# lixirui142/VidToMe

Hardware: AMD Instinct MI355X
Metric: denoising steps/sec, 16-frame 512x512 SD-1.5 chunk, ratio=0.5 (higher is better)
Workload: dtype f16 tokens; matching f16-MFMA filter + f32 exact refine (f32-identical indices); attention f16 MFMA with f32 accumulate

## Files before the change

### include/vidtome_hip.h

```cpp
#ifndef VIDTOME_HIP_H
#define VIDTOME_HIP_H

#include <stddef.h>
#include <stdint.h>

#ifdef __cplusplus
extern "C" {
#endif

#define VTM_ABI_VERSION 2

enum vtm_dtype { VTM_F32 = 0, VTM_F16 = 1, VTM_BF16 = 2 };

enum vtm_status {
    VTM_OK = 0,
    VTM_EINVAL = -1,
    VTM_ELAUNCH = -2,
    VTM_EWORKSPACE = -3
};

typedef void *vtm_stream_t;

int vtm_version(void);
const char *vtm_last_error(void);
int vtm_build_ablations(void);

#define VTM_MATCH_ROW_PAD 256
#define VTM_MATCH_K_PAD 32
int64_t vtm_pad_rows(int64_t n);
int64_t vtm_pad_k(int64_t C);

int vtm_normalize_gather(const void *x0, int64_t P0, const void *x1, int64_t P1, int dtype, int64_t B,
                         int64_t C, const int32_t *rows, int64_t n, float *norms, float *out,
                         int64_t n_pad, int64_t C_pad, vtm_stream_t stream);

int vtm_match(const float *a, const float *b, int64_t B, int64_t Ns, int64_t Nd, int64_t Ns_pad,
              int64_t Nd_pad, int64_t C_pad, int align, uint64_t *best, vtm_stream_t stream);

size_t vtm_match_filtered_ws_bytes(int64_t B, int64_t C, int64_t Ns, int64_t Nd, int align);
int vtm_match_filtered(const void *x0, int64_t P0, const void *x1, int64_t P1, int dtype, int64_t B,
                       int64_t C, const int32_t *a_rows, int64_t Ns, const int32_t *b_rows, int64_t Nd,
                       int align, void *ws, size_t ws_bytes, uint64_t *best, int32_t *flags_out,
                       vtm_stream_t stream);
int vtm_match_filtered_seeded(const void *x0, int64_t P0, const void *x1, int64_t P1, int dtype, int64_t B,
                              int64_t C, const int32_t *a_rows, int64_t Ns, const int32_t *b_rows, int64_t Nd,
                              int align, void *ws, size_t ws_bytes, uint64_t *best, int32_t *flags_out,
                              int64_t seed_L, int64_t seed_N, const int32_t *seed_pos1, const int32_t *seed_table,
                              vtm_stream_t stream);
#define VTM_MATCH_ONE_LAUNCH 0
#define VTM_MATCH_SCOUT_RANGE 1
#define VTM_MATCH_SCOUT_STEPS(k) (((k) & 0xff) << 8)
int vtm_match_filtered_plan(const void *x0, int64_t P0, const void *x1, int64_t P1, int dtype, int64_t B,
                            int64_t C, const int32_t *a_rows, int64_t Ns, const int32_t *b_rows, int64_t Nd,
                            int align, void *ws, size_t ws_bytes, uint64_t *best, int32_t *flags_out,
                            int64_t seed_L, int64_t seed_N, const int32_t *seed_pos1, const int32_t *seed_table,
                            int mode, vtm_stream_t stream);

#define VTM_POSITION_ORDER_MAX_N 16360
size_t vtm_position_order_counter_ints(int64_t B, int64_t N);
size_t vtm_position_order_ws_bytes(int64_t B, int64_t Ns, int64_t Nd, int64_t N);
int vtm_position_order(const int32_t *a_rows, int64_t Ns, const int32_t *b_rows, int64_t Nd, int64_t B, int64_t L,
                       int64_t N, const int32_t *pos1, int64_t P0, int64_t P1, int32_t *counters, void *ws,
                       size_t ws_bytes, int32_t *a_sorted, int32_t *a_order, int32_t *b_sorted, int32_t *b_order,
                       int32_t *table, int shared_order, vtm_stream_t stream);
int vtm_match_filtered_ordered(const void *x0, int64_t P0, const void *x1, int64_t P1, int dtype, int64_t B,
                               int64_t C, const int32_t *a_sorted, int64_t Ns, const int32_t *b_sorted, int64_t Nd,
                               int align, void *ws, size_t ws_bytes, uint64_t *best, int32_t *flags_out, int64_t seed_L,
                               int64_t seed_N, const int32_t *seed_pos1, const int32_t *seed_table, int mode,
                               const int32_t *a_order, const int32_t *b_order, vtm_stream_t stream);

int vtm_decode_best(const uint64_t *best, int64_t n, float *node_max, int32_t *node_idx,
                    vtm_stream_t stream);

size_t vtm_sort_ws_bytes(int64_t rows, int64_t n);
int vtm_sort_desc(const uint64_t *best, int64_t rows, int64_t n, int32_t *perm, void *ws,
                  size_t ws_bytes, vtm_stream_t stream);

int vtm_partition_counts(int64_t N_in, int64_t unm_pre, int64_t tnum, int64_t ts, int64_t randf,
                         int64_t *Ns, int64_t *Nd);
int vtm_partition_local(const int32_t *cur, int64_t B, int64_t N_in, int64_t unm_pre, int64_t tnum,
                        int64_t ts, int64_t randf, int32_t *a_pos, int32_t *b_pos, int32_t *a_rows,
                        int32_t *b_rows, int64_t Ns, int64_t Nd, vtm_stream_t stream);

int vtm_partition_global(const int32_t *cur_local, int64_t B, int64_t Ml, int64_t anchor_base,
                         int64_t Mg, int local_is_src, int32_t *a_pos, int32_t *b_pos,
                         int32_t *a_rows, int32_t *b_rows, int32_t *seed_table, int64_t tokens,
                         const int32_t *anchor_pos, vtm_stream_t stream);

int vtm_anchor_pos(const int32_t *amap, int64_t B, int64_t M, int64_t L, int64_t tokens, const int32_t *old_pos,
                   int64_t Mg, int32_t *out, vtm_stream_t stream);

int vtm_anchor_maps(const int32_t *inv_g, int64_t N_in, int64_t off, const int32_t *new_cur, int64_t M, int64_t B,
                    int64_t Ml, int64_t L, int64_t tokens, const int32_t *old_pos, int64_t Mg, int32_t *loc, int32_t *amap,
                    int32_t *pos, vtm_stream_t stream);

int vtm_plan_apply(const uint64_t *best, const int32_t *perm, const int32_t *a_pos,
                   const int32_t *b_pos, const int32_t *a_rows, const int32_t *b_rows, int64_t B,
                   int64_t N_in, int64_t Ns, int64_t Nd, int64_t r, int align, int32_t *new_cur,
                   int32_t *inv, int32_t *unm_idx, int32_t *src_idx, int32_t *dst_idx,
                   vtm_stream_t stream);

int vtm_compose(const int32_t *inv_acc, const int32_t *inv_level, int64_t B, int64_t n,
                int64_t level_len, int64_t offset, int32_t *out, vtm_stream_t stream);

int vtm_gather_rows(const void *x0, int64_t P0, const void *x1, int64_t P1, int dtype, int64_t B,
                    int64_t C, const int32_t *map, int64_t M, void *out, int64_t out_rows,
                    vtm_stream_t stream);

enum { VTM_REDUCE_SUM = 0, VTM_REDUCE_PROD = 1, VTM_REDUCE_MEAN = 2, VTM_REDUCE_AMAX = 3, VTM_REDUCE_AMIN = 4 };
int vtm_merge_reduce(const void *x, int dtype, int64_t B, int64_t N, int64_t C, const int32_t *src_rows,
                     const int32_t *dst_rows, const int32_t *seg_dst, const int32_t *seg_order, int64_t r, int64_t Nd,
                     int mode, void *out, int64_t out_ld, int64_t out_row0, vtm_stream_t stream);

int vtm_unmerge_add(const void *y, int64_t M, const int32_t *inv, const void *resid, int dtype,
                    int64_t B, int64_t L, int64_t C, void *out, vtm_stream_t stream);

int vtm_attention(const void *q, int64_t ldq, const void *k, int64_t ldk, const void *vt,
                  int64_t ldvt, void *out, int64_t ldo, int dtype, int64_t B, int64_t h, int64_t M,
                  int64_t Mp, int64_t d, float scale, int share_groups, void *ws, size_t ws_bytes,
                  vtm_stream_t stream);

size_t vtm_attention_ws_bytes(int64_t B, int64_t h, int64_t Mq, int64_t Mk, int64_t d);

int vtm_attention_kv(const void *q, int64_t ldq, const void *k, int64_t ldk, const void *vt, int64_t ldvt,
                     void *out, int64_t ldo, int dtype, int64_t B, int64_t h, int64_t Mq, int64_t Mqp,
                     int64_t Mk, int64_t Mkp, int64_t d, float scale, int share_groups, void *ws, size_t ws_bytes,
                     vtm_stream_t stream);

int vtm_attention_kv_sets(const void *q, int64_t ldq, const void *k, int64_t ldk, const void *vt, int64_t ldvt,
                          void *out, int64_t ldo, int dtype, int64_t B, int64_t h, int64_t Mq, int64_t Mqp,
                          int64_t Mkp, int64_t d, float scale, int n_sets, const int64_t *set_start,
                          const int64_t *set_len, const float *set_weight, vtm_stream_t stream);

int vtm_attention_kv_bounded(const void *q, int64_t ldq, const void *k, int64_t ldk, const void *vt, int64_t ldvt,
                             void *out, int64_t ldo, int dtype, int64_t B, int64_t h, int64_t Mq, int64_t Mqp,
                             int64_t Mk, int64_t Mkp, int64_t d, float scale, const int32_t *q_count, void *ws,
                             size_t ws_bytes, vtm_stream_t stream);
int vtm_attention_kv_shared_bounded(const void *q, int64_t ldq, const void *k, int64_t ldk, const void *vt, int64_t ldvt,
                                    void *out, int64_t ldo, int dtype, int64_t B, int64_t h, int64_t Mq, int64_t Mqp,
                                    int64_t Mk, int64_t Mkp, int64_t d, float scale, int share_groups,
                                    const int32_t *q_count, void *ws, size_t ws_bytes, vtm_stream_t stream);
size_t vtm_attention_kv_bounded_ws_bytes(int64_t B, int64_t h, int64_t Mq, int64_t Mk, int64_t d);

int vtm_transpose_cols(const void *x, int64_t ldx, int dtype, int64_t BF, int64_t N, int64_t C, void *out, int64_t ldo,
                       vtm_stream_t stream);

size_t vtm_fold_keys_ws_bytes(int64_t B, int64_t M, int64_t n_ids);
int vtm_fold_keys(const int32_t *cur, int64_t B, int64_t M, int64_t L, const int32_t *cid, int64_t Ma, int64_t n_ids,
                  int dtype, void *ws, size_t ws_bytes, int32_t *key_sel, uint32_t *k_bias, int64_t ldkb,
                  int32_t *k_count, vtm_stream_t stream);
int vtm_attention_kv_folded(const void *q, int64_t ldq, const void *k, int64_t ldk, const void *vt, int64_t ldvt,
                            void *out, int64_t ldo, int dtype, int64_t B, int64_t h, int64_t Mq, int64_t Mqp,
                            int64_t Mk, int64_t Mkp, int64_t d, float scale, const int32_t *q_count,
                            const int32_t *k_count, const uint32_t *k_bias, int64_t ldkb, void *ws, size_t ws_bytes,
                            vtm_stream_t stream);

size_t vtm_compact_queries_ws_bytes(int64_t B, int64_t Nd);
int vtm_compact_queries(const int32_t *loc, int64_t B, int64_t Ml, int64_t U, int64_t Nd, void *ws, size_t ws_bytes,
                        int32_t *qc, int32_t *tmap, int32_t *count, vtm_stream_t stream);

int64_t vtm_panel_rows(int64_t n);
int vtm_to_panels(const void *x, int dtype, int64_t rows, int64_t C, const int32_t *order, void *out, int64_t rows_pad,
                  vtm_stream_t stream);
int vtm_layernorm_panels(const void *x, const void *gamma, const void *beta, int dtype, int64_t rows, int64_t C, float eps,
                         void *out, int64_t panel_rows, vtm_stream_t stream);
int vtm_gather_panels(const void *x0, int64_t P0, const void *x1, int64_t P1, int dtype, int64_t B, int64_t C,
                      const int32_t *map, int64_t map_ld, const int32_t *map2, int64_t n, void *out, int64_t rows_per_sample,
                      vtm_stream_t stream);
int vtm_ff_geglu(const void *x_panels, int64_t n, int64_t n_pad, const void *w1_panels, int64_t D, int64_t w_rows_pad,
                 int64_t K, const float *bias, int dtype, void *out_panels, vtm_stream_t stream);
int vtm_linear_panels(const void *x_panels, int64_t n, int64_t n_pad, const void *w_panels, int64_t N, int64_t w_rows_pad,
                      int64_t K, const float *bias, const void *resid, int dtype, void *out, int64_t ldo,
                      vtm_stream_t stream);

int vtm_cfg_ddim(const void *x, const void *eps_uncond, const void *eps_cond, int dtype, int64_t n,
                 float guidance, float a, float b, float c, float d, void *eps_out, void *x_out,
                 vtm_stream_t stream);

int vtm_layernorm(const void *x, const void *gamma, const void *beta, int dtype, int64_t rows, int64_t C,
                  float eps, void *out, vtm_stream_t stream);

int vtm_geglu(const void *x, int dtype, int64_t rows, int64_t D, void *out, vtm_stream_t stream);

int vtm_linear_rows(const void *x0, int64_t P0, const void *x1, int64_t P1, int dtype, int64_t B, int64_t K,
                    const int32_t *rows, int64_t rows_ld, const int32_t *rows2, int64_t n, const void *W,
                    const void *bias, int64_t N, void *out, int64_t ldo, int64_t out_batch_stride,
                    int transposed, vtm_stream_t stream);

enum { VTM_LINEAR_NONE = 0, VTM_LINEAR_RESID = 1, VTM_LINEAR_GEGLU = 2 };
int vtm_linear_f32(const float *x0, int64_t P0, const float *x1, int64_t P1, int64_t B, int64_t K,
                   const int32_t *rows, int64_t rows_ld, const int32_t *rows2, int64_t n, const float *W,
                   const float *bias, int64_t N, int epilogue, const float *resid, void *out, int out_dtype,
                   int64_t ldo, int64_t out_batch_stride, int transposed, vtm_stream_t stream);

int vtm_lora_fold(const void *w, int dtype, const float *up, const float *down, int64_t c_out, int64_t c_in,
                  int64_t r, void *out, vtm_stream_t stream);

int vtm_dora_norms(const void *w, int dtype, const float *up, const float *down, int64_t c_out, int64_t c_in,
                   int64_t r, int64_t k_dora, float *norms, vtm_stream_t stream);
int vtm_dora_fold(const void *w, int dtype, const float *up, const float *down, const float *magnitude,
                  const float *norms, int64_t c_out, int64_t c_in, int64_t r, int64_t k_dora, void *out,
                  vtm_stream_t stream);

#ifdef __cplusplus
}
#endif
#endif
```

### vidtome_amd/_lib.py

```python
from __future__ import annotations

import ctypes
import functools
import os
import threading
from typing import Optional, Tuple

import torch

_HERE = os.path.dirname(os.path.abspath(__file__))
ABI_VERSION = 2
LIB_PATH = os.environ.get("VIDTOME_HIP_LIB") or os.path.join(_HERE, "lib", "libvidtome_hip.so")

VTM_F32, VTM_F16, VTM_BF16 = 0, 1, 2
ROW_PAD, K_PAD = 256, 32

_DT = {torch.float32: VTM_F32, torch.float16: VTM_F16, torch.bfloat16: VTM_BF16}

_vp, _i64, _int, _f32 = ctypes.c_void_p, ctypes.c_int64, ctypes.c_int, ctypes.c_float
_lib: Optional[ctypes.CDLL] = None

_SIGNATURES = {
    "vtm_version": ([], _int),
    "vtm_last_error": ([], ctypes.c_char_p),
    "vtm_build_ablations": ([], _int),
    "vtm_pad_rows": ([_i64], _i64),
    "vtm_pad_k": ([_i64], _i64),
    "vtm_normalize_gather": ([_vp, _i64, _vp, _i64, _int, _i64, _i64, _vp, _i64, _vp, _vp, _i64, _i64, _vp], _int),
    "vtm_match": ([_vp, _vp, _i64, _i64, _i64, _i64, _i64, _i64, _int, _vp, _vp], _int),
    "vtm_match_filtered_ws_bytes": ([_i64, _i64, _i64, _i64, _int], ctypes.c_size_t),
    "vtm_match_filtered": ([_vp, _i64, _vp, _i64, _int, _i64, _i64, _vp, _i64, _vp, _i64, _int, _vp, ctypes.c_size_t,
                            _vp, _vp, _vp], _int),
    "vtm_match_filtered_plan": ([_vp, _i64, _vp, _i64, _int, _i64, _i64, _vp, _i64, _vp, _i64, _int, _vp, ctypes.c_size_t,
                                 _vp, _vp, _i64, _i64, _vp, _vp, _int, _vp], _int),
    "vtm_match_filtered_ordered": ([_vp, _i64, _vp, _i64, _int, _i64, _i64, _vp, _i64, _vp, _i64, _int, _vp, ctypes.c_size_t,
                                    _vp, _vp, _i64, _i64, _vp, _vp, _int, _vp, _vp, _vp], _int),
    "vtm_position_order_counter_ints": ([_i64, _i64], ctypes.c_size_t),
    "vtm_position_order_ws_bytes": ([_i64, _i64, _i64, _i64], ctypes.c_size_t),
    "vtm_position_order": ([_vp, _i64, _vp, _i64, _i64, _i64, _i64, _vp, _i64, _i64, _vp, _vp, ctypes.c_size_t, _vp, _vp, _vp,
                            _vp, _vp, _int, _vp], _int),
    "vtm_match_filtered_seeded": ([_vp, _i64, _vp, _i64, _int, _i64, _i64, _vp, _i64, _vp, _i64, _int, _vp, ctypes.c_size_t,
                                   _vp, _vp, _i64, _i64, _vp, _vp, _vp], _int),
    "vtm_anchor_pos": ([_vp, _i64, _i64, _i64, _i64, _vp, _i64, _vp, _vp], _int),
    "vtm_decode_best": ([_vp, _i64, _vp, _vp, _vp], _int),
    "vtm_sort_ws_bytes": ([_i64, _i64], ctypes.c_size_t),
    "vtm_sort_desc": ([_vp, _i64, _i64, _vp, _vp, ctypes.c_size_t, _vp], _int),
    "vtm_partition_counts": ([_i64, _i64, _i64, _i64, _i64, ctypes.POINTER(_i64), ctypes.POINTER(_i64)], _int),
    "vtm_partition_local": ([_vp, _i64, _i64, _i64, _i64, _i64, _i64, _vp, _vp, _vp, _vp, _i64, _i64, _vp], _int),
    "vtm_partition_global": ([_vp, _i64, _i64, _i64, _i64, _int, _vp, _vp, _vp, _vp, _vp, _i64, _vp, _vp], _int),
    "vtm_plan_apply": ([_vp, _vp, _vp, _vp, _vp, _vp, _i64, _i64, _i64, _i64, _i64, _int, _vp, _vp, _vp, _vp,
                        _vp, _vp], _int),
    "vtm_compose": ([_vp, _vp, _i64, _i64, _i64, _i64, _vp, _vp], _int),
    "vtm_gather_rows": ([_vp, _i64, _vp, _i64, _int, _i64, _i64, _vp, _i64, _vp, _i64, _vp], _int),
    "vtm_unmerge_add": ([_vp, _i64, _vp, _vp, _int, _i64, _i64, _i64, _vp, _vp], _int),
    "vtm_merge_reduce": ([_vp, _int, _i64, _i64, _i64, _vp, _vp, _vp, _vp, _i64, _i64, _int, _vp, _i64, _i64, _vp], _int),
    "vtm_attention": ([_vp, _i64, _vp, _i64, _vp, _i64, _vp, _i64, _int, _i64, _i64, _i64, _i64, _i64, _f32,
                       _int, _vp, ctypes.c_size_t, _vp], _int),
    "vtm_attention_ws_bytes": ([_i64, _i64, _i64, _i64, _i64], ctypes.c_size_t),
    "vtm_attention_kv": ([_vp, _i64, _vp, _i64, _vp, _i64, _vp, _i64, _int, _i64, _i64, _i64, _i64, _i64, _i64, _i64,
                          _f32, _int, _vp, ctypes.c_size_t, _vp], _int),
    "vtm_attention_kv_sets": ([_vp, _i64, _vp, _i64, _vp, _i64, _vp, _i64, _int, _i64, _i64, _i64, _i64, _i64, _i64, _f32,
                               _int, ctypes.POINTER(_i64), ctypes.POINTER(_i64), ctypes.POINTER(_f32), _vp], _int),
    "vtm_attention_kv_bounded": ([_vp, _i64, _vp, _i64, _vp, _i64, _vp, _i64, _int, _i64, _i64, _i64, _i64, _i64, _i64, _i64,
                                  _f32, _vp, _vp, ctypes.c_size_t, _vp], _int),
    "vtm_attention_kv_shared_bounded": ([_vp, _i64, _vp, _i64, _vp, _i64, _vp, _i64, _int, _i64, _i64, _i64, _i64, _i64, _i64, _i64,
                                         _f32, _int, _vp, _vp, ctypes.c_size_t, _vp], _int),
    "vtm_attention_kv_bounded_ws_bytes": ([_i64, _i64, _i64, _i64, _i64], ctypes.c_size_t),
    "vtm_anchor_maps": ([_vp, _i64, _i64, _vp, _i64, _i64, _i64, _i64, _i64, _vp, _i64, _vp, _vp, _vp, _vp], _int),
    "vtm_transpose_cols": ([_vp, _i64, _int, _i64, _i64, _i64, _vp, _i64, _vp], _int),
    "vtm_fold_keys_ws_bytes": ([_i64, _i64, _i64], ctypes.c_size_t),
    "vtm_fold_keys": ([_vp, _i64, _i64, _i64, _vp, _i64, _i64, _int, _vp, ctypes.c_size_t, _vp, _vp, _i64, _vp, _vp], _int),
    "vtm_attention_kv_folded": ([_vp, _i64, _vp, _i64, _vp, _i64, _vp, _i64, _int, _i64, _i64, _i64, _i64, _i64, _i64, _i64,
                                 _f32, _vp, _vp, _vp, _i64, _vp, ctypes.c_size_t, _vp], _int),
    "vtm_compact_queries_ws_bytes": ([_i64, _i64], ctypes.c_size_t),
    "vtm_compact_queries": ([_vp, _i64, _i64, _i64, _i64, _vp, ctypes.c_size_t, _vp, _vp, _vp, _vp], _int),
    "vtm_panel_rows": ([_i64], _i64),
    "vtm_to_panels": ([_vp, _int, _i64, _i64, _vp, _vp, _i64, _vp], _int),
    "vtm_layernorm_panels": ([_vp, _vp, _vp, _int, _i64, _i64, _f32, _vp, _i64, _vp], _int),
    "vtm_gather_panels": ([_vp, _i64, _vp, _i64, _int, _i64, _i64, _vp, _i64, _vp, _i64, _vp, _i64, _vp], _int),
    "vtm_ff_geglu": ([_vp, _i64, _i64, _vp, _i64, _i64, _i64, _vp, _int, _vp, _vp], _int),
    "vtm_linear_panels": ([_vp, _i64, _i64, _vp, _i64, _i64, _i64, _vp, _vp, _int, _vp, _i64, _vp], _int),
    "vtm_cfg_ddim": ([_vp, _vp, _vp, _int, _i64, _f32, _f32, _f32, _f32, _f32, _vp, _vp, _vp], _int),
    "vtm_layernorm": ([_vp, _vp, _vp, _int, _i64, _i64, _f32, _vp, _vp], _int),
    "vtm_geglu": ([_vp, _int, _i64, _i64, _vp, _vp], _int),
    "vtm_linear_rows": ([_vp, _i64, _vp, _i64, _int, _i64, _i64, _vp, _i64, _vp, _i64, _vp, _vp, _i64, _vp, _i64, _i64,
                         _int, _vp], _int),
    "vtm_lora_fold": ([_vp, _int, _vp, _vp, _i64, _i64, _i64, _vp, _vp], _int),
    "vtm_dora_norms": ([_vp, _int, _vp, _vp, _i64, _i64, _i64, _i64, _vp, _vp], _int),
    "vtm_dora_fold": ([_vp, _int, _vp, _vp, _vp, _vp, _i64, _i64, _i64, _i64, _vp, _vp], _int),
    "vtm_linear_f32": ([_vp, _i64, _vp, _i64, _i64, _i64, _vp, _i64, _vp, _i64, _vp, _vp, _i64, _int, _vp, _vp, _int, _i64,
                        _i64, _int, _vp], _int),
}


def exported_symbols():
    return sorted(_SIGNATURES)


def lib() -> ctypes.CDLL:
    global _lib
    if _lib is None:
        if not os.path.exists(LIB_PATH):
            raise RuntimeError(
                f"{LIB_PATH} is missing: build it with `python -m vidtome_amd.build` (hipcc, gfx950). "
                "vidtome_amd has no CPU / eager fallback.")
        L = ctypes.CDLL(LIB_PATH)
        for name, (argtypes, restype) in _SIGNATURES.items():
            fn = getattr(L, name)
            fn.argtypes = argtypes
            fn.restype = restype
        if L.vtm_version() != ABI_VERSION:
            raise RuntimeError("libvidtome_hip.so ABI version mismatch")
        if L.vtm_build_ablations() != 0 and os.environ.get("VIDTOME_ALLOW_ABLATED") != "1":
            raise RuntimeError(f"{LIB_PATH} was built with ablation switches (mask {L.vtm_build_ablations():#x}); "
                               "set VIDTOME_ALLOW_ABLATED=1 to load it for a timing experiment")
        _lib = L
    return _lib


def _check(rc: int, what: str) -> None:
    if rc != 0:
        msg = lib().vtm_last_error()
        raise RuntimeError(f"{what} failed ({rc}): {msg.decode() if msg else ''}")


def _stream() -> int:
    return torch.cuda.current_stream().cuda_stream


def _on_device(fn):
    @functools.wraps(fn)
    def guarded(*args, **kwargs):
        dev = next((a.device if isinstance(a, torch.Tensor) else a for a in args
                    if isinstance(a, (torch.Tensor, torch.device))), None)
        if dev is None or dev.type != "cuda" or dev.index is None or dev.index == torch.cuda.current_device():
            return fn(*args, **kwargs)
        with torch.cuda.device(dev.index):
            return fn(*args, **kwargs)
    return guarded


def _ptr(t: Optional[torch.Tensor]) -> Optional[int]:
    return None if t is None else t.data_ptr()


_WS: dict = {}
_WS_LOCK = threading.Lock()


def _workspace(tag: str, nbytes: int, device: torch.device) -> torch.Tensor:
    key = (device.index, torch.cuda.current_stream(device).cuda_stream, tag, threading.get_ident())
    buf = _WS.get(key)
    if buf is None or buf.numel() < nbytes:
        new = torch.empty((max(int(nbytes), 16),), dtype=torch.uint8, device=device)
        with _WS_LOCK:
            if buf is None:
                alive = {t.ident for t in threading.enumerate()}
                for k in [k for k in list(_WS) if k[3] not in alive]:
                    _WS.pop(k, None)
            _WS[key] = new
        buf = new
    return buf


def release_workspaces() -> None:
    with _WS_LOCK:
        _WS.clear()
        _ZEROED.clear()


def _req(t: torch.Tensor, name: str) -> torch.Tensor:
    if not t.is_cuda:
        raise RuntimeError(f"{name} must live on the GPU (vidtome_amd has no CPU path)")
    if not t.is_contiguous():
        raise RuntimeError(f"{name} must be contiguous")
    return t


def dtype_code(t: torch.Tensor) -> int:
    try:
        return _DT[t.dtype]
    except KeyError:
        raise RuntimeError(f"unsupported dtype {t.dtype}") from None


def pad_rows(n: int) -> int:
    return (n + ROW_PAD - 1) // ROW_PAD * ROW_PAD


def pad_k(c: int) -> int:
    return (c + K_PAD - 1) // K_PAD * K_PAD


@_on_device
def normalize_gather(x0: torch.Tensor, x1: Optional[torch.Tensor], rows: torch.Tensor
                     ) -> Tuple[torch.Tensor, torch.Tensor]:
    _req(x0, "x0"), _req(rows, "rows")
    B, P0, C = x0.shape
    P1 = 0 if x1 is None else _req(x1, "x1").shape[1]
    n = rows.shape[1]
    n_pad, C_pad = pad_rows(n), pad_k(C)
    out = torch.empty((B, C_pad // 8, 2, n_pad, 4), dtype=torch.float32, device=x0.device)
    norms = torch.empty((B, max(n, 1)), dtype=torch.float32, device=x0.device)
    _check(lib().vtm_normalize_gather(_ptr(x0), P0, _ptr(x1), P1, dtype_code(x0), B, C, _ptr(rows), n,
                                      _ptr(norms), _ptr(out), n_pad, C_pad, _stream()), "vtm_normalize_gather")
    return out, norms


@_on_device
def match(a: torch.Tensor, b: torch.Tensor, Ns: int, Nd: int, align: bool) -> torch.Tensor:
    B, G, _, Ns_pad, _ = a.shape
    C_pad, Nd_pad = G * 8, b.shape[3]
    best = torch.empty((1 if align else B, Ns), dtype=torch.int64, device=a.device)
    _check(lib().vtm_match(_ptr(a), _ptr(b), B, Ns, Nd, Ns_pad, Nd_pad, C_pad, int(align), _ptr(best), _stream()),
           "vtm_match")
    return best


MATCH_ONE_LAUNCH, MATCH_SCOUT_RANGE = 0, 1


@_on_device
def match_filtered(x0: torch.Tensor, x1: Optional[torch.Tensor], a_rows: torch.Tensor, b_rows: torch.Tensor,
                   align: bool, want_flag: bool = False, seed=None, mode: int = MATCH_ONE_LAUNCH,
                   stats_host: Optional[torch.Tensor] = None, order=None, scout_steps: int = 0):
    _req(x0, "x0"), _req(a_rows, "a_rows"), _req(b_rows, "b_rows")
    B, P0, C = x0.shape
    P1 = 0 if x1 is None else _req(x1, "x1").shape[1]
    Ns, Nd = a_rows.shape[1], b_rows.shape[1]
    nbytes = lib().vtm_match_filtered_ws_bytes(B, C, Ns, Nd, int(align))
    ws = _workspace("match", nbytes, x0.device)
    best = torch.empty((1 if align else B, Ns), dtype=torch.int64, device=x0.device)
    flag = torch.zeros((8,), dtype=torch.int32, device=x0.device) if want_flag else None
    flags_out = _ptr(flag)
# ... 195 lines not shown
    if r > 0:
        keys = ((-1 - dst_idx.long()) << 32).contiguous()
        order = sort_desc(keys)
        seg_dst = torch.gather(dst_idx, 1, order.long()).contiguous()
    else:
        order = seg_dst = dst_idx
    _check(lib().vtm_merge_reduce(_ptr(x), dtype_code(x), B, N, C, _ptr(src_rows), _ptr(dst_rows), _ptr(seg_dst), _ptr(order),
                                  r, Nd, REDUCE_MODES[mode], _ptr(out), out.shape[1], out_row0, _stream()), "vtm_merge_reduce")
    return out


@_on_device
def unmerge_add(y: torch.Tensor, inv: torch.Tensor, resid: Optional[torch.Tensor]) -> torch.Tensor:
    _req(y, "y"), _req(inv, "inv")
    B, Mp, C = y.shape
    L = inv.shape[1]
    out = torch.empty((B, L, C), dtype=y.dtype, device=y.device)
    if resid is not None:
        _req(resid, "resid")
        if resid.numel() != out.numel() or resid.dtype != y.dtype:
            raise RuntimeError("residual shape/dtype mismatch")
    _check(lib().vtm_unmerge_add(_ptr(y), Mp, _ptr(inv), _ptr(resid), dtype_code(y), B, L, C, _ptr(out), _stream()),
           "vtm_unmerge_add")
    return out


@_on_device
def transpose_cols(x: torch.Tensor, c0: int, C: int) -> torch.Tensor:
    _req(x, "x")
    BF, N, ld = x.shape
    if x.stride(2) != 1 or x.stride(1) != ld or x.stride(0) != N * ld or c0 % 8 or C % 8:
        raise RuntimeError("transpose_cols: dense (BF, N, ld) input, column window aligned to 8")
    Np = (N + 7) // 8 * 8
    out = torch.empty((BF, C, Np), dtype=x.dtype, device=x.device)
    _check(lib().vtm_transpose_cols(x.data_ptr() + c0 * x.element_size(), ld, dtype_code(x), BF, N, C, _ptr(out), Np, _stream()),
           "vtm_transpose_cols")
    return out


SEED_MATCHER = os.environ.get("VIDTOME_SEED", "1") != "0"

SPLIT_ALL_BOUNDED = os.environ.get("VIDTOME_ATT_SPLIT_ALL", "1") != "0"

FOLD_KEYS = os.environ.get("VIDTOME_FOLD_KEYS", "1") != "0"


def _attention_ws(B: int, heads: int, Mq: int, Mk: int, d: int, device):
    nb = int(lib().vtm_attention_ws_bytes(B, heads, Mq, Mk, d))
    if nb == 0:
        return None, 0
    return _workspace("attention", nb, device), nb


@_on_device
def attention(q: torch.Tensor, k: torch.Tensor, vt: torch.Tensor, heads: int, M: int, scale: float,
              share_groups: int = 1) -> torch.Tensor:
    B, Mp, C = q.shape
    d = C // heads
    if q.stride(2) != 1 or k.stride(2) != 1 or vt.stride(2) != 1:
        raise RuntimeError("attention operands must be contiguous along their last axis")
    if q.stride(0) != Mp * q.stride(1) or k.stride(0) != Mp * k.stride(1) or vt.stride(0) != C * vt.stride(1):
        raise RuntimeError("attention operands must have dense batch strides")
    out = torch.zeros((B, Mp, C), dtype=q.dtype, device=q.device) if Mp != M else \
        torch.empty((B, Mp, C), dtype=q.dtype, device=q.device)
    ws, nb = _attention_ws(B, heads, M, M, d, q.device)
    _check(lib().vtm_attention(q.data_ptr(), q.stride(1), k.data_ptr(), k.stride(1), vt.data_ptr(), vt.stride(1),
                               out.data_ptr(), C, dtype_code(q), B, heads, M, Mp, d, float(scale),
                               int(share_groups), _ptr(ws), nb, _stream()), "vtm_attention")
    return out


@_on_device
def cfg_ddim(x: Optional[torch.Tensor], eps_uncond: torch.Tensor, eps_cond: Optional[torch.Tensor], guidance: float,
             a: float, b: float, c: float, d: float, want_eps: bool = False):
    _req(eps_uncond, "eps_uncond")
    n = eps_uncond.numel()
    b, c, d = (float(torch.tensor(v, dtype=torch.float32).to(eps_uncond.dtype)) for v in (b, c, d))
    a = float(torch.tensor(a, dtype=torch.float32))
    x_out = torch.empty_like(eps_uncond) if x is not None else None
    eps_out = torch.empty_like(eps_uncond) if (want_eps or x is None) else None
    _check(lib().vtm_cfg_ddim(_ptr(x), _ptr(eps_uncond), _ptr(eps_cond), dtype_code(eps_uncond), n, float(guidance),
                              float(a), float(b), float(c), float(d), _ptr(eps_out), _ptr(x_out), _stream()),
           "vtm_cfg_ddim")
    return (x_out, eps_out) if want_eps else (x_out if x is not None else eps_out)


@_on_device
def layernorm(x: torch.Tensor, weight: Optional[torch.Tensor], bias: Optional[torch.Tensor], eps: float) -> torch.Tensor:
    _req(x, "x")
    C = x.shape[-1]
    xc = x.contiguous()
    for name, p in (("weight", weight), ("bias", bias)):
        if p is not None and (p.dtype != x.dtype or p.numel() != C or p.device != x.device):
            raise RuntimeError(f"vidtome_amd: layernorm {name} must be a ({C},) {x.dtype} tensor on {x.device}")
    out = torch.empty_like(xc)
    _check(lib().vtm_layernorm(_ptr(xc), _ptr(weight.contiguous() if weight is not None else None),
                               _ptr(bias.contiguous() if bias is not None else None), dtype_code(xc),
                               xc.numel() // C, C, float(eps), _ptr(out), _stream()), "vtm_layernorm")
    return out


@_on_device
def attention_kv(q: torch.Tensor, k: torch.Tensor, vt: torch.Tensor, heads: int, Mq: int, Mk: int, scale: float,
                 use_workspace: bool = True, q_count: Optional[torch.Tensor] = None,
                 k_fold: Optional[Tuple[torch.Tensor, torch.Tensor]] = None, share_groups: int = 1) -> torch.Tensor:
    if share_groups != 1 and k_fold is not None:
        raise RuntimeError("attention_kv: shared probabilities do not go with folded keys")
    if k_fold is not None and q.dtype == torch.float32:
        raise RuntimeError("attention_kv: fp32 keys are never folded (k_fold takes fp16 / bf16 operands)")
    B, Mqp, C = q.shape
    Mkp = k.shape[1]
    d = C // heads
    if q.stride(2) != 1 or k.stride(2) != 1 or vt.stride(2) != 1:
        raise RuntimeError("attention operands must be contiguous along their last axis")
    if q.stride(0) != Mqp * q.stride(1) or k.stride(0) != Mkp * k.stride(1) or vt.stride(0) != C * vt.stride(1):
        raise RuntimeError("attention operands must have dense batch strides")
    out = torch.zeros((B, Mqp, C), dtype=q.dtype, device=q.device) if Mqp != Mq else \
        torch.empty((B, Mqp, C), dtype=q.dtype, device=q.device)
    ws, nb = _attention_ws(B, heads, Mq, Mk, d, q.device) if use_workspace else (None, 0)
    if q_count is not None and (q_count.dtype != torch.int32 or q_count.numel() != B or not q_count.is_cuda):
        raise RuntimeError("attention_kv: q_count must be a (B,) int32 device tensor")
    if q_count is not None and use_workspace and SPLIT_ALL_BOUNDED:
        nb2 = int(lib().vtm_attention_kv_bounded_ws_bytes(B, heads, Mq, Mk, d))
        if nb2 > nb:
            ws, nb = _workspace("attention", nb2, q.device), nb2
    if share_groups != 1 and q_count is not None:
        _check(lib().vtm_attention_kv_shared_bounded(q.data_ptr(), q.stride(1), k.data_ptr(), k.stride(1), vt.data_ptr(),
                                                     vt.stride(1), out.data_ptr(), C, dtype_code(q), B, heads, Mq, Mqp, Mk, Mkp,
                                                     d, float(scale), int(share_groups), _ptr(q_count), _ptr(ws), nb, _stream()),
               "vtm_attention_kv_shared_bounded")
        return out
    if k_fold is not None:
        k_count, k_bias = k_fold
        if k_count.dtype != torch.int32 or k_count.numel() != B or k_bias.dtype != torch.int32 or k_bias.dim() != 2 \
                or k_bias.shape[0] != B or k_bias.shape[1] < Mk or not k_bias.is_contiguous():
            raise RuntimeError("attention_kv: k_fold must be ((B,) int32 counts, (B, >= Mk) int32 bias words)")
        _check(lib().vtm_attention_kv_folded(q.data_ptr(), q.stride(1), k.data_ptr(), k.stride(1), vt.data_ptr(), vt.stride(1),
                                             out.data_ptr(), C, dtype_code(q), B, heads, Mq, Mqp, Mk, Mkp, d, float(scale),
                                             _ptr(q_count), _ptr(k_count), _ptr(k_bias), k_bias.shape[1], _ptr(ws), nb,
                                             _stream()), "vtm_attention_kv_folded")
        return out
    if q_count is not None:
        _check(lib().vtm_attention_kv_bounded(q.data_ptr(), q.stride(1), k.data_ptr(), k.stride(1), vt.data_ptr(),
                                              vt.stride(1), out.data_ptr(), C, dtype_code(q), B, heads, Mq, Mqp, Mk, Mkp,
                                              d, float(scale), _ptr(q_count), _ptr(ws), nb, _stream()),
               "vtm_attention_kv_bounded")
        return out
    _check(lib().vtm_attention_kv(q.data_ptr(), q.stride(1), k.data_ptr(), k.stride(1), vt.data_ptr(), vt.stride(1),
                                  out.data_ptr(), C, dtype_code(q), B, heads, Mq, Mqp, Mk, Mkp, d, float(scale),
                                  int(share_groups), _ptr(ws), nb, _stream()), "vtm_attention_kv")
    return out


MAX_KEY_SETS = 8


@_on_device
def attention_kv_range(q: torch.Tensor, k: torch.Tensor, vt: torch.Tensor, heads: int, Mq: int, start: int, Mk: int,
                       scale: float) -> torch.Tensor:
    start, Mk = int(start), int(Mk)
    B, Mqp, C = q.shape
    Mkp = k.shape[1]
    if start % 8 or start < 0 or Mk < 1 or start + Mk > Mkp or start + Mk > vt.shape[2]:
        raise RuntimeError("attention_kv_range: the range must start on a multiple of 8 and lie inside k and vt")
    if start == 0:
        return attention_kv(q, k, vt, heads, Mq, Mk, scale)
    d = C // heads
    if q.stride(2) != 1 or k.stride(2) != 1 or vt.stride(2) != 1:
        raise RuntimeError("attention operands must be contiguous along their last axis")
    if q.stride(0) != Mqp * q.stride(1) or k.stride(0) != Mkp * k.stride(1) or vt.stride(0) != C * vt.stride(1):
        raise RuntimeError("attention operands must have dense batch strides")
    out = torch.zeros((B, Mqp, C), dtype=q.dtype, device=q.device) if Mqp != Mq else \
        torch.empty((B, Mqp, C), dtype=q.dtype, device=q.device)
    ws, nb = _attention_ws(B, heads, Mq, Mk, d, q.device)
    es = k.element_size()
    _check(lib().vtm_attention_kv(q.data_ptr(), q.stride(1), k.data_ptr() + start * k.stride(1) * es, k.stride(1),
                                  vt.data_ptr() + start * es, vt.stride(1), out.data_ptr(), C, dtype_code(q), B, heads, Mq, Mqp,
                                  Mk, Mkp, d, float(scale), 1, _ptr(ws), nb, _stream()), "vtm_attention_kv")
    return out


@_on_device
def attention_kv_sets(q: torch.Tensor, k: torch.Tensor, vt: torch.Tensor, heads: int, Mq: int, sets, scale: float
                      ) -> torch.Tensor:
    sets = [(int(s), int(n), float(w)) for s, n, w in sets]
    if not 1 <= len(sets) <= MAX_KEY_SETS:
        raise RuntimeError(f"attention_kv_sets: 1 .. {MAX_KEY_SETS} key sets, got {len(sets)}")
    if q.dtype not in (torch.float16, torch.bfloat16) or k.dtype != q.dtype or vt.dtype != q.dtype:
        raise RuntimeError("attention_kv_sets: q, k and vt must share one of fp16 / bf16 (fp32 models keep the module path)")
    B, Mqp, C = q.shape
    Mkp = k.shape[1]
    d = C // heads
    if q.stride(2) != 1 or k.stride(2) != 1 or vt.stride(2) != 1:
        raise RuntimeError("attention operands must be contiguous along their last axis")
    if q.stride(0) != Mqp * q.stride(1) or k.stride(0) != Mkp * k.stride(1) or vt.stride(0) != C * vt.stride(1):
        raise RuntimeError("attention operands must have dense batch strides")
    if k.shape[0] != B or vt.shape[0] != B or k.shape[2] != C or vt.shape[1] != C:
        raise RuntimeError("attention_kv_sets: k must be (B, Mkp, C) and vt (B, C, ldvt)")
    if len(sets) == 1 and sets[0][2] == 1.0:
        return attention_kv_range(q, k, vt, heads, Mq, sets[0][0], sets[0][1], scale)
    out = torch.zeros((B, Mqp, C), dtype=q.dtype, device=q.device) if Mqp != Mq else \
        torch.empty((B, Mqp, C), dtype=q.dtype, device=q.device)
    n = len(sets)
    starts = (_i64 * n)(*[s for s, _, _ in sets])
    lens = (_i64 * n)(*[m for _, m, _ in sets])
    weights = (_f32 * n)(*[w for _, _, w in sets])
    _check(lib().vtm_attention_kv_sets(q.data_ptr(), q.stride(1), k.data_ptr(), k.stride(1), vt.data_ptr(), vt.stride(1),
                                       out.data_ptr(), C, dtype_code(q), B, heads, Mq, Mqp, Mkp, d, float(scale), n, starts,
                                       lens, weights, _stream()), "vtm_attention_kv_sets")
    return out


@_on_device
def compact_queries(loc: torch.Tensor, U: int, Nd: int) -> Tuple[torch.Tensor, torch.Tensor, torch.Tensor]:
    _req(loc, "loc")
    B, Ml = loc.shape
    i32 = dict(dtype=torch.int32, device=loc.device)
    qc, tmap, count = torch.empty((B, Ml), **i32), torch.empty((B, Ml), **i32), torch.empty((B,), **i32)
    nb = int(lib().vtm_compact_queries_ws_bytes(B, Nd))
    ws = _workspace("compact", nb, loc.device)
    _check(lib().vtm_compact_queries(_ptr(loc), B, Ml, U, Nd, _ptr(ws), nb, _ptr(qc), _ptr(tmap), _ptr(count), _stream()),
           "vtm_compact_queries")
    return qc, tmap, count


@_on_device
def fold_keys(cur: torch.Tensor, L: int, cid: torch.Tensor, n_ids: int, dtype: torch.dtype
              ) -> Tuple[torch.Tensor, torch.Tensor, torch.Tensor]:
    _req(cur, "cur")
    _req(cid, "cid")
    B, M = cur.shape
    Mp = (M + 7) // 8 * 8
    i32 = dict(dtype=torch.int32, device=cur.device)
    key_sel, k_bias, k_count = torch.empty((B, M), **i32), torch.empty((B, Mp), **i32), torch.empty((B,), **i32)
    code = {torch.float16: 1, torch.bfloat16: 2}[dtype]
    nb = int(lib().vtm_fold_keys_ws_bytes(B, M, n_ids))
    ws = _workspace("fold", nb, cur.device)
    _check(lib().vtm_fold_keys(_ptr(cur), B, M, L, _ptr(cid), cid.shape[1], n_ids, code, _ptr(ws), nb, _ptr(key_sel),
                               _ptr(k_bias), Mp, _ptr(k_count), _stream()), "vtm_fold_keys")
    return key_sel, k_bias, k_count


@_on_device
def geglu(x: torch.Tensor) -> torch.Tensor:
    _req(x, "x")
    D = x.shape[-1] // 2
    xc = x.contiguous()
    out = torch.empty(xc.shape[:-1] + (D,), dtype=x.dtype, device=x.device)
    _check(lib().vtm_geglu(_ptr(xc), dtype_code(xc), xc.numel() // (2 * D), D, _ptr(out), _stream()), "vtm_geglu")
    return out


@_on_device
def linear_rows(x0: torch.Tensor, x1: Optional[torch.Tensor], rows: Optional[torch.Tensor],
                rows2: Optional[torch.Tensor], n: int, weight: torch.Tensor, bias: Optional[torch.Tensor],
                transposed: bool = False, pad_to: int = 8, out: Optional[torch.Tensor] = None) -> torch.Tensor:
    _req(x0, "x0"), _req(weight, "weight")
    B, P0, K = x0.shape
    P1 = 0 if x1 is None else _req(x1, "x1").shape[1]
    N = weight.shape[0]
    if weight.shape[1] != K or weight.dtype != x0.dtype:
        raise RuntimeError("linear_rows: weight must be (N, K) in the token dtype")
    if rows is not None:
        _req(rows, "rows")
    if rows2 is not None:
        _req(rows2, "rows2")
    n_pad = (n + pad_to - 1) // pad_to * pad_to
    if out is None:
        out = torch.empty((B, N, n_pad) if transposed else (B, n_pad, N), dtype=x0.dtype, device=x0.device)
        if n_pad != n:
            (out[:, :, n:] if transposed else out[:, n:]).zero_()
    if out.stride(2) != 1:
        raise RuntimeError("linear_rows: out must be contiguous along its last axis")
    _check(lib().vtm_linear_rows(_ptr(x0), P0, _ptr(x1), P1, dtype_code(x0), B, K, _ptr(rows),
                                 0 if rows is None else rows.shape[1], _ptr(rows2), n, _ptr(weight),
                                 _ptr(bias.contiguous() if bias is not None else None), N, out.data_ptr(), out.stride(1),
                                 out.stride(0), int(transposed), _stream()), "vtm_linear_rows")
    return out


LINEAR_NONE, LINEAR_RESID, LINEAR_GEGLU = 0, 1, 2
_EPILOGUES = {"none": LINEAR_NONE, "resid": LINEAR_RESID, "geglu": LINEAR_GEGLU}


@_on_device
def linear_f32(x0: torch.Tensor, x1: Optional[torch.Tensor], rows: Optional[torch.Tensor],
               rows2: Optional[torch.Tensor], n: int, weight: torch.Tensor, bias: Optional[torch.Tensor],
               epilogue: str = "none", resid: Optional[torch.Tensor] = None, out_dtype: torch.dtype = torch.float32,
               transposed: bool = False, pad_to: int = 8, out: Optional[torch.Tensor] = None) -> torch.Tensor:
    _req(x0, "x0"), _req(weight, "weight")
    B, P0, K = x0.shape
    P1 = 0 if x1 is None else _req(x1, "x1").shape[1]
    N = weight.shape[0]
    if x0.dtype != torch.float32 or weight.dtype != torch.float32 or weight.shape[1] != K \
            or (x1 is not None and x1.dtype != torch.float32):
        raise RuntimeError("linear_f32: tokens and weight must be fp32, weight (N, K)")
    if out_dtype not in (torch.float32, torch.float16):
        raise RuntimeError("linear_f32: out_dtype must be fp32 or fp16")
    epi = _EPILOGUES[epilogue]
    Nout = N // 2 if epi == LINEAR_GEGLU else N
    if bias is not None:
        bias = bias.detach().float().contiguous()
    for t, name in ((rows, "rows"), (rows2, "rows2")):
        if t is not None:
            _req(t, name)
    n_pad = (n + pad_to - 1) // pad_to * pad_to
    if out is None:
        out = torch.empty((B, Nout, n_pad) if transposed else (B, n_pad, Nout), dtype=out_dtype, device=x0.device)
        if n_pad != n:
            (out[:, :, n:] if transposed else out[:, n:]).zero_()
    if out.stride(2) != 1 or out.dtype != out_dtype:
        raise RuntimeError("linear_f32: out must be of out_dtype and contiguous along its last axis")
    if epi == LINEAR_RESID and (resid is None or resid.dtype != torch.float32 or resid.shape[0] != B
                                or resid.stride()[B == 1:] != out.stride()[B == 1:]):
        raise RuntimeError("linear_f32: resid must be fp32 with the strides of the result")
    _check(lib().vtm_linear_f32(_ptr(x0), P0, _ptr(x1), P1, B, K, _ptr(rows), 0 if rows is None else rows.shape[1],
                                _ptr(rows2), n, _ptr(weight), _ptr(bias), N, epi, _ptr(resid), out.data_ptr(),
                                dtype_code(out), out.stride(1), out.stride(0), int(transposed), _stream()),
           "vtm_linear_f32")
    return out


def panel_rows(n: int) -> int:
    return (n + ROW_PAD - 1) // ROW_PAD * ROW_PAD


@_on_device
def to_panels(x: torch.Tensor, order: Optional[torch.Tensor] = None, rows: Optional[int] = None) -> torch.Tensor:
    _req(x, "x")
    C = x.shape[-1]
    x2 = x.reshape(-1, C)
    n = x2.shape[0] if order is None else order.numel()
    n = n if rows is None else rows
    out = torch.empty((C // 8, panel_rows(n), 8), dtype=x.dtype, device=x.device)
    _check(lib().vtm_to_panels(_ptr(x2), dtype_code(x2), n, C, _ptr(order), _ptr(out), out.shape[1], _stream()),
           "vtm_to_panels")
    return out


@_on_device
def layernorm_panels(x: torch.Tensor, weight: Optional[torch.Tensor], bias: Optional[torch.Tensor], eps: float) -> torch.Tensor:
    _req(x, "x")
    C = x.shape[-1]
    xc = x.contiguous()
    rows = xc.numel() // C
    out = torch.empty((C // 8, panel_rows(rows), 8), dtype=x.dtype, device=x.device)
    _check(lib().vtm_layernorm_panels(_ptr(xc), _ptr(weight), _ptr(bias), dtype_code(xc), rows, C, float(eps), _ptr(out),
                                      out.shape[1], _stream()), "vtm_layernorm_panels")
    return out


@_on_device
def ff_geglu(x_panels: torch.Tensor, n: int, w1_panels: torch.Tensor, D: int, bias: Optional[torch.Tensor]) -> torch.Tensor:
    K = x_panels.shape[0] * 8
    out = torch.empty((D // 8, x_panels.shape[1], 8), dtype=x_panels.dtype, device=x_panels.device)
    _check(lib().vtm_ff_geglu(_ptr(x_panels), n, x_panels.shape[1], _ptr(w1_panels), D, w1_panels.shape[1], K, _ptr(bias),
                              dtype_code(x_panels), _ptr(out), _stream()), "vtm_ff_geglu")
    return out


@_on_device
def linear_panels(x_panels: torch.Tensor, n: int, w_panels: torch.Tensor, N: int, bias: Optional[torch.Tensor],
                  resid: Optional[torch.Tensor] = None, out: Optional[torch.Tensor] = None) -> torch.Tensor:
    K = x_panels.shape[0] * 8
    if x_panels.stride(2) != 1 or x_panels.stride(1) != 8 or w_panels.stride(2) != 1 or w_panels.stride(1) != 8 \
            or w_panels.shape[0] * 8 != K:
        raise RuntimeError("linear_panels: operands must be (K / 8, rows, 8) panel tensors (or row ranges of one)")
    if out is None:
        out = torch.empty((n, N), dtype=x_panels.dtype, device=x_panels.device)
    if out.stride(1) != 1 or out.shape[0] < n or out.shape[1] < N:
        raise RuntimeError("linear_panels: out must be an (n, N) view, contiguous along its rows")
    if resid is not None:
        _req(resid, "resid")
        if resid.numel() != n * N or resid.dtype != out.dtype or out.stride(0) != N:
            raise RuntimeError("linear_panels: residual shape / dtype mismatch")
    _check(lib().vtm_linear_panels(_ptr(x_panels), n, x_panels.stride(0) // 8, _ptr(w_panels), N, w_panels.stride(0) // 8, K,
                                   _ptr(bias), _ptr(resid), dtype_code(x_panels), out.data_ptr(), out.stride(0), _stream()),
           "vtm_linear_panels")
    return out


@_on_device
def gather_panels(x0: torch.Tensor, x1: Optional[torch.Tensor], rows: Optional[torch.Tensor], rows2: Optional[torch.Tensor],
                  n: int) -> torch.Tensor:
    _req(x0, "x0")
    B, P0, C = x0.shape
    P1 = 0 if x1 is None else _req(x1, "x1").shape[1]
    n_pad = panel_rows(n)
    out = torch.empty((C // 8, B * n_pad, 8), dtype=x0.dtype, device=x0.device)
    _check(lib().vtm_gather_panels(_ptr(x0), P0, _ptr(x1), P1, dtype_code(x0), B, C, _ptr(rows),
                                   0 if rows is None else rows.shape[1], _ptr(rows2), n, _ptr(out), n_pad, _stream()),
           "vtm_gather_panels")
    return out


@_on_device
def lora_fold(w: torch.Tensor, up: torch.Tensor, down: torch.Tensor, out: Optional[torch.Tensor] = None) -> torch.Tensor:
    _req(w, "w"), _req(up, "up"), _req(down, "down")
    c_out, c_in = w.shape
    r = up.shape[1]
    if up.dtype != torch.float32 or down.dtype != torch.float32 or tuple(up.shape) != (c_out, r) \
            or tuple(down.shape) != (r, c_in) or up.device != w.device or down.device != w.device:
        raise RuntimeError("lora_fold: up must be (c_out, r) and down (r, c_in) fp32 tensors on w's device")
    if out is None:
        out = torch.empty_like(w)
    _check(lib().vtm_lora_fold(_ptr(w), dtype_code(w), _ptr(up), _ptr(down), c_out, c_in, r, _ptr(_req(out, "out")),
                               _stream()), "vtm_lora_fold")
    return out


def _fold_operands(what: str, w: torch.Tensor, up: torch.Tensor, down: torch.Tensor, k_dora: int) -> Tuple[int, int, int]:
    _req(w, "w"), _req(up, "up"), _req(down, "down")
    c_out, c_in = w.shape
    r = up.shape[1]
    if up.dtype != torch.float32 or down.dtype != torch.float32 or tuple(up.shape) != (c_out, r) \
            or tuple(down.shape) != (r, c_in) or up.device != w.device or down.device != w.device:
        raise RuntimeError(f"{what}: up must be (c_out, r) and down (r, c_in) fp32 tensors on w's device")
    if not 0 < k_dora <= r:
        raise RuntimeError(f"{what}: k_dora {k_dora} not in [1, r = {r}]")
    return c_out, c_in, r


@_on_device
def dora_norms(w: torch.Tensor, up: torch.Tensor, down: torch.Tensor, k_dora: int,
               out: Optional[torch.Tensor] = None) -> torch.Tensor:
    c_out, c_in, r = _fold_operands("dora_norms", w, up, down, k_dora)
    if out is None:
        out = torch.empty(c_out, dtype=torch.float32, device=w.device)
    if out.dtype != torch.float32 or tuple(out.shape) != (c_out,) or out.device != w.device:
        raise RuntimeError("dora_norms: out must be an fp32 (c_out,) tensor on w's device")
    _check(lib().vtm_dora_norms(_ptr(w), dtype_code(w), _ptr(up), _ptr(down), c_out, c_in, r, k_dora, _ptr(_req(out, "out")),
                                _stream()), "vtm_dora_norms")
    return out


@_on_device
def dora_fold(w: torch.Tensor, up: torch.Tensor, down: torch.Tensor, magnitude: torch.Tensor, k_dora: int,
              norms: Optional[torch.Tensor] = None, out: Optional[torch.Tensor] = None) -> torch.Tensor:
    c_out, c_in, r = _fold_operands("dora_fold", w, up, down, k_dora)
    if norms is None:
        norms = dora_norms(w, up, down, k_dora)
    for name, t in (("magnitude", magnitude), ("norms", norms)):
        if t.dtype != torch.float32 or tuple(t.shape) != (c_out,) or t.device != w.device:
            raise RuntimeError(f"dora_fold: {name} must be an fp32 (c_out,) tensor on w's device")
    if out is None:
        out = torch.empty_like(w)
    _check(lib().vtm_dora_fold(_ptr(w), dtype_code(w), _ptr(up), _ptr(down), _ptr(_req(magnitude, "magnitude")),
                               _ptr(_req(norms, "norms")), c_out, c_in, r, k_dora, _ptr(_req(out, "out")), _stream()),
           "vtm_dora_fold")
    return out
```

### vidtome_amd/csrc/attention.hip

```cpp
#include "attention_plan.h"

#include <algorithm>
#include <type_traits>

namespace {

template <typename T, int D>
__global__ __launch_bounds__(waves_for(D) * 64) void attention_combine_kernel(
    const float *__restrict__ partial, T *__restrict__ out, int64_t ldo, int64_t H, int64_t M, int64_t Mp, int64_t nqb,
    int64_t id0, int nsplit, int xcd_groups, const int32_t *__restrict__ q_count, const DevPlan *__restrict__ dev_plan) {
    constexpr int WAVES = waves_for(D), NT = WAVES * 64, QB = WAVES * QW, DV = (D + 31) / 32;
    constexpr bool PV16 = pv16_for(D);
    constexpr int NA = acc_floats(D), NM = max_floats(D), REC = rec_floats(D);
    const int tid = threadIdx.x, lane = tid & 63, wave = tid >> 6;
    const int l31 = lane & 31, hi = lane >> 5;
    int64_t rec0 = (int64_t)blockIdx.x * nsplit;
    int64_t pos = id0 + blockIdx.x;
    if (dev_plan != nullptr) {
        if ((int)blockIdx.x >= dev_plan->split_items) return;
        nqb = dev_plan->nqb;
        xcd_groups = nqb >= 64 ? xcd_groups : 0;
        pos = dev_plan->tier[0].items + blockIdx.x;
        int ti = 1;
        while (ti + 1 < dev_plan->ntiers && pos >= dev_plan->tier[ti + 1].item0) ++ti;
        const DevTier tr = dev_plan->tier[ti];
        nsplit = tr.nsplit;
        rec0 = tr.rec0 + (pos - tr.item0) * tr.nsplit;
    }
    const int64_t lin = item_of(pos, nqb, xcd_groups);
    const int64_t b = lin / (nqb * H), h = (lin / nqb) % H;
    const int64_t q0 = (lin % nqb) * QB + wave * QW;
    if (q_count != nullptr && (lin % nqb) * QB >= (int64_t)q_count[b]) return;
    float acc[NA], m[NM], l = 0.0f;
#pragma unroll
    for (int r = 0; r < NA; ++r) acc[r] = 0.0f;
#pragma unroll
    for (int j = 0; j < NM; ++j) m[j] = -INFINITY;
    for (int sp = 0; sp < nsplit; ++sp) {
        const float *pp = partial + (rec0 + sp) * REC * NT + tid;
        float fa[NM], fb[NM];
#pragma unroll
        for (int j = 0; j < NM; ++j) {
            const float ms = pp[(NA + j) * NT];
            const float mn = fmaxf(m[j], ms);
            fa[j] = __builtin_amdgcn_exp2f(m[j] - mn);
            fb[j] = __builtin_amdgcn_exp2f(ms - mn);
            m[j] = mn;
        }
        l = l * fa[0] + pp[(NA + NM) * NT] * fb[0];
#pragma unroll
        for (int r = 0; r < NA; ++r) {
            const int j = PV16 ? (r >> 2) & 1 : 0;
            acc[r] = acc[r] * fa[j] + pp[r * NT] * fb[j];
        }
    }
    if constexpr (PV16) {
        f32x4 o[(D + 16) / 16][2];
#pragma unroll
        for (int r = 0; r < NA; ++r) o[r >> 3][(r >> 2) & 1][r & 3] = acc[r];
        write_output16<T, D>(o, out, ldo, b, h, q0, M, Mp, lane);
    } else {
        f32x16 o[DV];
#pragma unroll
        for (int r = 0; r < NA; ++r) o[r >> 4][r & 15] = acc[r];
        write_output<T, D>(o, l, out, ldo, b, h, q0, M, Mp, l31, hi);
    }
}

template <typename T, int D>
__global__ __launch_bounds__(waves_for(D) * 64) void attention_combine_parts_kernel(
    const float *__restrict__ partial, T *__restrict__ out, int64_t ldo, int64_t H, int64_t M, int64_t Mp, int64_t nqb,
    int64_t id0, int nsplit, int xcd_groups, const int32_t *__restrict__ q_count) {
    using elem = typename Frag<T>::elem;
    static_assert(!pv16_for(D), "32-row O^T layout");
    constexpr int WAVES = waves_for(D), NT = WAVES * 64, QB = WAVES * QW;
    constexpr int NA = acc_floats(D), REC = rec_floats(D);
    constexpr bool SPARE = (D % 32) != 0;
    constexpr int LREG_ALL = SPARE ? (D / 32) * 16 + ((D % 32) & 3) + 4 * ((D % 32) >> 3) : 0;
    constexpr int LHI = ((D % 32) >> 2) & 1;
    const int tid = threadIdx.x, lane = tid & 63, wave = tid >> 6;
    const int l31 = lane & 31, hi = lane >> 5;
    const int64_t lin = item_of(id0 + blockIdx.x, nqb, xcd_groups);
    const int64_t b = lin / (nqb * H), h = (lin / nqb) % H;
    const int64_t q0 = (lin % nqb) * QB + wave * QW;
    if (q_count != nullptr && (lin % nqb) * QB >= (int64_t)q_count[b]) return;
    const int r0 = (int)blockIdx.y * 8;
    const float *p0 = partial + (int64_t)blockIdx.x * nsplit * REC * NT + tid;
    float m = -INFINITY;
#pragma unroll 4
    for (int sp = 0; sp < nsplit; ++sp) m = fmaxf(m, p0[((int64_t)sp * REC + NA) * NT]);
    float acc[8], den = 0.0f;
#pragma unroll
    for (int i = 0; i < 8; ++i) acc[i] = 0.0f;
#pragma unroll 4
    for (int sp = 0; sp < nsplit; ++sp) {
        const float *pp = p0 + (int64_t)sp * REC * NT;
        const float ms = pp[NA * NT];
        const float w = ms == -INFINITY ? 0.0f : __builtin_amdgcn_exp2f(ms - m);
        den = __builtin_fmaf(pp[(SPARE ? LREG_ALL : NA + 1) * NT], w, den);
#pragma unroll
        for (int i = 0; i < 8; ++i) acc[i] = __builtin_fmaf(pp[(r0 + i) * NT], w, acc[i]);
    }
    const float l_tot = SPARE ? __shfl(den, l31 + 32 * LHI, 64) : den + __shfl_xor(den, 32, 64);
    const float inv_l = 1.0f / l_tot;
    const int64_t qi = q0 + l31;
    if (qi < M) {
        T *op = out + (b * Mp + qi) * ldo + h * D;
        const int dv = r0 >> 4, g0 = (r0 & 15) >> 2;
#pragma unroll
        for (int gi = 0; gi < 2; ++gi) {
            const int d0 = dv * 32 + 8 * (g0 + gi) + 4 * hi;
            if (d0 < D) {
                elem w4[4];
#pragma unroll
                for (int e = 0; e < 4; ++e) w4[e] = (elem)(acc[gi * 4 + e] * inv_l);
                *reinterpret_cast<uint2 *>(op + d0) = *reinterpret_cast<uint2 *>(w4);
            }
        }
    }
}

template <typename T, int D, bool FOLD>
__global__ __launch_bounds__(waves_for(D) * 64, (D <= 48 ? 4 : D <= 96 ? 4 : 1)) void attention_kernel(
    const T *__restrict__ q, int64_t ldq, const T *__restrict__ k, int64_t ldk,
    const T *__restrict__ vt, int64_t ldvt, T *__restrict__ out, int64_t ldo, int64_t H,
    int64_t M, int64_t Mp, int64_t Mk_arg, int64_t Mkp, float scale_log2e, int64_t src_batch, int64_t nqb, int64_t nwhole,
    int nsplit_tail, float *__restrict__ partial_base, int xcd_groups, const int32_t *__restrict__ q_count,
    int64_t split_major_items, const int32_t *__restrict__ k_count, const uint32_t *__restrict__ k_bias, int64_t ldkb,
    const DevPlan *__restrict__ dev_plan) {
    using F = Frag<T>;
    using vec = typename F::vec;
    using elem = typename F::elem;
    constexpr int WAVES = waves_for(D), NT = WAVES * 64, QB = WAVES * QW;
    constexpr int DK = (D + 15) / 16;
    constexpr int DV = (D + 31) / 32;
    constexpr bool PV16 = pv16_for(D);
    constexpr int DV16 = (D + 16) / 16, VROWS = vrows_for(D);
    constexpr bool SPARE = (D % 32) != 0;
    constexpr bool BIAS = (D % 16) != 0;
    constexpr int BIAS_HI = (D % 16) / 8, BIAS_E = D % 8;
    static_assert(!FOLD || (BIAS && D % 8 == 0 && D % 16 == 8), "key folding needs the spare k-slots of a d % 16 == 8 head");
    constexpr int K_STRIDE = DK * 16 + 8;
    constexpr int DCH = D / 8;
    constexpr int K_CHUNKS = KV * DCH;
    constexpr int V_CHUNKS = D * (KV / 8);
    constexpr int K_PER_T = (K_CHUNKS + NT - 1) / NT;
    constexpr int V_PER_T = (V_CHUNKS + NT - 1) / NT;
    constexpr int SK_TILE = KV * K_STRIDE, SV_TILE = VROWS * VT_STRIDE;

    extern __shared__ __attribute__((aligned(16))) char smem[];
    elem *sK = reinterpret_cast<elem *>(smem);
    elem *sV = sK + 2 * SK_TILE;

    const int tid = threadIdx.x, lane = tid & 63, wave = tid >> 6;
    const int l31 = lane & 31, hi = lane >> 5;
    const int l15 = lane & 15, g16 = lane >> 4;
    int64_t tier_item0 = nwhole, tier_wg0 = nwhole, tier_rec0 = 0;
    if (dev_plan != nullptr) {
        nqb = dev_plan->nqb;
        xcd_groups = nqb >= 64 ? xcd_groups : 0;
        int ti = 0;
        while (ti + 1 < dev_plan->ntiers && (int)blockIdx.x >= dev_plan->tier[ti + 1].wg0) ++ti;
        const DevTier tr = dev_plan->tier[ti];
        if ((int64_t)blockIdx.x >= (int64_t)tr.wg0 + (int64_t)tr.items * tr.nsplit) return;
        nwhole = dev_plan->tier[0].items;
        nsplit_tail = tr.nsplit;
        split_major_items = tr.items;
        tier_item0 = tr.item0;
        tier_wg0 = tr.wg0;
        tier_rec0 = tr.rec0;
    }
    const bool tail_wg = (int64_t)blockIdx.x >= nwhole;
    const int64_t tail_id = (int64_t)blockIdx.x - tier_wg0;
    const int nsplit = tail_wg ? nsplit_tail : 1;
    const int64_t tail_item = split_major_items ? tail_id % split_major_items : tail_id / nsplit;
    const int split = !tail_wg ? 0 : split_major_items ? (int)(tail_id / split_major_items) : (int)(tail_id % nsplit);
    const int64_t lin = item_of(tail_wg ? tier_item0 + tail_item : (int64_t)blockIdx.x, nqb, xcd_groups);
    float *partial = tail_wg ? partial_base + (tier_rec0 + tail_item * nsplit + split) * rec_floats(D) * (waves_for(D) * 64) : nullptr;
    const int64_t b = lin / (nqb * H), h = (lin / nqb) % H;
    const int64_t bq = b % src_batch;
    const int64_t q0 = (lin % nqb) * QB + wave * QW;
    const int64_t C = H * D;
    int64_t Mk = Mk_arg;
    if constexpr (FOLD) {
        const int64_t kc = k_count[b];
        Mk = kc < Mk_arg ? (kc > 0 ? kc : 1) : Mk_arg;
    }
    if (q_count != nullptr && (lin % nqb) * QB >= (int64_t)q_count[b]) return;

    for (int i = tid; i < 2 * KV * (K_STRIDE - D); i += NT) {
        const int row = i / (K_STRIDE - D), c = D + i % (K_STRIDE - D);
        if (FOLD && (c == D + 2 || c == D + 3)) continue;
        sK[row * K_STRIDE + c] = (elem)((BIAS && c == D) ? 1.0f : 0.0f);
    }
    if constexpr (VROWS > D) {
        for (int i = tid; i < 2 * (VROWS - D) * VT_STRIDE; i += NT) {
            const int bufi = i / ((VROWS - D) * VT_STRIDE), rem = i % ((VROWS - D) * VT_STRIDE);
            const int row = D + rem / VT_STRIDE, c = rem % VT_STRIDE;
            sV[bufi * SV_TILE + row * VT_STRIDE + c] = (elem)((row == D) ? 1.0f : 0.0f);
        }
    }

    vec qf[DK];
    {
        const int64_t qi = q0 + l31;
        const T *qp = q + (bq * Mp + (qi < M ? qi : 0)) * ldq + h * D;
#pragma unroll
        for (int ks = 0; ks < DK; ++ks) {
            const int d0 = ks * 16 + hi * 8;
            uint4 v = make_uint4(0, 0, 0, 0);
            if (d0 < D && qi < M) v = *reinterpret_cast<const uint4 *>(qp + d0);
            qf[ks] = *reinterpret_cast<vec *>(&v);
            if constexpr (BIAS) {
#pragma unroll
                for (int e = 0; e < 8; ++e) qf[ks][e] = (elem)((float)qf[ks][e] * scale_log2e);
            }
        }
        if constexpr (FOLD) {
            if (hi == BIAS_HI) {
                qf[DK - 1][BIAS_E + 2] = (elem)1.0f;
                qf[DK - 1][BIAS_E + 3] = (elem)1.0f;
            }
        }
    }

    uint32_t kgo[K_PER_T], vgo[V_PER_T];
    int koff[K_PER_T], voff[V_PER_T], krow[K_PER_T], vkey[V_PER_T];
    bool kok[K_PER_T], vok[V_PER_T];
#pragma unroll
    for (int i = 0; i < K_PER_T; ++i) {
        const int c = tid + i * NT;
        kok[i] = c < K_CHUNKS;
        krow[i] = c / DCH;
        kgo[i] = kok[i] ? (uint32_t)(krow[i] * (int)ldk + (c % DCH) * 8) * 2u : 0u;
        koff[i] = krow[i] * K_STRIDE + (c % DCH) * 8;
    }
#pragma unroll
    for (int i = 0; i < V_PER_T; ++i) {
        const int c = tid + i * NT;
        vok[i] = c < V_CHUNKS;
        vkey[i] = (c % (KV / 8)) * 8;
        vgo[i] = vok[i] ? (uint32_t)((c / (KV / 8)) * (int)ldvt + vkey[i]) * 2u : 0u;
        voff[i] = (c / (KV / 8)) * VT_STRIDE + (vkey[i] & ~15) + ((vkey[i] >> 3) & 1) * 4;
    }
    const auto rsrc_k = __builtin_amdgcn_make_buffer_rsrc(const_cast<T *>(k + bq * Mkp * ldk + h * D), 0, 0x7fffffff, 0x00020000);
    const auto rsrc_v = __builtin_amdgcn_make_buffer_rsrc(const_cast<T *>(vt + (b * C + h * D) * ldvt), 0, 0x7fffffff, 0x00020000);
    const uint32_t kstep = (uint32_t)(KV * ldk) * 2u, vstep = (uint32_t)KV * 2u;
    uint32_t so_k = 0, so_v = 0;
    const auto rsrc_b = __builtin_amdgcn_make_buffer_rsrc(const_cast<uint32_t *>(FOLD ? k_bias + b * ldkb : nullptr), 0, 0x7fffffff, 0x00020000);
    uint32_t so_b = 0, rbias = 0;
    [[maybe_unused]] const uint32_t bgo = (uint32_t)(tid & (KV - 1)) * 4u;
    auto fetch = [](const auto &rsrc, uint32_t voff_, uint32_t soff_) {
        return __builtin_bit_cast(uint4, __builtin_amdgcn_raw_buffer_load_b128(rsrc, voff_, soff_, 0));
    };

    uint4 rk[K_PER_T], rv[V_PER_T];
    auto issue_full = [&]() {
#pragma unroll
        for (int i = 0; i < K_PER_T; ++i) rk[i] = fetch(rsrc_k, kgo[i], so_k);
#pragma unroll
        for (int i = 0; i < V_PER_T; ++i) rv[i] = fetch(rsrc_v, vgo[i], so_v);
        if constexpr (FOLD) {
            rbias = __builtin_amdgcn_raw_buffer_load_b32(rsrc_b, bgo, so_b, 0);
            so_b += (uint32_t)KV * 4u;
        }
        so_k += kstep;
        so_v += vstep;
    };
    auto issue_tail = [&](int64_t key0) {
#pragma unroll
        for (int i = 0; i < K_PER_T; ++i) {
            uint4 v = make_uint4(0, 0, 0, 0);
            if (kok[i] && key0 + krow[i] < Mk) v = fetch(rsrc_k, kgo[i], so_k);
            rk[i] = v;
        }
#pragma unroll
        for (int i = 0; i < V_PER_T; ++i) {
            uint4 v = make_uint4(0, 0, 0, 0);
            const int64_t key = key0 + vkey[i];
            if (vok[i] && key < Mk) {
                v = fetch(rsrc_v, vgo[i], so_v);
                mask_keys(v, (int)(Mk - key));
// ... 97 lines not shown
            }
        };

        auto raise_shift = [&]() {
            float mt = fmaxf(s[0][0], s[1][0]);
#pragma unroll
            for (int r = 1; r < 16; ++r) mt = fmaxf(fmaxf(mt, s[0][r]), s[1][r]);
            if constexpr (BIAS) {
                mt = fmaxf(mt, __shfl_xor(mt, 32, 64));
                if (!__all(m_bias + mt <= m_run + DEFER_THR)) {
                    const float m_new = (float)(elem)(fmaxf(m_run, m_bias + mt));
                    const float alpha = __builtin_amdgcn_exp2f(m_run - m_new);
                    const float delta = m_bias - m_new;
                    m_run = m_new;
                    m_bias = m_new;
                    l_run *= alpha;
                    rescale(alpha);
#pragma unroll
                    for (int kb = 0; kb < 2; ++kb)
#pragma unroll
                        for (int r = 0; r < 16; ++r) s[kb][r] += delta;
                    if (hi == BIAS_HI) qf[DK - 1][BIAS_E] = (elem)(-m_new);
                }
            } else {
                mt = fmaxf(mt, __shfl_xor(mt, 32, 64)) * scale_log2e;
                if (!__all(mt <= m_run + DEFER_THR)) {
                    const float m_new = fmaxf(m_run, mt);
                    const float alpha = __builtin_amdgcn_exp2f(m_run - m_new);
                    m_run = m_new;
                    l_run *= alpha;
                    rescale(alpha);
                }
            }
        };
        vec pf[4];
        auto softmax_step = [&](int st) {
            float p[8];
#pragma unroll
            for (int e = 0; e < 8; ++e) {
                const float sv = s[st >> 1][8 * (st & 1) + e];
                p[e] = __builtin_amdgcn_exp2f(BIAS ? sv : __builtin_fmaf(sv, scale_log2e, -m_run));
                if constexpr (!SPARE) l_run += p[e];
            }
            F::pack8(pf[st], p);
        };
        compute_s();
        if constexpr (PV16) {
            static_assert(BIAS, "16-row O^T blocks imply a spare k-slot");
            const elem *vp = sV + buf * SV_TILE + l15 * VT_STRIDE + (g16 & 1) * 16 + (g16 >> 1) * 8;
#pragma unroll
            for (int st = 0; st < 4; ++st) softmax_step(st);
            uint32_t pw[16];
#pragma unroll
            for (int st = 0; st < 4; ++st) {
                const u32x4 w = __builtin_bit_cast(u32x4, pf[st]);
#pragma unroll
                for (int j = 0; j < 4; ++j) pw[4 * st + j] = w[j];
            }
#pragma unroll
            for (int j = 0; j < 5; ++j) pw[j] = F::pmax3(pw[3 * j], pw[3 * j + 1], pw[3 * j + 2]);
            const uint32_t pr = F::pmax3(F::pmax3(pw[0], pw[1], pw[2]), F::pmax3(pw[3], pw[4], pw[15]), pw[15]);
            const uint32_t ptop = max(pr >> 16, pr & 0xffffu);
            if (__any(ptop > F::BITS_256 || m_run == -INFINITY)) {
                compute_s();
                raise_shift();
#pragma unroll
                for (int st = 0; st < 4; ++st) softmax_step(st);
            }
#pragma unroll
            for (int ks = 0; ks < 2; ++ks) {
                vec a[DV16];
#pragma unroll
                for (int dv = 0; dv < DV16; ++dv)
                    a[dv] = *reinterpret_cast<const vec *>(vp + ks * 32 + dv * 16 * VT_STRIDE);
                u32x4 x = __builtin_bit_cast(u32x4, pf[2 * ks]), y = __builtin_bit_cast(u32x4, pf[2 * ks + 1]);
#pragma unroll
                for (int w = 0; w < 4; ++w) {
                    const auto r = __builtin_amdgcn_permlane16_swap(x[w], y[w], false, false);
                    x[w] = r[0];
                    y[w] = r[1];
                }
                const vec p0 = __builtin_bit_cast(vec, x), p1 = __builtin_bit_cast(vec, y);
#pragma unroll
                for (int dv = 0; dv < DV16; ++dv) {
                    o16[dv][0] = F::mfma16(a[dv], p0, o16[dv][0]);
                    o16[dv][1] = F::mfma16(a[dv], p1, o16[dv][1]);
                }
            }
        } else {
            raise_shift();
#pragma unroll
            for (int st = 0; st < 4; ++st) softmax_step(st);
#pragma unroll
            for (int dv = 0; dv < DV; ++dv) {
                const elem *vp = sV + buf * SV_TILE + (dv * 32 + l31) * VT_STRIDE + 8 * hi;
#pragma unroll
                for (int st = 0; st < 4; ++st)
                    o[dv] = F::mfma(*reinterpret_cast<const vec *>(vp + st * 16), pf[st], o[dv]);
            }
        }
    };
    using std::false_type;
    using std::true_type;

    const int ntiles = (int)((Mk + KV - 1) / KV), nfull = (int)(Mk / KV);
    const int tps = (ntiles + nsplit - 1) / nsplit;
    const int tb = split * tps, te = tb + tps < ntiles ? tb + tps : ntiles;
    const int fe = te < nfull ? te : nfull;
    so_k = (uint32_t)tb * kstep;
    so_v = (uint32_t)tb * vstep;
    so_b = (uint32_t)tb * (uint32_t)KV * 4u;
    if (tb < fe) issue_full(); else issue_tail((int64_t)tb * KV);
    write_lds(0);
    __syncthreads();

    int t = tb;
    int buf = 0;
    for (; t + 1 < fe; ++t) {
        issue_full();
        tile(false_type{}, buf, (int64_t)t * KV);
        write_lds(buf ^ 1);
        __syncthreads();
        buf ^= 1;
    }
    if (t < fe) {
        const bool ragged_next = te > fe;
        if (ragged_next) issue_tail((int64_t)fe * KV);
        tile(false_type{}, buf, (int64_t)t * KV);
        if (ragged_next) write_lds(buf ^ 1);
        __syncthreads();
        ++t;
        buf ^= 1;
    }
    if (t < te) tile(true_type{}, buf, (int64_t)t * KV);

    if (partial) {
        constexpr int NA = acc_floats(D), NM = max_floats(D);
        float *pp = partial + tid;
        if constexpr (PV16) {
#pragma unroll
            for (int r = 0; r < NA; ++r) pp[r * NT] = o16[r >> 3][(r >> 2) & 1][r & 3];
#pragma unroll
            for (int qh = 0; qh < 2; ++qh) pp[(NA + qh) * NT] = __shfl(m_run, 16 * qh + l15, 64);
        } else {
#pragma unroll
            for (int r = 0; r < NA; ++r) pp[r * NT] = o[r >> 4][r & 15];
            pp[NA * NT] = m_run;
        }
        pp[(NA + NM) * NT] = l_run;
        return;
    }
    if constexpr (PV16)
        write_output16<T, D>(o16, out, ldo, b, h, q0, M, Mp, lane);
    else
        write_output<T, D>(o, l_run, out, ldo, b, h, q0, M, Mp, l31, hi);
}

constexpr size_t lds_for(int D) { return (size_t)2 * (KV * ((D + 15) / 16 * 16 + 8) + vrows_for(D) * VT_STRIDE) * 2; }

template <typename T, int D, bool FOLD>
void launch_main(const Call &c, const Launch &g) {
    hipLaunchKernelGGL((attention_kernel<T, D, FOLD>), dim3((unsigned)g.wgs), dim3(waves_for(D) * 64), lds_for(D), c.s,
                       (const T *)c.q, c.ldq, (const T *)c.k, c.ldk, (const T *)c.vt, c.ldvt, (T *)c.out, c.ldo, c.h, c.M, c.Mp,
                       c.Mk, c.Mkp, g.scale_log2e, g.src_batch, g.nqb, g.whole, g.nsplit, g.partial, g.xcd_groups, c.q_count,
                       g.split_major, c.k_count, c.k_bias, c.ldkb, plan_of(g));
}

template <typename T, int D>
void launch_combine(const Call &c, const Launch &g) {
    if constexpr (!pv16_for(D) && acc_floats(D) % 8 == 0) {
        if (g.plan == nullptr && g.split_items * 4 <= vtm::device_cus()) {
            hipLaunchKernelGGL((attention_combine_parts_kernel<T, D>), dim3((unsigned)g.split_items, (unsigned)(acc_floats(D) / 8)),
                               dim3(waves_for(D) * 64), 0, c.s, (const float *)g.partial, (T *)c.out, c.ldo, c.h, c.M, c.Mp,
                               g.nqb, g.whole, g.nsplit, g.xcd_groups, c.q_count);
            return;
        }
    }
    hipLaunchKernelGGL((attention_combine_kernel<T, D>), dim3((unsigned)g.split_items), dim3(waves_for(D) * 64), 0, c.s,
                       (const float *)g.partial, (T *)c.out, c.ldo, c.h, c.M, c.Mp, g.nqb, g.whole, g.nsplit, g.xcd_groups,
                       c.q_count, plan_of(g));
}

template <typename T, int D, bool FOLD = false>
Family make_family() {
    Family f;
    f.qb = waves_for(D) * QW;
    f.wg_per_cu = D <= 48 ? 2 : 1;
    f.rec_bytes = (size_t)rec_floats(D) * (waves_for(D) * 64) * sizeof(float);
    f.xcd_min_nqb = 64;
    f.ws_devplan_min_tiles = 16;
    if constexpr (lds_for(D) > 64 * 1024) f.lds_opt_in = opt_in_lds<attention_kernel<T, D, FOLD>, lds_for(D)>;
    f.main = launch_main<T, D, FOLD>;
    f.combine = launch_combine<T, D>;
    return f;
}

int shape16_for(int64_t d, int share_groups, int dtype) {
    if (d != 40 || (dtype != VTM_F16 && dtype != VTM_BF16)) return 0;
    return share_groups <= 3 ? share_groups : 0;
}

size_t ws_bytes_any(int64_t B, int64_t h, int64_t Mq, int64_t Mk, int64_t d, bool bounded) {
    if (B <= 0 || h <= 0 || Mq <= 0 || Mk <= 0) return 0;
    return with_head_dim(d, [&](auto dim) {
        constexpr int D = decltype(dim)::value;
        size_t n = ws_bytes(make_family<__half, D>(), B, h, Mq, Mk, bounded);
        if constexpr (D == 40) {
            n = std::max(n, ws_bytes(family16s(VTM_F16, false), B, h, Mq, Mk, bounded));
            for (int ng = 2; ng <= 3; ++ng)
                if (B % ng == 0) n = std::max(n, ws_bytes(family16g(VTM_F16, ng), B, h, Mq, Mk, bounded));
        }
        return n;
    });
}

int check_call(const Call &c, int64_t d, const char *who) {
    VTM_REQUIRE(c.q && c.k && c.vt && c.out && (!c.fold || (c.k_count && c.k_bias)), "%s: null pointer", who);
    VTM_REQUIRE(c.B > 0 && c.h > 0 && c.M > 0 && c.Mk > 0 && c.Mp >= c.M && c.Mkp >= c.Mk && (c.fold ? c.ldkb >= c.Mk : d > 0),
                "%s: bad sizes", who);
    VTM_REQUIRE(c.share_groups >= 1 && c.B % c.share_groups == 0, "%s: B %% share_groups != 0", who);
    if (c.fold)
        VTM_REQUIRE(d == 40 || d == 8, "%s: head dim %lld has no spare k-slots for the bias (d = 8, 40 do)", who, (long long)d);
    VTM_REQUIRE(c.ldq % 8 == 0 && c.ldk % 8 == 0 && c.ldvt % 8 == 0 && c.ldo % 4 == 0 && c.ldvt >= c.Mk,
                "%s: leading dimensions must keep 16-byte alignment (ldvt >= Mk, %% 8)", who);
    VTM_REQUIRE((c.Mkp * c.ldk + d) * 2 < (1ll << 31) && (d * c.ldvt + c.Mkp) * 2 < (1ll << 31) &&
                    (!c.fold || c.Mkp * 4 < (1ll << 31)),
                "%s: a (sample, head) slice of K or V^T must stay below 2 GiB", who);
    return VTM_OK;
}

}

VTM_EXPORT size_t vtm_attention_ws_bytes(int64_t B, int64_t h, int64_t Mq, int64_t Mk, int64_t d) {
    return ws_bytes_any(B, h, Mq, Mk, d, false);
}

VTM_EXPORT size_t vtm_attention_kv_bounded_ws_bytes(int64_t B, int64_t h, int64_t Mq, int64_t Mk, int64_t d) {
    return ws_bytes_any(B, h, Mq, Mk, d, true);
}

static int attention_any(const void *q, int64_t ldq, const void *k, int64_t ldk, const void *vt, int64_t ldvt,
                         void *out, int64_t ldo, int dtype, int64_t B, int64_t h, int64_t Mq, int64_t Mqp, int64_t Mk,
                         int64_t Mkp, int64_t d, float scale, int share_groups, void *ws, size_t ws_bytes,
                         const int32_t *q_count, vtm_stream_t stream) {
    const Call c{q, ldq, k, ldk, vt, ldvt, out, ldo, dtype, B, h, Mq, Mqp, Mk, Mkp, scale, share_groups, ws, ws_bytes,
                 q_count, vtm::as_stream(stream), false, nullptr, nullptr, 0};
    if (const int e = check_call(c, d, "vtm_attention")) return e;
    if (dtype == VTM_F32) return attention_f32(c, d);
    const int ng = shape16_for(d, share_groups, dtype);
    if (ng == 1) return attention16(c);
    if (ng > 1 && (ng * (B / share_groups) * h * d * ldvt) * 2 < (1ll << 31)) return attention16g(c, ng);
    if (dtype != VTM_F16 && dtype != VTM_BF16)
        return vtm::fail(VTM_EINVAL, "vtm_attention: dtype must be VTM_F16, VTM_BF16 or VTM_F32");
    return with_head_dim(d, [&](auto dim) {
        constexpr int D = decltype(dim)::value;
        return planned_launch(c, dtype == VTM_F16 ? make_family<__half, D>() : make_family<vtm_bf16, D>());
    });
}

VTM_EXPORT int vtm_attention_kv(const void *q, int64_t ldq, const void *k, int64_t ldk, const void *vt, int64_t ldvt,
                                void *out, int64_t ldo, int dtype, int64_t B, int64_t h, int64_t Mq, int64_t Mqp, int64_t Mk,
                                int64_t Mkp, int64_t d, float scale, int share_groups, void *ws, size_t ws_bytes,
                                vtm_stream_t stream) {
    return attention_any(q, ldq, k, ldk, vt, ldvt, out, ldo, dtype, B, h, Mq, Mqp, Mk, Mkp, d, scale, share_groups, ws,
                         ws_bytes, nullptr, stream);
}

VTM_EXPORT int vtm_attention_kv_bounded(const void *q, int64_t ldq, const void *k, int64_t ldk, const void *vt, int64_t ldvt,
                                        void *out, int64_t ldo, int dtype, int64_t B, int64_t h, int64_t Mq, int64_t Mqp,
                                        int64_t Mk, int64_t Mkp, int64_t d, float scale, const int32_t *q_count, void *ws,
                                        size_t ws_bytes, vtm_stream_t stream) {
    VTM_REQUIRE(q_count, "vtm_attention_kv_bounded: null q_count");
    return attention_any(q, ldq, k, ldk, vt, ldvt, out, ldo, dtype, B, h, Mq, Mqp, Mk, Mkp, d, scale, 1, ws, ws_bytes,
                         q_count, stream);
}

VTM_EXPORT int vtm_attention_kv_shared_bounded(const void *q, int64_t ldq, const void *k, int64_t ldk, const void *vt, int64_t ldvt,
                                               void *out, int64_t ldo, int dtype, int64_t B, int64_t h, int64_t Mq, int64_t Mqp,
                                               int64_t Mk, int64_t Mkp, int64_t d, float scale, int share_groups,
                                               const int32_t *q_count, void *ws, size_t ws_bytes, vtm_stream_t stream) {
    VTM_REQUIRE(q_count, "vtm_attention_kv_shared_bounded: null q_count");
    VTM_REQUIRE(share_groups >= 1 && B % share_groups == 0, "vtm_attention_kv_shared_bounded: B %% share_groups != 0");
    return attention_any(q, ldq, k, ldk, vt, ldvt, out, ldo, dtype, B, h, Mq, Mqp, Mk, Mkp, d, scale, share_groups, ws, ws_bytes,
                         q_count, stream);
}

VTM_EXPORT int vtm_attention_kv_folded(const void *q, int64_t ldq, const void *k, int64_t ldk, const void *vt, int64_t ldvt,
                                       void *out, int64_t ldo, int dtype, int64_t B, int64_t h, int64_t Mq, int64_t Mqp,
                                       int64_t Mk, int64_t Mkp, int64_t d, float scale, const int32_t *q_count,
                                       const int32_t *k_count, const uint32_t *k_bias, int64_t ldkb, void *ws, size_t ws_bytes,
                                       vtm_stream_t stream) {
    const Call c{q, ldq, k, ldk, vt, ldvt, out, ldo, dtype, B, h, Mq, Mqp, Mk, Mkp, scale, 1, ws, ws_bytes,
                 q_count, vtm::as_stream(stream), true, k_count, k_bias, ldkb};
    if (const int e = check_call(c, d, "vtm_attention_kv_folded")) return e;
    if (dtype == VTM_F32) return vtm::fail(VTM_EINVAL, "vtm_attention_kv_folded: fp32 keys are never folded (dtype must be VTM_F16 or VTM_BF16)");
    if (dtype != VTM_F16 && dtype != VTM_BF16) return vtm::fail(VTM_EINVAL, "vtm_attention_kv_folded: dtype must be VTM_F16 or VTM_BF16");
    if (d == 40) return attention16(c);
    return planned_launch(c, dtype == VTM_F16 ? make_family<__half, 8, true>() : make_family<vtm_bf16, 8, true>());
}

VTM_EXPORT int vtm_attention(const void *q, int64_t ldq, const void *k, int64_t ldk, const void *vt,
                             int64_t ldvt, void *out, int64_t ldo, int dtype, int64_t B, int64_t h, int64_t M,
                             int64_t Mp, int64_t d, float scale, int share_groups, void *ws, size_t ws_bytes,
                             vtm_stream_t stream) {
    return vtm_attention_kv(q, ldq, k, ldk, vt, ldvt, out, ldo, dtype, B, h, M, Mp, M, Mp, d, scale, share_groups, ws,
                            ws_bytes, stream);
}
```

### vidtome_amd/csrc/attention_common.h

```cpp
#pragma once
#include "common.h"

namespace vtm_att {

typedef float f32x16 __attribute__((ext_vector_type(16)));
typedef float f32x4 __attribute__((ext_vector_type(4)));
typedef unsigned u32x4 __attribute__((ext_vector_type(4)));
typedef unsigned short u16x2 __attribute__((ext_vector_type(2)));
typedef _Float16 h16x8 __attribute__((ext_vector_type(8)));
typedef _Float16 h16x2 __attribute__((ext_vector_type(2)));
typedef __bf16 b16x8 __attribute__((ext_vector_type(8)));

constexpr int waves_for(int D) { return D <= 48 ? 8 : D <= 96 ? 16 : 4; }
constexpr int QW = 32;
constexpr int KV = 64;
constexpr int VT_STRIDE = KV + 8;
constexpr float DEFER_THR = 8.0f;

constexpr bool pv16_for(int D) { return (D % 32) != 0 && (D + 16) / 16 * 16 < (D + 31) / 32 * 32; }
constexpr int vrows_for(int D) { return pv16_for(D) ? (D + 16) / 16 * 16 : (D + 31) / 32 * 32; }
constexpr int acc_floats(int D) { return pv16_for(D) ? (D + 16) / 16 * 8 : (D + 31) / 32 * 16; }
constexpr int max_floats(int D) { return pv16_for(D) ? 2 : 1; }
constexpr int rec_floats(int D) { return acc_floats(D) + max_floats(D) + 1; }

template <typename T> struct Frag;
template <> struct Frag<__half> {
    using vec = h16x8;
    using elem = _Float16;
    __device__ static f32x16 mfma(vec a, vec b, f32x16 c) {
        return __builtin_amdgcn_mfma_f32_32x32x16_f16(a, b, c, 0, 0, 0);
    }
    __device__ static f32x4 mfma16(vec a, vec b, f32x4 c) {
        return __builtin_amdgcn_mfma_f32_16x16x32_f16(a, b, c, 0, 0, 0);
    }
    static constexpr uint32_t BITS_256 = 0x5C00u;
    __device__ static uint32_t pmax3(uint32_t a, uint32_t b, uint32_t c) {
        uint32_t d;
        asm("v_pk_maximum3_f16 %0, %1, %2, %3" : "=v"(d) : "v"(a), "v"(b), "v"(c));
        return d;
    }
    __device__ static void pack8(vec &dst, const float (&p)[8]) {
#pragma unroll
        for (int i = 0; i < 8; ++i) dst[i] = (_Float16)p[i];
    }
};
template <> struct Frag<vtm_bf16> {
    using vec = b16x8;
    using elem = __bf16;
    __device__ static f32x16 mfma(vec a, vec b, f32x16 c) {
        return __builtin_amdgcn_mfma_f32_32x32x16_bf16(a, b, c, 0, 0, 0);
    }
    __device__ static f32x4 mfma16(vec a, vec b, f32x4 c) {
        return __builtin_amdgcn_mfma_f32_16x16x32_bf16(a, b, c, 0, 0, 0);
    }
    static constexpr uint32_t BITS_256 = 0x4380u;
    __device__ static uint32_t pmax3(uint32_t a, uint32_t b, uint32_t c) {
        const u16x2 m = __builtin_elementwise_max(__builtin_elementwise_max(__builtin_bit_cast(u16x2, a),
                                                                            __builtin_bit_cast(u16x2, b)),
                                                  __builtin_bit_cast(u16x2, c));
        return __builtin_bit_cast(uint32_t, m);
    }
    __device__ static void pack8(vec &dst, const float (&p)[8]) {
#pragma unroll
        for (int i = 0; i < 8; ++i) dst[i] = (__bf16)p[i];
    }
};

__device__ __forceinline__ int64_t item_of(int64_t pos, int64_t nqb, int xcd_groups) {
    if (xcd_groups == 0) return pos;
    const int64_t xcd = pos & 7, slot = pos >> 3;
    return (xcd + 8 * (slot / nqb)) * nqb + slot % nqb;
}

__device__ __forceinline__ void mask_keys(uint4 &v, int valid) {
    uint32_t *w = reinterpret_cast<uint32_t *>(&v);
#pragma unroll
    for (int j = 0; j < 4; ++j) {
        const uint32_t keep = (2 * j + 1 < valid) ? 0xffffffffu : (2 * j < valid) ? 0x0000ffffu : 0u;
        w[j] &= keep;
    }
}

template <typename T, int D>
__device__ __forceinline__ void write_output(const f32x16 (&o)[(D + 31) / 32], float l_run, T *__restrict__ out,
                                             int64_t ldo, int64_t b, int64_t h, int64_t q0, int64_t M, int64_t Mp,
                                             int l31, int hi) {
    using elem = typename Frag<T>::elem;
    constexpr int DV = (D + 31) / 32;
    constexpr bool SPARE = (D % 32) != 0;
    float l_tot;
    if constexpr (SPARE) {
        constexpr int LB = D / 32, LR = D % 32;
        constexpr int LHI = (LR >> 2) & 1, LREG = (LR & 3) + 4 * (LR >> 3);
        l_tot = __shfl(o[LB][LREG], l31 + 32 * LHI, 64);
    } else {
        l_tot = l_run + __shfl_xor(l_run, 32, 64);
    }
    const float inv_l = 1.0f / l_tot;
    const int64_t qi = q0 + l31;
    if (qi < M) {
        T *op = out + (b * Mp + qi) * ldo + h * D;
#pragma unroll
        for (int dv = 0; dv < DV; ++dv)
#pragma unroll
            for (int g = 0; g < 4; ++g) {
                const int d0 = dv * 32 + 8 * g + 4 * hi;
                if (d0 < D) {
                    elem w[4];
#pragma unroll
                    for (int e = 0; e < 4; ++e) w[e] = (elem)(o[dv][g * 4 + e] * inv_l);
                    *reinterpret_cast<uint2 *>(op + d0) = *reinterpret_cast<uint2 *>(w);
                }
            }
    }
}

template <typename T, int D>
__device__ __forceinline__ void write_output16(const f32x4 (&o)[(D + 16) / 16][2], T *__restrict__ out, int64_t ldo,
                                               int64_t b, int64_t h, int64_t q0, int64_t M, int64_t Mp, int lane) {
    using elem = typename Frag<T>::elem;
    constexpr int DV16 = (D + 16) / 16;
    constexpr int LB = D / 16, LG = (D % 16) / 4, LE = D % 4;
    const int l15 = lane & 15, g = lane >> 4;
#pragma unroll
    for (int qh = 0; qh < 2; ++qh) {
        const float inv_l = 1.0f / __shfl(o[LB][qh][LE], 16 * LG + l15, 64);
        const int64_t qi = q0 + 16 * qh + l15;
        if (qi < M) {
            T *op = out + (b * Mp + qi) * ldo + h * D;
#pragma unroll
            for (int dv = 0; dv < DV16; ++dv) {
                const int d0 = dv * 16 + 4 * g;
                if (d0 < D) {
                    elem w[4];
#pragma unroll
                    for (int e = 0; e < 4; ++e) w[e] = (elem)(o[dv][qh][e] * inv_l);
                    *reinterpret_cast<uint2 *>(op + d0) = *reinterpret_cast<uint2 *>(w);
                }
            }
        }
    }
}

}
```

### vidtome_amd/csrc/attention_plan.h

```cpp
#pragma once
#include "attention_common.h"

#include <algorithm>
#include <atomic>
#include <type_traits>

namespace vtm_att {

struct TailPlan {
    int64_t nqb, total, full;
    int nsplit;
    size_t ws_bytes;
    bool split_all;
};

inline TailPlan plan_tail(int64_t B_items, int64_t h, int64_t Mq, int64_t Mk, int64_t QB, int wg_per_cu, size_t rec_bytes,
                          bool bounded) {
    TailPlan p;
    p.nqb = vtm::cdiv(Mq, QB);
    p.total = p.nqb * h * B_items;
    const int64_t slots = (int64_t)vtm::device_cus() * wg_per_cu;
    p.full = p.total / slots * slots;
    const int64_t rem = p.total - p.full, ntiles = vtm::cdiv(Mk, KV);
    p.nsplit = 1;
    p.ws_bytes = 0;
    p.split_all = false;
    if (bounded && p.total >= 2 * slots && ntiles >= 64 && p.total % 8 == 0) {
        p.full = 0;
        p.nsplit = 2;
        p.split_all = true;
        p.ws_bytes = (size_t)p.total * 2 * rec_bytes;
        return p;
    }
    if (p.full > 0 && rem > 0 && rem * 4 <= slots && ntiles >= 32) {
        int64_t ns = slots / rem;
        if (ns > 16) ns = 16;
        if (ns > ntiles / 8) ns = ntiles / 8;
        if (ns >= 2) {
            p.nsplit = (int)ns;
            p.ws_bytes = (size_t)rem * ns * rec_bytes;
        }
    }
    if (p.nsplit == 1) p.full = p.total;
    return p;
}

struct Call {
    const void *q; int64_t ldq; const void *k; int64_t ldk; const void *vt; int64_t ldvt; void *out; int64_t ldo;
    int dtype; int64_t B, h, M, Mp, Mk, Mkp; float scale; int share_groups; void *ws; size_t ws_bytes;
    const int32_t *q_count; hipStream_t s; bool fold; const int32_t *k_count; const uint32_t *k_bias; int64_t ldkb;
    const struct KeySets *sets = nullptr;
};

constexpr int MAX_KEY_SETS = 8;
struct KeySets {
    int n;
    int start[MAX_KEY_SETS], len[MAX_KEY_SETS];
    float w[MAX_KEY_SETS];
};

struct Launch {
    int64_t wgs;
    int64_t split_items;
    int64_t nqb, whole;
    int nsplit;
    float *partial;
    int xcd_groups;
    int64_t split_major;
    const void *plan;
    float scale_log2e;
    int64_t src_batch;
};

struct Family {
    const char *name = "vtm_attention";
    int qb = 0;
    int wg_per_cu = 1;
    size_t rec_bytes = 0;
    int share = 1;
    int key_tile = KV;
    int xcd_min_nqb = 0;
    bool host_split_all = true;
    int64_t ws_devplan_min_tiles = 0;
    hipError_t (*lds_opt_in)() = nullptr;
    void (*main)(const Call &, const Launch &) = nullptr;
    void (*combine)(const Call &, const Launch &) = nullptr;
};

template <typename Fn>
auto with_head_dim(int64_t d, Fn &&fn) {
    switch (d) {
        case 40: return fn(std::integral_constant<int, 40>{});
        case 64: return fn(std::integral_constant<int, 64>{});
        case 80: return fn(std::integral_constant<int, 80>{});
        case 160: return fn(std::integral_constant<int, 160>{});
        case 8: return fn(std::integral_constant<int, 8>{});
        case 16: return fn(std::integral_constant<int, 16>{});
        case 32: return fn(std::integral_constant<int, 32>{});
        case 96: return fn(std::integral_constant<int, 96>{});
        case 128: return fn(std::integral_constant<int, 128>{});
    }
    using R = decltype(fn(std::integral_constant<int, 8>{}));
    if constexpr (std::is_same_v<R, size_t>)
        return size_t(0);
    else
        return vtm::fail(VTM_EINVAL, "vtm_attention: unsupported head dim %lld (have 8,16,32,40,64,80,96,128,160)",
                         (long long)d);
}

Family family16s(int dtype, bool fold);
int attention16(const Call &c);
Family family16g(int dtype, int ng);
int attention16g(const Call &c, int ng);
int attention_f32(const Call &c, int64_t d);

}

namespace {

using namespace vtm_att;

constexpr int PLAN_TIERS = 8;
constexpr int PLAN_MAX_SPLIT = 16;
struct DevTier {
    int wg0, item0, items, nsplit, rec0;
};
struct DevPlan {
    int nqb, ntiers, split_items, pad;
    DevTier tier[PLAN_TIERS];
};
constexpr int64_t plan_tail_wgs(int slots) { return (int64_t)(PLAN_TIERS - 1) * slots; }
constexpr int64_t plan_split_items(int slots) { return slots; }

__global__ void attention16_plan_kernel(const int32_t *__restrict__ q_count, int B, int H, int QB, int slots, int ntiles,
                                        DevPlan *__restrict__ plan) {
    if (threadIdx.x != 0 || blockIdx.x != 0) return;
    int nqb = 1;
    for (int b = 0; b < B; ++b) {
        const int n = (q_count[b] + QB - 1) / QB;
        nqb = n > nqb ? n : nqb;
    }
    const int L = nqb * H * B, S = slots;
    int max_ns = ntiles / 8;
    max_ns = max_ns > PLAN_MAX_SPLIT ? PLAN_MAX_SPLIT : max_ns < 1 ? 1 : max_ns;
    DevPlan p;
    p.nqb = nqb;
    p.pad = 0;
    int nt = 0, wg = 0, item = 0, rec = 0;
    int whole = L - L % S;
    if (max_ns < 2 || (L % S) * 5 >= S * 4 || (L < S && L * 2 > S)) whole = L;
    p.tier[nt++] = DevTier{0, 0, whole, 1, 0};
    wg = item = whole;
    while (item < L && nt < PLAN_TIERS) {
        const int rem = L - item;
        int n = 2;
        while (n < max_ns && S / n > rem) n *= 2;
        if (n > max_ns) n = max_ns;
        int take = S / n < rem ? S / n : rem;
        if (nt == PLAN_TIERS - 1) take = rem;
        p.tier[nt++] = DevTier{wg, item, take, n, rec};
        wg += take * n;
        rec += take * n;
        item += take;
    }
    p.ntiers = nt;
    p.split_items = L - whole;
    for (int i = nt; i < PLAN_TIERS; ++i) p.tier[i] = DevTier{wg, item, 0, 1, rec};
    *plan = p;
}

constexpr size_t DEVPLAN_HEADER = 256;
static_assert(sizeof(DevPlan) <= 256, "the plan lives in the workspace header");
inline size_t devplan_ws_bytes(int slots, size_t rec_bytes) { return DEVPLAN_HEADER + (size_t)plan_tail_wgs(slots) * rec_bytes; }

inline const DevPlan *plan_of(const Launch &g) { return static_cast<const DevPlan *>(g.plan); }

template <auto Kernel, size_t LDS>
hipError_t opt_in_lds() {
    static_assert(LDS > 64 * 1024, "up to 64 KB of dynamic LDS need no opt-in");
    static std::atomic<bool> done[vtm::MAX_DEVICES];
    const int dev = vtm::current_device();
    if (done[dev].load(std::memory_order_acquire)) return hipSuccess;
    const hipError_t e = hipFuncSetAttribute(reinterpret_cast<const void *>(Kernel),
                                             hipFuncAttributeMaxDynamicSharedMemorySize, (int)LDS);
    if (e == hipSuccess) done[dev].store(true, std::memory_order_release);
    return e;
}

inline int planned_launch(const Call &c, const Family &f) {
    if (f.lds_opt_in) {
        const hipError_t e = f.lds_opt_in();
        if (e != hipSuccess) return vtm::fail(VTM_ELAUNCH, "%s: LDS attribute: %s", f.name, hipGetErrorString(e));
    }
    const int64_t B = c.B / f.share;
    const int slots = vtm::device_cus() * f.wg_per_cu;
    const int xcd_pairs = (B * c.h) % 8 == 0 ? (int)(B * c.h / 8) : 0;
    Launch g;
    g.scale_log2e = c.scale * 1.4426950408889634f;
    g.src_batch = c.B / c.share_groups;
    const int64_t nqb_max = vtm::cdiv(c.M, f.qb);
    if (c.q_count != nullptr && c.ws != nullptr && c.ws_bytes >= devplan_ws_bytes(slots, f.rec_bytes) &&
        nqb_max * c.h * B >= 2 * slots) {
        DevPlan *plan = reinterpret_cast<DevPlan *>(c.ws);
        const int64_t total = nqb_max * c.h * B, tail_max = plan_tail_wgs(slots);
// ... 49 lines not shown
```

### vidtome_amd/csrc/ff.hip

```cpp
#include "common.h"

#include <algorithm>
#include <cstdlib>
#include <type_traits>

namespace {

constexpr int FBD = 128;
constexpr int FBS = 256;
constexpr int FBK = 64;
constexpr int THREADS = 256;
constexpr int MAX_TILES_PER_WG = 16;

typedef float f32x16 __attribute__((ext_vector_type(16)));
typedef _Float16 h16x8 __attribute__((ext_vector_type(8)));
typedef __bf16 b16x8 __attribute__((ext_vector_type(8)));
typedef uint32_t u32x4 __attribute__((ext_vector_type(4)));
typedef __attribute__((address_space(3))) void lds_void;

template <typename T> struct Mma;
template <> struct Mma<__half> {
    __device__ static f32x16 run(u32x4 a, u32x4 b, f32x16 c) {
        return __builtin_amdgcn_mfma_f32_32x32x16_f16(__builtin_bit_cast(h16x8, a), __builtin_bit_cast(h16x8, b), c, 0, 0, 0);
    }
    __device__ static uint16_t bits(float v) { return __half_as_ushort(__float2half_rn(v)); }
    __device__ static float round(float v) { return __half2float(__float2half_rn(v)); }
};
template <> struct Mma<vtm_bf16> {
    __device__ static f32x16 run(u32x4 a, u32x4 b, f32x16 c) {
        return __builtin_amdgcn_mfma_f32_32x32x16_bf16(__builtin_bit_cast(b16x8, a), __builtin_bit_cast(b16x8, b), c, 0, 0, 0);
    }
    __device__ static uint16_t bits(float v) { return __bfloat16_as_ushort(__float2bfloat16(v)); }
    __device__ static float round(float v) { return __bfloat162float(__float2bfloat16(v)); }
};

__device__ __forceinline__ float gelu_erf(float g) {
    const float x = __builtin_fabsf(g) * 0.70710678118654752440f;
    const float t = __builtin_amdgcn_rcpf(__builtin_fmaf(0.3275911f, x, 1.0f));
    float p = __builtin_fmaf(1.061405429f, t, -1.453152027f);
    p = __builtin_fmaf(p, t, 1.421413741f);
    p = __builtin_fmaf(p, t, -0.284496736f);
    p = __builtin_fmaf(p, t, 0.254829592f);
    const float e = p * t * __builtin_amdgcn_exp2f(-x * x * 1.4426950408889634f);
    return 0.5f * g * (g < 0.0f ? e : 2.0f - e);
}

enum { EPI_GEGLU = 0, EPI_ROWS = 1 };

struct Epi {
    const float *bias;
    void *out;
    int64_t out_rows_pad;
    int64_t ldo;
    const void *resid;
    int64_t n;
    int64_t N;
    int64_t nbias;
};

template <typename T, int EPI>
__global__ __launch_bounds__(THREADS, 2) void panel_gemm_kernel(
    const uint4 *__restrict__ ah, const uint4 *__restrict__ bh, int64_t Ns_pad, int64_t Nd_pad, int64_t C_pad,
    int ns_tiles, int nd_tiles, int nsplit, int tiles_per_split, int total_src_tiles, int patch_tiles, Epi E) {
    __shared__ __attribute__((aligned(16))) uint4 sA[2][8 * FBD];
    __shared__ float sBias[MAX_TILES_PER_WG * FBD];
    __shared__ __attribute__((aligned(16))) uint16_t sOut[EPI == EPI_ROWS ? 4 * 32 * (FBD + 8) : 8];

    const int tid = threadIdx.x, lane = tid & 63;
    const int wave = __builtin_amdgcn_readfirstlane(tid >> 6);
    const int l31 = lane & 31, kh = lane >> 5;

    const int xcd = blockIdx.x & 7, slot = blockIdx.x >> 3;
    const int per_group = patch_tiles * nsplit;
    const int grp = (slot / per_group) * 8 + xcd;
    const int q = slot % per_group;
    const int stg = grp * patch_tiles + q % patch_tiles;
    const int split = q / patch_tiles;
    if (stg >= total_src_tiles) return;
    const int st_ = stg % ns_tiles;
    const int jt0 = split * tiles_per_split;
    const int jt1 = min(jt0 + tiles_per_split, nd_tiles);
    if (jt0 >= jt1) return;

    const int KT = (int)(C_pad / FBK);
    const int steps = (jt1 - jt0) * KT;
    const uint4 *srch = ah, *dsth = bh;
    const int64_t srow0 = (int64_t)st_ * FBS + wave * 64;

    __shared__ Epi sE;
    if (tid == 0) sE = E;
    {
        const int cnt = (jt1 - jt0) * FBD;
        const float *bsrc = E.bias != nullptr ? E.bias + (int64_t)jt0 * FBD : nullptr;
#pragma unroll
        for (int k = 0; k < MAX_TILES_PER_WG * FBD / THREADS; ++k) {
            const int i = tid + k * THREADS;
            if (i < cnt) sBias[i] = (bsrc != nullptr && (int64_t)jt0 * FBD + i < E.nbias) ? bsrc[i] : 0.0f;
        }
    }

    constexpr int NB = 2, PG = 2;
    const uint32_t voff_b = (uint32_t)(kh * Ns_pad + srow0 + l31) * 16u;
    const int64_t bgroup = 2 * Ns_pad;
    u32x4 rb[4][2];
    auto await_b = [&](auto count_tag, u32x4 (&r)[2]) {
        constexpr int N = decltype(count_tag)::value;
        asm volatile("s_waitcnt vmcnt(%2)" : "+v"(r[0]), "+v"(r[1]) : "n"(N));
    };
    const uint32_t voff_a = (uint32_t)lane * 16u;
    f32x16 acc[4][2];

    const char *const src_b = reinterpret_cast<const char *>(srch);
    const int64_t kstep_b = bgroup * 16;
    const int64_t panel_b = Nd_pad * 16;
    const int64_t tile_dk = 8 * panel_b;
    const int64_t tile_dwrap = FBD * 16 - (int64_t)(KT - 1) * tile_dk;
    const uint32_t lds_a = (uint32_t)reinterpret_cast<uintptr_t>((lds_void *)&sA[0][wave * 2 * FBD]);
    auto load_b1 = [&](const char *pb_, int ks, int sb, u32x4 &dst) {
        const char *ph = pb_ + ks * kstep_b;
        if (sb == 0) asm volatile("global_load_dwordx4 %0, %1, %2" : "=v"(dst) : "v"(voff_b), "s"(ph));
        else asm volatile("global_load_dwordx4 %0, %1, %2 offset:512" : "=v"(dst) : "v"(voff_b), "s"(ph));
    };
    auto load_a_piece = [&](const char *pa_, int buf_, int t) {
        const char *g = pa_ + (t >> 1) * panel_b + (t & 1) * 1024;
        const uint32_t lds_off = lds_a + (uint32_t)buf_ * (uint32_t)sizeof(sA[0]) + (uint32_t)t * 1024u;
        asm volatile("s_mov_b32 m0, %0\n\ts_nop 0\n\tglobal_load_lds_dwordx4 %1, %2" : : "s"(lds_off), "v"(voff_a), "s"(g) : "memory");
    };
    const uint32_t *const dummy_rows = reinterpret_cast<const uint32_t *>(bh);
    uint32_t am[2] = {0u, 0u};
    const uint32_t voff_m = 0u;
    u32x4 fa[2][4];
    const char *pa1 = reinterpret_cast<const char *>(dsth + (int64_t)wave * 2 * Nd_pad + (int64_t)jt0 * FBD);
    const char *pb = src_b;
    {
        load_a_piece(pa1, 0, 0);
        load_a_piece(pa1, 0, 1);
        load_a_piece(pa1, 0, 2);
        load_a_piece(pa1, 0, 3);
        asm volatile("s_waitcnt vmcnt(0)" ::: "memory");
        __syncthreads();
        if (steps > 1) pa1 += KT == 1 ? tile_dwrap : tile_dk;
        load_b1(pb, 0, 0, rb[0][0]);
        load_b1(pb, 0, 1, rb[0][1]);
        load_b1(pb, 1, 0, rb[1][0]);
        load_b1(pb, 1, 1, rb[1][1]);
        load_a_piece(pa1, 1, 0);
        load_a_piece(pa1, 1, 1);
#pragma unroll
        for (int ib = 0; ib < 4; ++ib) fa[0][ib] = __builtin_bit_cast(u32x4, sA[0][kh * FBD + ib * 32 + l31]);
    }

    auto epilogue = [&](int jt) {
        const float *bt = sBias + (jt - jt0) * FBD;
        if constexpr (EPI == EPI_GEGLU) {
            uint16_t *outp = static_cast<uint16_t *>(sE.out);
            const int64_t out_rows_pad = sE.out_rows_pad;
#pragma unroll
            for (int sb = 0; sb < 2; ++sb) {
                const int64_t tok = srow0 + sb * 32 + l31;
#pragma unroll
                for (int ibp = 0; ibp < 2; ++ibp)
#pragma unroll
                    for (int qq = 0; qq < 4; ++qq) {
                        uint16_t w4[4];
#pragma unroll
                        for (int e = 0; e < 4; ++e) {
                            const int r = 4 * qq + e, row = 32 * ibp + e + 8 * qq + 4 * kh;
                            const float bv = bt[row], bg = bt[64 + row];
                            const float v = Mma<T>::round(acc[ibp][sb][r] + bv);
                            const float g = Mma<T>::round(acc[ibp + 2][sb][r] + bg);
                            w4[e] = Mma<T>::bits(v * Mma<T>::round(gelu_erf(g)));
                        }
                        const int64_t g2 = (int64_t)jt * 8 + ibp * 4 + qq;
                        *reinterpret_cast<uint2 *>(outp + (g2 * out_rows_pad + tok) * 8 + 4 * kh) = *reinterpret_cast<const uint2 *>(w4);
                    }
            }
        } else {
            constexpr int SO = FBD + 8;
            uint16_t *my = sOut + wave * 32 * SO;
            uint16_t *outp = static_cast<uint16_t *>(sE.out);
            const uint16_t *resp = static_cast<const uint16_t *>(sE.resid);
            const int64_t ldo = sE.ldo, n_tok = sE.n, n_ch = sE.N;
#pragma unroll
            for (int sb = 0; sb < 2; ++sb) {
#pragma unroll
                for (int ib = 0; ib < 4; ++ib)
#pragma unroll
                    for (int qq = 0; qq < 4; ++qq) {
                        float f4[4];
#pragma unroll
                        for (int e = 0; e < 4; ++e) {
                            const int row = 32 * ib + e + 8 * qq + 4 * kh;
                            f4[e] = acc[ib][sb][4 * qq + e] + bt[row];
                        }
                        uint16_t w4[4];
#pragma unroll
                        for (int e = 0; e < 4; ++e) w4[e] = Mma<T>::bits(f4[e]);
                        *reinterpret_cast<uint2 *>(my + l31 * SO + 32 * ib + 8 * qq + 4 * kh) = *reinterpret_cast<const uint2 *>(w4);
                    }
                __builtin_amdgcn_wave_barrier();
                constexpr int PR = FBD / 8;
#pragma unroll
                for (int it = 0; it < 32 * PR / 64; ++it) {
                    const int p = lane + 64 * it;
                    const int row = p / PR, c8 = (p % PR) * 8;
                    const int64_t tok = srow0 + sb * 32 + row, ch = (int64_t)jt * FBD + c8;
                    if (tok < n_tok && ch < n_ch) {
                        uint4 v = *reinterpret_cast<const uint4 *>(my + row * SO + c8);
                        if (resp != nullptr) {
                            const uint4 rv = *reinterpret_cast<const uint4 *>(resp + tok * ldo + ch);
                            const T *a8 = reinterpret_cast<const T *>(&v), *r8 = reinterpret_cast<const T *>(&rv);
                            uint4 o;
                            uint16_t *o8 = reinterpret_cast<uint16_t *>(&o);
#pragma unroll
                            for (int e = 0; e < 8; ++e) o8[e] = Mma<T>::bits(vtm::to_f32(a8[e]) + vtm::to_f32(r8[e]));
                            v = o;
                        }
                        *reinterpret_cast<uint4 *>(outp + tok * ldo + ch) = v;
                    }
                }
                __builtin_amdgcn_wave_barrier();
            }
        }
    };

    int kt = 0, jt = jt0;
    for (int st = 0; st < steps; ++st) {
        const int buf = st & 1;
        const bool wrap = kt + 1 == KT;
        const int kt1 = wrap ? 0 : kt + 1;
        const bool wrap1 = kt1 + 1 == KT;
        const char *const pbn = st + 1 < steps ? (wrap ? src_b : pb + 4 * kstep_b) : pb;
        const char *const pa2 = st + 2 < steps ? pa1 + (wrap1 ? tile_dwrap : tile_dk) : pa1;
        auto group = [&](auto s_tag, auto first_tag) {
            constexpr int s = decltype(s_tag)::value;
            constexpr bool FIRST = decltype(first_tag)::value;
            constexpr int COUNT = s == 1 ? NB + 2 * PG : s == 2 ? NB + PG + 2 : NB + 2;
            if constexpr (s != 0) await_b(std::integral_constant<int, COUNT>{}, rb[s]);
            if constexpr (s == 1) asm volatile("" : : "v"(am[0]), "v"(am[1]));
            u32x4 (&fh)[4] = fa[s & 1];
            u32x4 (&fn)[4] = fa[(s + 1) & 1];
#pragma unroll
            for (int j = 0; j < 8; ++j) {
                const int sb = j >> 2, ib = j & 3;
                f32x16 c = acc[ib][sb];
                if constexpr (FIRST) {
#pragma unroll
                    for (int r = 0; r < 16; ++r) c[r] = 0.0f;
                }
                acc[ib][sb] = Mma<T>::run(fh[ib], rb[s][sb], c);
                __builtin_amdgcn_sched_barrier(0);
                if (j < 4) {
                    if constexpr (s < 3) fn[j] = __builtin_bit_cast(u32x4, sA[buf][((s + 1) * 2 + kh) * FBD + j * 32 + l31]);
                    else fn[j] = __builtin_bit_cast(u32x4, sA[buf ^ 1][kh * FBD + j * 32 + l31]);
                } else if (j < 6) {
                    if constexpr (s < 2) load_b1(pb, s + 2, j - 4, rb[s + 2][j - 4]);
                    else load_b1(pbn, s - 2, j - 4, rb[s - 2][j - 4]);
                } else {
                    if constexpr (s == 0) load_a_piece(pa1, buf ^ 1, j - 4);
                    if constexpr (s == 3) load_a_piece(pa2, buf, j - 6);
                    if constexpr (s == 1)
                        asm volatile("global_load_dword %0, %1, %2" : "=v"(am[j - 6]) : "v"(voff_m), "s"(dummy_rows));
                }
                __builtin_amdgcn_sched_barrier(0);
            }
        };
        await_b(std::integral_constant<int, NB + PG>{}, rb[0]);
        if (kt == 0) group(std::integral_constant<int, 0>{}, std::true_type{});
        else group(std::integral_constant<int, 0>{}, std::false_type{});
        group(std::integral_constant<int, 1>{}, std::false_type{});
        group(std::integral_constant<int, 2>{}, std::false_type{});
        asm volatile("s_waitcnt vmcnt(%0) lgkmcnt(0)" ::"n"(2 * NB + 2) : "memory");
        __syncthreads();
        group(std::integral_constant<int, 3>{}, std::false_type{});
        if (wrap) {
            epilogue(jt);
            ++jt;
        }
        kt = kt1;
        pb = pbn;
        pa1 = pa2;
    }
    asm volatile("s_waitcnt vmcnt(0)" ::: "memory");
}

template <typename T>
__global__ __launch_bounds__(256) void to_panels_kernel(const T *__restrict__ x, int64_t rows, int64_t C, int64_t rows_pad,
                                                        const int32_t *__restrict__ order, uint4 *__restrict__ out) {
    const int64_t G = C / 8;
    const int64_t i = (int64_t)blockIdx.x * blockDim.x + threadIdx.x;
    if (i >= rows_pad * G) return;
    const int64_t g = i % G, r = i / G;
    uint4 v = make_uint4(0, 0, 0, 0);
    if (r < rows) {
        const int64_t src = order ? order[r] : r;
        if (src >= 0) v = *reinterpret_cast<const uint4 *>(x + src * C + g * 8);
    }
    out[g * rows_pad + r] = v;
}

template <typename T>
__global__ __launch_bounds__(256) void gather_panels_kernel(const T *__restrict__ x0, int64_t P0, const T *__restrict__ x1,
                                                            int64_t P1, int64_t B, int64_t C, const int32_t *__restrict__ map,
                                                            int64_t map_ld, const int32_t *__restrict__ map2, int64_t n,
                                                            int64_t rows_per_sample, int64_t stride, uint4 *__restrict__ out) {
    const int64_t G = C / 8;
    const int64_t i = (int64_t)blockIdx.x * blockDim.x + threadIdx.x;
    if (i >= B * rows_per_sample * G) return;
    const int64_t g = i % G, r = (i / G) % rows_per_sample, b = i / (G * rows_per_sample);
    uint4 v = make_uint4(0, 0, 0, 0);
    if (r < n) {
        int64_t p = map2 ? map2[b * n + r] : r;
        if (map) p = map[b * map_ld + p];
        const T *row = p < P0 ? x0 + (b * P0 + p) * C : x1 + (b * P1 + (p - P0)) * C;
        v = *reinterpret_cast<const uint4 *>(row + g * 8);
    }
    out[g * stride + b * rows_per_sample + r] = v;
}

inline int64_t pad256(int64_t n) { return vtm::cdiv(n, FBS) * FBS; }

template <typename T, int EPI>
int launch_panel_gemm(const void *tok, int64_t n, int64_t n_pad, const void *w, int64_t Nw, int64_t Nw_pad, int64_t K,
                      const Epi &E, hipStream_t s) {
    VTM_REQUIRE(2 * n_pad * 16 < (1ll << 32), "panel GEMM: %lld token panel rows exceed the 32-bit fragment offset",
                (long long)n_pad);
    const int ns_tiles = (int)vtm::cdiv(n, FBS), nd_tiles = (int)vtm::cdiv(Nw, FBD);
    const int total_src_tiles = ns_tiles;
    const int max_patch = (int64_t)16 * FBS * K * 2 <= (3 << 20) ? 16 : 8;
    const int tiles_per_xcd = (int)vtm::cdiv(total_src_tiles, 8);
    const int patches_per_xcd = (int)vtm::cdiv(tiles_per_xcd, max_patch);
    const int patch_tiles = (int)vtm::cdiv(tiles_per_xcd, patches_per_xcd);
    const int ngroups = (int)vtm::cdiv(total_src_tiles, patch_tiles);
    const int64_t slots = (int64_t)vtm::device_cus() * 2;
    int64_t nsplit = vtm::cdiv(3 * slots, (int64_t)ns_tiles);
    nsplit = std::max<int64_t>(nsplit, vtm::cdiv(nd_tiles, MAX_TILES_PER_WG));
    nsplit = std::min<int64_t>(std::max<int64_t>(nsplit, 1), nd_tiles);
    const int tiles_per_split = (int)vtm::cdiv(nd_tiles, nsplit);
    nsplit = vtm::cdiv(nd_tiles, tiles_per_split);
    const int64_t grid = (int64_t)8 * vtm::cdiv(ngroups, 8) * patch_tiles * nsplit;
    if (grid >= (1ll << 31)) return vtm::fail(VTM_EINVAL, "vtm_ff: grid too large");
    hipLaunchKernelGGL((panel_gemm_kernel<T, EPI>), dim3((unsigned)grid), dim3(THREADS), 0, s, (const uint4 *)tok,
                       (const uint4 *)w, n_pad, Nw_pad, K, ns_tiles, nd_tiles, (int)nsplit, tiles_per_split, total_src_tiles,
                       patch_tiles, E);
    return vtm::launch_status("vtm_ff");
}

}

VTM_EXPORT int64_t vtm_panel_rows(int64_t n) { return n <= 0 ? 0 : pad256(n); }

VTM_EXPORT int vtm_to_panels(const void *x, int dtype, int64_t rows, int64_t C, const int32_t *order, void *out,
                             int64_t rows_pad, vtm_stream_t stream) {
    VTM_REQUIRE(x && out && rows > 0 && C > 0 && C % 8 == 0, "vtm_to_panels: bad arguments");
    VTM_REQUIRE(rows_pad >= rows && rows_pad % FBS == 0, "vtm_to_panels: rows_pad must be vtm_panel_rows(rows) or more");
    VTM_REQUIRE(dtype == VTM_F16 || dtype == VTM_BF16, "vtm_to_panels: dtype must be VTM_F16 or VTM_BF16");
    const int64_t total = rows_pad * (C / 8);
    hipLaunchKernelGGL(to_panels_kernel<__half>, dim3((unsigned)vtm::cdiv(total, 256)), dim3(256), 0, vtm::as_stream(stream),
                       (const __half *)x, rows, C, rows_pad, order, (uint4 *)out);
    return vtm::launch_status("vtm_to_panels");
}

VTM_EXPORT int vtm_gather_panels(const void *x0, int64_t P0, const void *x1, int64_t P1, int dtype, int64_t B, int64_t C,
                                 const int32_t *map, int64_t map_ld, const int32_t *map2, int64_t n, void *out,
                                 int64_t rows_per_sample, vtm_stream_t stream) {
    VTM_REQUIRE(x0 && out && B > 0 && C > 0 && C % 8 == 0 && n > 0, "vtm_gather_panels: bad arguments");
    VTM_REQUIRE(P1 == 0 || x1, "vtm_gather_panels: x1 is null but P1 > 0");
    VTM_REQUIRE(map || map2 || n <= P0 + P1, "vtm_gather_panels: identity rows must lie inside the pool");
    VTM_REQUIRE(!map || map_ld > 0, "vtm_gather_panels: map_ld");
    VTM_REQUIRE(rows_per_sample >= n && rows_per_sample % FBS == 0, "vtm_gather_panels: rows_per_sample must be a multiple of 256 >= n");
    VTM_REQUIRE(dtype == VTM_F16 || dtype == VTM_BF16, "vtm_gather_panels: dtype must be VTM_F16 or VTM_BF16");
    const int64_t total = B * rows_per_sample * (C / 8);
    hipLaunchKernelGGL(gather_panels_kernel<__half>, dim3((unsigned)vtm::cdiv(total, 256)), dim3(256), 0, vtm::as_stream(stream),
                       (const __half *)x0, P0, (const __half *)x1, P1, B, C, map, map_ld, map2, n, rows_per_sample,
                       B * rows_per_sample, (uint4 *)out);
    return vtm::launch_status("vtm_gather_panels");
}

VTM_EXPORT int vtm_ff_geglu(const void *x_panels, int64_t n, int64_t n_pad, const void *w1_panels, int64_t D, int64_t w_rows_pad,
                            int64_t K, const float *bias, int dtype, void *out_panels, vtm_stream_t stream) {
    VTM_REQUIRE(x_panels && w1_panels && out_panels, "vtm_ff_geglu: null pointer");
    VTM_REQUIRE(n > 0 && n_pad >= n && n_pad % FBS == 0, "vtm_ff_geglu: token rows must be padded to 256");
    VTM_REQUIRE(D > 0 && D % 64 == 0 && w_rows_pad >= 2 * D && w_rows_pad % FBS == 0, "vtm_ff_geglu: D %% 64, packed weight rows padded to 256");
    VTM_REQUIRE(K > 0 && K % FBK == 0, "vtm_ff_geglu: K must be a multiple of 64");
    Epi E{bias, out_panels, n_pad, 0, nullptr, n, D, 2 * D};
    hipStream_t s = vtm::as_stream(stream);
    if (dtype == VTM_F16) return launch_panel_gemm<__half, EPI_GEGLU>(x_panels, n, n_pad, w1_panels, 2 * D, w_rows_pad, K, E, s);
    if (dtype == VTM_BF16) return launch_panel_gemm<vtm_bf16, EPI_GEGLU>(x_panels, n, n_pad, w1_panels, 2 * D, w_rows_pad, K, E, s);
    return vtm::fail(VTM_EINVAL, "vtm_ff_geglu: dtype must be VTM_F16 or VTM_BF16");
}

VTM_EXPORT int vtm_linear_panels(const void *x_panels, int64_t n, int64_t n_pad, const void *w_panels, int64_t N, int64_t w_rows_pad,
                                 int64_t K, const float *bias, const void *resid, int dtype, void *out, int64_t ldo,
                                 vtm_stream_t stream) {
    VTM_REQUIRE(x_panels && w_panels && out, "vtm_linear_panels: null pointer");
    VTM_REQUIRE(n > 0 && n_pad >= vtm::cdiv(n, FBS) * FBS, "vtm_linear_panels: token rows must be padded to 256");
    VTM_REQUIRE(N > 0 && N % 8 == 0 && w_rows_pad >= vtm::cdiv(N, FBD) * FBD, "vtm_linear_panels: N %% 8, weight rows padded to 128");
    VTM_REQUIRE(K > 0 && K % FBK == 0, "vtm_linear_panels: K must be a multiple of 64");
    VTM_REQUIRE(ldo >= N && ldo % 8 == 0 && (reinterpret_cast<uintptr_t>(out) & 15) == 0 &&
                    (reinterpret_cast<uintptr_t>(resid) & 15) == 0, "vtm_linear_panels: output rows must be 16-byte aligned");
    Epi E{bias, out, 0, ldo, resid, n, N, N};
    hipStream_t s = vtm::as_stream(stream);
    if (dtype == VTM_F16) return launch_panel_gemm<__half, EPI_ROWS>(x_panels, n, n_pad, w_panels, N, w_rows_pad, K, E, s);
    if (dtype == VTM_BF16) return launch_panel_gemm<vtm_bf16, EPI_ROWS>(x_panels, n, n_pad, w_panels, N, w_rows_pad, K, E, s);
    return vtm::fail(VTM_EINVAL, "vtm_linear_panels: dtype must be VTM_F16 or VTM_BF16");
}
```

### vidtome_amd/patch.py

```python
from __future__ import annotations

import math
import os
from typing import Any, Callable, Dict, Optional, Tuple, Type

import torch
import torch.nn.functional as F

from . import _lib, ip_adapter, lora, merge
from .utils import init_generator, isinstance_str, join_frame, split_frame

LIVE_QUERIES = os.environ.get("VIDTOME_LIVE_QUERIES", "1") != "0"
COMPACT_QUERIES = os.environ.get("VIDTOME_COMPACT_QUERIES", "1") != "0"


class MergePlan:

    __slots__ = ("fsize", "L", "M", "gather_map", "_inv", "_inv_parts", "_merged", "levels", "global_level", "local_chunk",
                 "x_joined", "anchors_in", "q_rows", "inv_q", "q_count", "pad_to", "fold_args", "_key_fold", "aligned")

    def __init__(self):
        self.levels = []
        self.global_level = None
        self.local_chunk = None
# ... 253 lines not shown
def _pnp_share_groups(attn: torch.nn.Module) -> int:
    sched = getattr(attn, "injection_schedule", None)
    if sched is not None:
        t = getattr(attn, "t", None)
        if t is not None and (t in sched or t == 1000):
            n = _pnp_num_inputs(attn)
            if n is None:
                raise RuntimeError("PnP injection is registered on attn1 but num_inputs is unknown")
            return n
    return 1


def _built_here(device):
    if not torch.cuda.is_available() or torch.device(device).type != "cuda":
        return None
    st = torch.cuda.current_stream(device)
    ev = torch.cuda.Event()
    ev.record(st)
    return ev, st.cuda_stream


def _built_before(mark, device) -> None:
    if mark is not None:
        cur = torch.cuda.current_stream(device)
        if cur.cuda_stream != mark[1]:
            cur.wait_event(mark[0])


def _linear(m: torch.nn.Module, dtype=None, device=None):
    p = lora.linear_params(m, dtype, device)
    if p is None:
        raise RuntimeError(f"vidtome_amd: {type(m).__name__} is not a projection the fused path can read")
    return p


def _fused_weights(attn: torch.nn.Module, dtype, device):
    cache = attn.__dict__.get("_vtm_wcache")
    wq, bq, kq = _linear(attn.to_q)
    wk, bk, kk = _linear(attn.to_k)
    key = (kq, kk, dtype, device)
    if cache is None or cache[0] != key:
        wqk = torch.cat([wq, wk], dim=0).to(device=device, dtype=dtype).contiguous()
        bqk = None
        if bq is not None or bk is not None:
            zq = bq if bq is not None else torch.zeros_like(wq[:, 0])
            zk = bk if bk is not None else torch.zeros_like(wk[:, 0])
            bqk = torch.cat([zq, zk]).to(device=device, dtype=dtype)
        cache = (key, wqk, bqk, _built_here(device))
        attn.__dict__["_vtm_wcache"] = cache
    _built_before(cache[3], device)
    return cache[1], cache[2]


_HEAD_DIMS = (8, 16, 32, 40, 64, 80, 96, 128, 160)
_PLAIN_PROCESSORS = ("AttnProcessor", "AttnProcessor2_0", "XFormersAttnProcessor")
_warned = set()


def _warn_once(key: str, msg: str) -> None:
    if key not in _warned:
        _warned.add(key)
        import warnings
        warnings.warn(msg, stacklevel=3)


def _readable_linear(m) -> bool:
    return lora.recognise(m) is not None


def _out_linear(attn: torch.nn.Module):
    to_out = attn.to_out
    return to_out[0] if isinstance(to_out, (torch.nn.ModuleList, torch.nn.Sequential, list, tuple)) else to_out


def fused_attention_ok(attn: torch.nn.Module, x: torch.Tensor, self_attn: bool = True,
                       processors=_PLAIN_PROCESSORS) -> bool:
    if not (x.is_cuda and x.dim() == 3 and x.dtype in (torch.float16, torch.bfloat16, torch.float32)):
        return False
    if not all(hasattr(attn, a) for a in ("to_q", "to_k", "to_v", "to_out", "heads")):
        return False
    if not all(_readable_linear(m) for m in (attn.to_q, attn.to_k, attn.to_v, _out_linear(attn))):
        return False
    C = x.shape[-1]
    if lora.base_linear(attn.to_q).out_features != C or C % attn.heads or (C // attn.heads) not in _HEAD_DIMS:
        return False
    if any(getattr(attn, a, None) is not None for a in ("group_norm", "spatial_norm", "norm_cross", "norm_q", "norm_k")):
        return False
    if getattr(attn, "rescale_output_factor", 1.0) != 1.0 or getattr(attn, "residual_connection", False):
        return False
    proc = getattr(attn, "processor", None)
    if proc is not None and type(proc).__name__ not in processors:
        return False
    if "forward" in attn.__dict__ and not (self_attn and _pnp_num_inputs(attn) is not None):
        return False
    to_out = attn.to_out
    if attn.training and isinstance(to_out, (torch.nn.ModuleList, torch.nn.Sequential)) and len(to_out) > 1 \
            and getattr(to_out[1], "p", 0.0) != 0.0:
        return False
    return True


PROJ_MODE = os.environ.get("VIDTOME_PROJ", "auto")
FUSED_PROJ = PROJ_MODE != "blas"


def _proj_dtypes_ok(attn: torch.nn.Module, dtype) -> bool:
    for lin in (attn.to_q, attn.to_k, attn.to_v, _out_linear(attn)):
        if not _linear_dtype_ok(lin, dtype):
            return False
    return True


def _linear_dtype_ok(lin: torch.nn.Module, dtype) -> bool:
    base = lora.base_linear(lin)
    return base.weight.dtype == dtype and (base.bias is None or base.bias.dtype == dtype)


def _has_bias(lin: torch.nn.Module) -> bool:
    return lora.linear_params(lin)[1] is not None


def fused_projections_ok(attn: torch.nn.Module, x: torch.Tensor) -> bool:
    if not FUSED_PROJ or x.dtype not in (torch.float16, torch.bfloat16) or x.shape[-1] % 32 \
            or not _proj_dtypes_ok(attn, x.dtype):
        return False
    return PROJ_MODE == "rows" or (PROJ_MODE == "auto" and x.shape[-1] <= 320)


def panel_projections_ok(attn: torch.nn.Module, x: torch.Tensor) -> bool:
    return (PROJ_MODE in ("auto", "panels") and x.dtype in (torch.float16, torch.bfloat16) and x.shape[-1] % 64 == 0
            and _proj_dtypes_ok(attn, x.dtype) and not _has_bias(attn.to_v))


def _panel_weight(lin: torch.nn.Module):
    w, b, key = _linear(lin)
    return _packed(lin, "rows", key, w.device, lambda: (_lib.to_panels(w.detach().contiguous()),
                                                       None if b is None else b.detach().float().contiguous()))


def self_attention_panels(attn: torch.nn.Module, x0: torch.Tensor, x1: Optional[torch.Tensor], rows: Optional[torch.Tensor],
                          q_rows: Optional[torch.Tensor] = None, q_count: Optional[torch.Tensor] = None) -> torch.Tensor:
    B, _, C = x0.shape
    M = x0.shape[1] if rows is None else rows.shape[1]
    heads = attn.heads
    scale = getattr(attn, "scale", None) or (C // heads) ** -0.5
    share = _pnp_share_groups(attn)
    Mpad = _lib.panel_rows(M)
    xp = _lib.gather_panels(x0, x1, rows, None, M)
    wq, bq = _panel_weight(attn.to_q)
    wk, bk = _panel_weight(attn.to_k)
    wv, _ = _panel_weight(attn.to_v)
    k_op = _lib.linear_panels(xp, B * Mpad, wk, C, bk).view(B, Mpad, C)
    vt = torch.empty((B, C, Mpad), dtype=x0.dtype, device=x0.device)
    M8 = (M + 7) // 8 * 8
    for b in range(B):
        _lib.linear_panels(wv, C, xp[:, b * Mpad:(b + 1) * Mpad], M8, None, out=vt[b])
    if q_rows is None:
        q_op = _lib.linear_panels(xp, B * Mpad, wq, C, bq).view(B, Mpad, C)
        o = _lib.attention(q_op, k_op, vt, heads, M, scale, share)
        Mq, Mqpad = M, Mpad
    else:
        Mq = q_rows.shape[1]
        Mqpad = _lib.panel_rows(Mq)
        qp = _lib.gather_panels(x0, x1, rows, q_rows, Mq)
        q_op = _lib.linear_panels(qp, B * Mqpad, wq, C, bq).view(B, Mqpad, C)
        o = _lib.attention_kv(q_op, k_op, vt, heads, Mq, M, scale, q_count=q_count, share_groups=share)
    wo, bo = _panel_weight(_out_linear(attn))
    op = _lib.to_panels(o.view(B * Mqpad, C))
    return _lib.linear_panels(op, B * Mqpad, wo, C, bo).view(B, Mqpad, C)


def unmerged_site(block: torch.nn.Module, x: torch.Tensor) -> bool:
    info = block._tome_info
    if info["size"] is None:
        return False
    downsample = int(math.ceil(math.sqrt((info["size"][0] * info["size"][1]) // x.shape[1])))
    return downsample > info["args"]["max_downsample"]


def unmerged_self_attention_ok(block: torch.nn.Module, x: torch.Tensor) -> bool:
    norm, attn = block.norm1, block.attn1
    return (x.is_cuda and x.dim() == 3 and x.shape[1] % 8 == 0 and type(norm) is torch.nn.LayerNorm and len(norm.normalized_shape) == 1
            and norm.normalized_shape[0] == x.shape[-1] and (norm.weight is None or norm.weight.dtype == x.dtype)
            and (norm.bias is None or norm.bias.dtype == x.dtype) and fused_attention_ok(attn, x)
            and panel_projections_ok(attn, x) and not fused_projections_ok(attn, x) and _pnp_share_groups(attn) == 1
            and unmerged_site(block, x))


def unmerged_self_attention_residual(block: torch.nn.Module, hidden_states: torch.Tensor) -> torch.Tensor:
    attn, norm = block.attn1, block.norm1
    BF, N, C = hidden_states.shape
    heads = attn.heads
    scale = getattr(attn, "scale", None) or (C // heads) ** -0.5
    hs = hidden_states.contiguous()
    n = BF * N

    qkv_params = [_linear(m) for m in (attn.to_q, attn.to_k, attn.to_v)]

    def pack_qkv():
        w = torch.cat([p[0] for p in qkv_params], dim=0).detach().contiguous()
        bs = [p[1] for p in qkv_params]
        b = None if all(x is None for x in bs) else torch.cat(
            [torch.zeros(C, device=w.device) if x is None else x.detach().float() for x in bs]).contiguous()
        return _lib.to_panels(w), b
    wqkv, bqkv = _packed(attn, "qkv", tuple(p[2] for p in qkv_params), qkv_params[0][0].device, pack_qkv)
    xp = _lib.layernorm_panels(hs, norm.weight, norm.bias, norm.eps)
    qkv = _lib.linear_panels(xp, n, wqkv, 3 * C, bqkv).view(BF, N, 3 * C)
    vt = _lib.transpose_cols(qkv, 2 * C, C)
    o = _lib.attention(qkv[:, :, :C], qkv[:, :, C:2 * C], vt, heads, N, scale, 1)
    wo, bo = _panel_weight(_out_linear(attn))
    op = _lib.to_panels(o.view(n, C))
    return _lib.linear_panels(op, n, wo, C, bo, resid=hs.view(n, C)).view(BF, N, C)


def self_attention_segment(block: torch.nn.Module, hidden_states: torch.Tensor, encoder_hidden_states=None,
                           attention_mask=None, cross_attention_kwargs=None) -> torch.Tensor:
    if (encoder_hidden_states is None or not block.only_cross_attention) and attention_mask is None \
            and not cross_attention_kwargs and unmerged_self_attention_ok(block, hidden_states):
        return unmerged_self_attention_residual(block, hidden_states)
    return patched_self_attention_segment(block, hidden_states, layer_norm(block.norm1, hidden_states),
                                          encoder_hidden_states, attention_mask, cross_attention_kwargs, None)


def _weight(m: torch.nn.Module, dtype) -> torch.Tensor:
    w = _linear(m)[0]
    return w if (w.dtype == dtype and w.is_contiguous()) else w.to(dtype).contiguous()


def _bias(m: torch.nn.Module, dtype) -> Optional[torch.Tensor]:
    b = _linear(m)[1]
    return None if b is None else b.to(dtype)


def self_attention_rows(attn: torch.nn.Module, x0: torch.Tensor, x1: Optional[torch.Tensor],
                        rows: Optional[torch.Tensor], q_rows: Optional[torch.Tensor] = None,
                        q_count: Optional[torch.Tensor] = None, plan: Optional["MergePlan"] = None) -> torch.Tensor:
    B, _, C = x0.shape
    M = x0.shape[1] if rows is None else rows.shape[1]
    Mp = (M + 7) // 8 * 8
    heads = attn.heads
    scale = getattr(attn, "scale", None) or (C // heads) ** -0.5
    share = _pnp_share_groups(attn)
    dt = x0.dtype
    wqk, bqk = _fused_weights(attn, dt, x0.device)
    bv = _bias(attn.to_v, dt)
    fold = None
    if plan is not None and rows is not None and share == 1 and (C // heads) in (8, 40):
        fold = plan.key_fold(dt)
    if fold is not None:
        key_sel, k_bias, k_count = fold
        vt = _lib.linear_rows(x0, x1, rows, key_sel, M, _weight(attn.to_v, dt), bv, transposed=True)
        k_op = _lib.linear_rows(x0, x1, rows, key_sel, M, wqk[C:], None if bqk is None else bqk[C:])
        Mq = M if q_rows is None else q_rows.shape[1]
        q_op = _lib.linear_rows(x0, x1, rows, q_rows, Mq, wqk[:C], None if bqk is None else bqk[:C])
        o = _lib.attention_kv(q_op, k_op, vt, heads, Mq, M, scale, q_count=q_count, k_fold=(k_count, k_bias))
        to_out = _out_linear(attn)
        return _lib.linear_rows(o, None, None, None, Mq, _weight(to_out, dt), _bias(to_out, dt))
    vt = _lib.linear_rows(x0, x1, rows, None, M, _weight(attn.to_v, dt), bv, transposed=True)
    if q_rows is None:
        qk = _lib.linear_rows(x0, x1, rows, None, M, wqk, bqk)
        o = _lib.attention(qk[:, :, :C], qk[:, :, C:], vt, heads, M, scale, share)
        Mq = M
    else:
        Mq = q_rows.shape[1]
        k_op = _lib.linear_rows(x0, x1, rows, None, M, wqk[C:], None if bqk is None else bqk[C:])
        q_op = _lib.linear_rows(x0, x1, rows, q_rows, Mq, wqk[:C], None if bqk is None else bqk[:C])
        o = _lib.attention_kv(q_op, k_op, vt, heads, Mq, M, scale, q_count=q_count, share_groups=share)
    to_out = _out_linear(attn)
    return _lib.linear_rows(o, None, None, None, Mq, _weight(to_out, dt), _bias(to_out, dt))


def _fp32_projections(block: torch.nn.Module) -> bool:
    return getattr(block, "fp32_projections", False) is True


def f32_projections_ok(attn: torch.nn.Module, x: torch.Tensor) -> bool:
    return x.is_cuda and x.dtype == torch.float32 and x.shape[-1] % 8 == 0 and _proj_dtypes_ok(attn, torch.float32)


def self_attention_f32(attn: torch.nn.Module, x0: torch.Tensor, x1: Optional[torch.Tensor], rows: Optional[torch.Tensor],
                       q_rows: Optional[torch.Tensor] = None, q_count: Optional[torch.Tensor] = None,
                       fp32_core: bool = False) -> torch.Tensor:
    B, _, C = x0.shape
    M = x0.shape[1] if rows is None else rows.shape[1]
    heads = attn.heads
    scale = getattr(attn, "scale", None) or (C // heads) ** -0.5
    share = _pnp_share_groups(attn)
    f32 = torch.float32
    core = f32 if fp32_core else torch.float16
    wqk, bqk = _fused_weights(attn, f32, x0.device)
    vt = _lib.linear_f32(x0, x1, rows, None, M, _weight(attn.to_v, f32), _bias(attn.to_v, f32), out_dtype=core,
                         transposed=True)
    if q_rows is None:
        qk = _lib.linear_f32(x0, x1, rows, None, M, wqk, bqk, out_dtype=core)
        o = _lib.attention(qk[:, :, :C], qk[:, :, C:], vt, heads, M, scale, share)
        Mq = M
    else:
        Mq = q_rows.shape[1]
        k_op = _lib.linear_f32(x0, x1, rows, None, M, wqk[C:], None if bqk is None else bqk[C:], out_dtype=core)
        q_op = _lib.linear_f32(x0, x1, rows, q_rows, Mq, wqk[:C], None if bqk is None else bqk[:C], out_dtype=core)
        o = _lib.attention_kv(q_op, k_op, vt, heads, Mq, M, scale, q_count=q_count, share_groups=share)
    to_out = _out_linear(attn)
    return _lib.linear_f32(o.float(), None, None, None, Mq, _weight(to_out, f32), _bias(to_out, f32))


def self_attention(attn: torch.nn.Module, x: torch.Tensor, M: Optional[int] = None,
                   q_rows: Optional[torch.Tensor] = None, q_count: Optional[torch.Tensor] = None,
                   fp32_core: bool = False) -> torch.Tensor:
    B, Mp, C = x.shape
    M = Mp if M is None else M
    heads = attn.heads
    scale = getattr(attn, "scale", None) or (C // heads) ** -0.5
    share = _pnp_share_groups(attn)
    if x.shape[1] % 8:
        pad = 8 - x.shape[1] % 8
        x = F.pad(x, (0, 0, 0, pad))
        Mp = x.shape[1]
    core = x.dtype
    if x.dtype != torch.float32 and PROJ_MODE != "blas":
        _warn_once("lib-proj", f"vidtome_amd: attn1 projections of a {x.dtype} model run as library GEMMs (C = {C}: the "
                               "hand-written projection kernels take C % 32 == 0 with all four projection weights in the "
                               "tokens' dtype and no bias on to_v at C > 320)")
    if x.dtype == torch.float32 and not fp32_core:
        core = torch.float16
        _warn_once("fp32-core", "vidtome_amd: fp32 model -- the self-attention core (QK^T, softmax, PV) runs on the "
                                "fp16 MFMA with fp32 accumulation; projections, matching and merging stay fp32")
    wqk, bqk = _fused_weights(attn, x.dtype, x.device)
    if q_rows is None:
        qk = F.linear(x, wqk, bqk).to(core)
        q_op, k_op = qk[:, :, :C], qk[:, :, C:]
    else:
        xq = _lib.gather_rows(x, None, q_rows, pad_to=8)
        q_op = F.linear(xq, wqk[:C], None if bqk is None else bqk[:C]).to(core)
        k_op = F.linear(x, wqk[C:], None if bqk is None else bqk[C:]).to(core)
    wv, bv, _ = _linear(attn.to_v, x.dtype)
    if B <= 4:
        vt = torch.empty((B, C, Mp), dtype=x.dtype, device=x.device)
        for bi in range(B):
            torch.mm(wv, x[bi].t(), out=vt[bi])
    else:
        vt = torch.matmul(wv, x.transpose(1, 2))
    if bv is not None:
        vt = vt + bv[None, :, None]
    vt = vt.to(core)
    if q_rows is None:
        o = _lib.attention(q_op, k_op, vt, heads, M, scale, share)
    else:
        o = _lib.attention_kv(q_op, k_op, vt, heads, q_rows.shape[1], M, scale, q_count=q_count, share_groups=share)
    o = o.to(x.dtype)
    wo, bo, _ = _linear(_out_linear(attn), o.dtype)
    return F.linear(o, wo, bo)


def _cross_kv(to_k: torch.nn.Module, to_v: torch.nn.Module, enc: torch.Tensor, C: int, panels: bool = True):
    B, Mkp, D = enc.shape
    dt = enc.dtype
    if panels and D % 64 == 0 and lora.base_linear(to_k).weight.dtype == dt and lora.base_linear(to_v).weight.dtype == dt:
        ep = _lib.to_panels(enc.reshape(B * Mkp, D))
        wk, bk = _panel_weight(to_k)
        wv, bv = _panel_weight(to_v)
        k = _lib.linear_panels(ep, B * Mkp, wk, C, bk).view(B, Mkp, C)
        vt = _lib.linear_panels(ep, B * Mkp, wv, C, bv).view(B, Mkp, C).transpose(1, 2).contiguous()
    else:
        if panels:
            _warn_once("lib-cross-kv", f"vidtome_amd: attn2's k / v projections run as library GEMMs (conditioning width "
                                       f"{D} is not a multiple of 64, or to_k / to_v are not of the tokens' dtype)")
        k = _apply_linear(to_k, enc)
        vt = _apply_linear(to_v, enc).transpose(1, 2).contiguous()
    return k, vt


def _pad_keys(enc: torch.Tensor, dt) -> torch.Tensor:
    enc = enc.to(dt)
    pad = -enc.shape[1] % 8
    return F.pad(enc, (0, 0, 0, pad)) if pad else enc


def _ip_key_sets(attn: torch.nn.Module, ip: "ip_adapter.Call", dt, C: int, panels: bool):
    sets, active, _ = ip_adapter.key_sets(ip.text.shape[1], [im.shape[1] for im in ip.images], ip.scales)
    k, vt = _cross_kv(attn.to_k, attn.to_v, _pad_keys(ip.text, dt), C, panels)
    if active:
        parts = [(k, vt)] + [_cross_kv(ip.k_proj[a], ip.v_proj[a], _pad_keys(ip.images[a], dt), C, panels) for a in active]
        k = torch.cat([p[0] for p in parts], dim=1)
        vt = torch.cat([p[1] for p in parts], dim=2)
    return k, vt, sets


def norm_cross_attention_residual(norm: torch.nn.Module, attn: torch.nn.Module, hidden_states: torch.Tensor,
                                  encoder_hidden_states: torch.Tensor, ip: Optional["ip_adapter.Call"] = None
                                  ) -> torch.Tensor:
    B, N, C = hidden_states.shape
    heads = attn.heads
    scale = getattr(attn, "scale", None) or (C // heads) ** -0.5
    dt = hidden_states.dtype
    hs = hidden_states.contiguous()
    n = B * N
    wq, bq = _panel_weight(attn.to_q)
    wo, bo = _panel_weight(_out_linear(attn))
    xp = _lib.layernorm_panels(hs, norm.weight, norm.bias, norm.eps)
    q = _lib.linear_panels(xp, n, wq, C, bq).view(B, N, C)
    if N % 8:
        raise RuntimeError("norm_cross_attention_residual: token count must be a multiple of 8")
    if ip is None:
        Mk = encoder_hidden_states.shape[1]
        k, vt = _cross_kv(attn.to_k, attn.to_v, _pad_keys(encoder_hidden_states, dt), C)
        o = _lib.attention_kv(q, k, vt, heads, N, Mk, scale)
    else:
        k, vt, sets = _ip_key_sets(attn, ip, dt, C, True)
        o = _lib.attention_kv_sets(q, k, vt, heads, N, sets, scale)
    op = _lib.to_panels(o.view(n, C))
    return _lib.linear_panels(op, n, wo, C, bo, resid=hs.view(n, C)).view(B, N, C)


def _apply_linear(m: torch.nn.Module, t: torch.Tensor) -> torch.Tensor:
    w, b, _ = _linear(m, t.dtype)
    return F.linear(t, w, b)


def fused_cross_ok(norm: torch.nn.Module, attn: torch.nn.Module, x: torch.Tensor, encoder_hidden_states,
                   attention_mask, kwargs, processors=_PLAIN_PROCESSORS) -> bool:
    return (FF_MODE == "panels" and isinstance(encoder_hidden_states, torch.Tensor) and attention_mask is None and not kwargs
            and encoder_hidden_states.dim() == 3 and x.dim() == 3 and x.is_cuda and x.dtype in (torch.float16, torch.bfloat16)
            and type(norm) is torch.nn.LayerNorm and len(norm.normalized_shape) == 1
            and norm.normalized_shape[0] == x.shape[-1] and x.shape[-1] % 64 == 0 and x.shape[1] % 8 == 0
            and (norm.weight is None or norm.weight.dtype == x.dtype) and (norm.bias is None or norm.bias.dtype == x.dtype)
            and _proj_dtypes_ok(attn, x.dtype) and fused_attention_ok(attn, x, self_attn=False, processors=processors))


def ip_cross_call(attn: torch.nn.Module, x: torch.Tensor, encoder_hidden_states, attention_mask, kwargs,
                  norm: Optional[torch.nn.Module] = None) -> Optional["ip_adapter.Call"]:
    if not ip_adapter.is_ip_processor(attn):
        return None
    ip = ip_adapter.recognise(attn, x, encoder_hidden_states, attention_mask, kwargs)
    if ip is None:
        return None
    if norm is not None:
        return ip if fused_cross_ok(norm, attn, x, ip.text, None, None, ip_adapter.PROCESSORS) else None
    return ip if fused_attention_ok(attn, x, self_attn=False, processors=ip_adapter.PROCESSORS) else None


def _f32_layernorm_ok(norm: torch.nn.Module, x: torch.Tensor) -> bool:
    return (type(norm) is torch.nn.LayerNorm and len(norm.normalized_shape) == 1 and norm.normalized_shape[0] == x.shape[-1]
            and x.shape[-1] % 8 == 0 and x.shape[-1] <= 2048
            and (norm.weight is None or norm.weight.dtype == torch.float32)
            and (norm.bias is None or norm.bias.dtype == torch.float32))


def f32_cross_ok(block: torch.nn.Module, norm: torch.nn.Module, attn: torch.nn.Module, x: torch.Tensor,
                 encoder_hidden_states, attention_mask, kwargs) -> bool:
    return (_fp32_projections(block) and isinstance(encoder_hidden_states, torch.Tensor) and attention_mask is None
            and not kwargs and encoder_hidden_states.dim() == 3 and x.dim() == 3 and x.is_cuda and x.dtype == torch.float32
            and encoder_hidden_states.shape[0] == x.shape[0] and encoder_hidden_states.shape[-1] % 8 == 0
            and _f32_layernorm_ok(norm, x) and _proj_dtypes_ok(attn, torch.float32)
            and fused_attention_ok(attn, x, self_attn=False))


def norm_cross_attention_f32(norm: torch.nn.Module, attn: torch.nn.Module, hidden_states: torch.Tensor,
                             encoder_hidden_states: torch.Tensor) -> torch.Tensor:
    B, N, C = hidden_states.shape
    heads = attn.heads
    scale = getattr(attn, "scale", None) or (C // heads) ** -0.5
    f32 = torch.float32
    hs = hidden_states.contiguous()
    enc = encoder_hidden_states.to(f32).contiguous()
    Mk = enc.shape[1]
    xn = _lib.layernorm(hs, norm.weight, norm.bias, norm.eps)
    q = _lib.linear_f32(xn, None, None, None, N, _weight(attn.to_q, f32), _bias(attn.to_q, f32))
    k = _lib.linear_f32(enc, None, None, None, Mk, _weight(attn.to_k, f32), _bias(attn.to_k, f32))
    vt = _lib.linear_f32(enc, None, None, None, Mk, _weight(attn.to_v, f32), _bias(attn.to_v, f32),
                         transposed=True)
    o = _lib.attention_kv(q, k, vt, heads, N, Mk, scale)
    to_out = _out_linear(attn)
    return _lib.linear_f32(o, None, None, None, N, _weight(to_out, f32), _bias(to_out, f32), epilogue="resid", resid=hs,
                           out=torch.empty_like(hs))


def cross_attention(attn: torch.nn.Module, x: torch.Tensor, encoder_hidden_states: Optional[torch.Tensor],
                    attention_mask=None, **kwargs) -> torch.Tensor:
    plain = (isinstance(encoder_hidden_states, torch.Tensor) and attention_mask is None and not kwargs
             and encoder_hidden_states.dim() == 3 and x.dtype in (torch.float16, torch.bfloat16)
             and fused_attention_ok(attn, x, self_attn=False))
    if not plain:
        ip = ip_cross_call(attn, x, encoder_hidden_states, attention_mask, kwargs)
        if ip is None:
            return attn(x, encoder_hidden_states=encoder_hidden_states, attention_mask=attention_mask, **kwargs)
        B, N, C = x.shape
        scale = getattr(attn, "scale", None) or (C // attn.heads) ** -0.5
        xq = F.pad(x, (0, 0, 0, -N % 8)) if N % 8 else x
        k, vt, sets = _ip_key_sets(attn, ip, x.dtype, C, False)
        o = _lib.attention_kv_sets(_apply_linear(attn.to_q, xq), k, vt, attn.heads, N, sets, scale)
        return _apply_linear(_out_linear(attn), o)[:, :N]
    B, N, C = x.shape
    enc = encoder_hidden_states.to(x.dtype)
    Mk = enc.shape[1]
    heads = attn.heads
    scale = getattr(attn, "scale", None) or (C // heads) ** -0.5
    Np, Mkp = (N + 7) // 8 * 8, (Mk + 7) // 8 * 8
    if Np != N:
        x = F.pad(x, (0, 0, 0, Np - N))
    if Mkp != Mk:
        enc = F.pad(enc, (0, 0, 0, Mkp - Mk))
    q = _apply_linear(attn.to_q, x)
    k = _apply_linear(attn.to_k, enc)
    vt = _apply_linear(attn.to_v, enc).transpose(1, 2).contiguous()
    o = _lib.attention_kv(q, k, vt, heads, N, Mk, scale)
    return _apply_linear(_out_linear(attn), o)[:, :N]


FF_MODE = os.environ.get("VIDTOME_FF", "panels")


def _packed(module: torch.nn.Module, name: str, tag, dev, build):
    cache = module.__dict__.setdefault("_vtm_packed", {})
    hit = cache.get(name)
    if hit is None or hit[0] != tag:
        hit = cache[name] = (tag, build(), _built_here(dev))
    _built_before(hit[2], dev)
    return hit[1]


def _geglu_ff(ff: torch.nn.Module):
    net = getattr(ff, "net", None)
    if (net is not None and len(net) == 3 and net[0].__class__.__name__ == "GEGLU" and hasattr(net[0], "proj")
            and _readable_linear(net[0].proj) and _readable_linear(net[2])
            and (not ff.training or getattr(net[1], "p", 0.0) == 0.0)):
        return net[0].proj, net[2]
    return None


def fused_ff_ok(norm: torch.nn.Module, ff: torch.nn.Module, x: torch.Tensor) -> bool:
    if FF_MODE != "panels" or not x.is_cuda or x.dtype not in (torch.float16, torch.bfloat16):
        return False
    lin = _geglu_ff(ff)
    if lin is None or type(norm) is not torch.nn.LayerNorm or len(norm.normalized_shape) != 1:
        return False
    proj, out = (lora.base_linear(m) for m in lin)
    C = x.shape[-1]
    D = proj.out_features // 2
    return (norm.normalized_shape[0] == C and C % 64 == 0 and C <= 2048 and proj.in_features == C and D % 64 == 0
            and out.in_features == D and out.out_features == C and proj.weight.dtype == x.dtype
            and out.weight.dtype == x.dtype and (norm.weight is None or norm.weight.dtype == x.dtype)
            and (norm.bias is None or norm.bias.dtype == x.dtype))


def norm_feed_forward_residual(norm: torch.nn.Module, ff: torch.nn.Module, hidden_states: torch.Tensor) -> torch.Tensor:
    proj, out = _geglu_ff(ff)
    C = hidden_states.shape[-1]
    pw, pb, pkey = _linear(proj)
    D = pw.shape[0] // 2

    def pack_w1():
        t = torch.arange(D // 64, device=pw.device)[:, None] * 64 + torch.arange(64, device=pw.device)[None, :]
        order = torch.cat([t, t + D], dim=1).reshape(-1).to(torch.int32)
        b = None if pb is None else pb.detach().float()[order.long()].contiguous()
        return _lib.to_panels(pw.detach().contiguous(), order), b

    w1, b1 = _packed(proj, "geglu", pkey, pw.device, pack_w1)
    w2, b2 = _panel_weight(out)
    hs = hidden_states.contiguous()
    n = hs.numel() // C
    xp = _lib.layernorm_panels(hs, norm.weight, norm.bias, norm.eps)
    hp = _lib.ff_geglu(xp, n, w1, D, b1)
    return _lib.linear_panels(hp, n, w2, C, b2, resid=hs.view(n, C)).view(hidden_states.shape)
# ... 297 lines not shown
```

Baseline: 22.71.

## Write attention output directly in panel layout and batch per-sample V projections

Adds a panel-layout epilogue to the attention main and combine kernels, so self and cross attention write the (C/8, rows, 8) panel tensor that the output projection consumes. This removes the separate to_panels pass and its round trip through memory. It also replaces the per-sample Python loop of V-transposed linear_panels calls with one batched GEMM launch over a second grid dimension. The cost is extra template instantiations and zero-fill work for padding rows in the panel writer, and the panel path only covers head dims 64 and 160.

Result: no change. 22.84, median of 2 (+0.6%).

```diff
diff --git a/include/vidtome_hip.h b/include/vidtome_hip.h
--- a/include/vidtome_hip.h
+++ b/include/vidtome_hip.h
@@ -142,6 +142,11 @@
                                     const int32_t *q_count, void *ws, size_t ws_bytes, vtm_stream_t stream);
 size_t vtm_attention_kv_bounded_ws_bytes(int64_t B, int64_t h, int64_t Mq, int64_t Mk, int64_t d);
 
+int vtm_attention_kv_panels(const void *q, int64_t ldq, const void *k, int64_t ldk, const void *vt, int64_t ldvt,
+                            void *out_panels, int64_t panel_rows, int dtype, int64_t B, int64_t h, int64_t Mq, int64_t Mqp,
+                            int64_t Mk, int64_t Mkp, int64_t d, float scale, int share_groups, const int32_t *q_count,
+                            void *ws, size_t ws_bytes, vtm_stream_t stream);
+
 int vtm_transpose_cols(const void *x, int64_t ldx, int dtype, int64_t BF, int64_t N, int64_t C, void *out, int64_t ldo,
                        vtm_stream_t stream);
 
@@ -172,6 +177,9 @@
 int vtm_linear_panels(const void *x_panels, int64_t n, int64_t n_pad, const void *w_panels, int64_t N, int64_t w_rows_pad,
                       int64_t K, const float *bias, const void *resid, int dtype, void *out, int64_t ldo,
                       vtm_stream_t stream);
+int vtm_linear_panels_batched(const void *x_panels, int64_t n, int64_t n_pad, const void *w_panels, int64_t N,
+                              int64_t w_rows_pad, int64_t K, const float *bias, int dtype, void *out, int64_t ldo,
+                              int64_t nbatch, int64_t w_batch_rows, int64_t out_batch, vtm_stream_t stream);
 
 int vtm_cfg_ddim(const void *x, const void *eps_uncond, const void *eps_cond, int dtype, int64_t n,
                  float guidance, float a, float b, float c, float d, void *eps_out, void *x_out,
diff --git a/vidtome_amd/_lib.py b/vidtome_amd/_lib.py
--- a/vidtome_amd/_lib.py
+++ b/vidtome_amd/_lib.py
@@ -65,6 +65,8 @@
                                   _f32, _vp, _vp, ctypes.c_size_t, _vp], _int),
     "vtm_attention_kv_shared_bounded": ([_vp, _i64, _vp, _i64, _vp, _i64, _vp, _i64, _int, _i64, _i64, _i64, _i64, _i64, _i64, _i64,
                                          _f32, _int, _vp, _vp, ctypes.c_size_t, _vp], _int),
+    "vtm_attention_kv_panels": ([_vp, _i64, _vp, _i64, _vp, _i64, _vp, _i64, _int, _i64, _i64, _i64, _i64, _i64, _i64, _i64,
+                                 _f32, _int, _vp, _vp, ctypes.c_size_t, _vp], _int),
     "vtm_attention_kv_bounded_ws_bytes": ([_i64, _i64, _i64, _i64, _i64], ctypes.c_size_t),
     "vtm_anchor_maps": ([_vp, _i64, _i64, _vp, _i64, _i64, _i64, _i64, _i64, _vp, _i64, _vp, _vp, _vp, _vp], _int),
     "vtm_transpose_cols": ([_vp, _i64, _int, _i64, _i64, _i64, _vp, _i64, _vp], _int),
@@ -80,6 +82,7 @@
     "vtm_gather_panels": ([_vp, _i64, _vp, _i64, _int, _i64, _i64, _vp, _i64, _vp, _i64, _vp, _i64, _vp], _int),
     "vtm_ff_geglu": ([_vp, _i64, _i64, _vp, _i64, _i64, _i64, _vp, _int, _vp, _vp], _int),
     "vtm_linear_panels": ([_vp, _i64, _i64, _vp, _i64, _i64, _i64, _vp, _vp, _int, _vp, _i64, _vp], _int),
+    "vtm_linear_panels_batched": ([_vp, _i64, _i64, _vp, _i64, _i64, _i64, _vp, _int, _vp, _i64, _i64, _i64, _i64, _vp], _int),
     "vtm_cfg_ddim": ([_vp, _vp, _vp, _int, _i64, _f32, _f32, _f32, _f32, _f32, _vp, _vp, _vp], _int),
     "vtm_layernorm": ([_vp, _vp, _vp, _int, _i64, _i64, _f32, _vp, _vp], _int),
     "vtm_geglu": ([_vp, _int, _i64, _i64, _vp, _vp], _int),
@@ -581,6 +584,43 @@
     return out
 
 
+PANEL_HEAD_DIMS = (64, 80, 160)
+PANEL_SITE_HEAD_DIMS = (64, 160)
+
+
+@_on_device
+def attention_kv_panels(q: torch.Tensor, k: torch.Tensor, vt: torch.Tensor, heads: int, Mq: int, Mk: int, scale: float,
+                        q_count: Optional[torch.Tensor] = None, share_groups: int = 1,
+                        out: Optional[torch.Tensor] = None) -> torch.Tensor:
+    B, Mqp, C = q.shape
+    Mkp = k.shape[1]
+    d = C // heads
+    if d not in PANEL_HEAD_DIMS or q.dtype not in (torch.float16, torch.bfloat16):
+        raise RuntimeError(f"attention_kv_panels: fp16 / bf16 heads of {PANEL_HEAD_DIMS} channels, got {q.dtype}, d = {d}")
+    if q.stride(2) != 1 or k.stride(2) != 1 or vt.stride(2) != 1:
+        raise RuntimeError("attention operands must be contiguous along their last axis")
+    if q.stride(0) != Mqp * q.stride(1) or k.stride(0) != Mkp * k.stride(1) or vt.stride(0) != C * vt.stride(1):
+        raise RuntimeError("attention operands must have dense batch strides")
+    if q_count is not None and (q_count.dtype != torch.int32 or q_count.numel() != B or not q_count.is_cuda):
+        raise RuntimeError("attention_kv_panels: q_count must be a (B,) int32 device tensor")
+    if out is None:
+        shape = (C // 8, panel_rows(B * Mqp), 8)
+        out = torch.zeros(shape, dtype=q.dtype, device=q.device) if q_count is not None else \
+            torch.empty(shape, dtype=q.dtype, device=q.device)
+    elif out.shape[0] != C // 8 or out.shape[1] < B * Mqp or out.shape[2] != 8 or not out.is_contiguous() or out.dtype != q.dtype:
+        raise RuntimeError("attention_kv_panels: out must be a contiguous (C / 8, >= B * Mqp, 8) panel tensor")
+    ws, nb = _attention_ws(B, heads, Mq, Mk, d, q.device)
+    if q_count is not None and SPLIT_ALL_BOUNDED:
+        nb2 = int(lib().vtm_attention_kv_bounded_ws_bytes(B, heads, Mq, Mk, d))
+        if nb2 > nb:
+            ws, nb = _workspace("attention", nb2, q.device), nb2
+    _check(lib().vtm_attention_kv_panels(q.data_ptr(), q.stride(1), k.data_ptr(), k.stride(1), vt.data_ptr(), vt.stride(1),
+                                         out.data_ptr(), out.shape[1], dtype_code(q), B, heads, Mq, Mqp, Mk, Mkp, d,
+                                         float(scale), int(share_groups), _ptr(q_count), _ptr(ws), nb, _stream()),
+           "vtm_attention_kv_panels")
+    return out
+
+
 MAX_KEY_SETS = 8
 
 
@@ -810,6 +850,23 @@
 
 
 @_on_device
+def linear_panels_batched(w_panels: torch.Tensor, n: int, x_panels: torch.Tensor, B: int, rows: int, batch_rows: int,
+                          out: torch.Tensor) -> torch.Tensor:
+    K = x_panels.shape[0] * 8
+    if x_panels.stride(2) != 1 or x_panels.stride(1) != 8 or w_panels.stride(2) != 1 or w_panels.stride(1) != 8 \
+            or w_panels.shape[0] * 8 != K:
+        raise RuntimeError("linear_panels_batched: operands must be (K / 8, rows, 8) panel tensors (or row ranges of one)")
+    if out.dim() != 3 or out.shape[0] != B or out.shape[1] != n or out.shape[2] < rows or out.stride(2) != 1 \
+            or out.stride(0) != n * out.stride(1) or out.dtype != x_panels.dtype:
+        raise RuntimeError("linear_panels_batched: out must be a dense (B, n, ldo >= rows) tensor of the operands' dtype")
+    _check(lib().vtm_linear_panels_batched(_ptr(w_panels), n, w_panels.stride(0) // 8, _ptr(x_panels), rows,
+                                           x_panels.stride(0) // 8, K, None, dtype_code(x_panels), out.data_ptr(),
+                                           out.stride(1), B, batch_rows, out.stride(0), _stream()),
+           "vtm_linear_panels_batched")
+    return out
+
+
+@_on_device
 def gather_panels(x0: torch.Tensor, x1: Optional[torch.Tensor], rows: Optional[torch.Tensor], rows2: Optional[torch.Tensor],
                   n: int) -> torch.Tensor:
     _req(x0, "x0")
diff --git a/vidtome_amd/csrc/attention.hip b/vidtome_amd/csrc/attention.hip
--- a/vidtome_amd/csrc/attention.hip
+++ b/vidtome_amd/csrc/attention.hip
@@ -5,10 +5,11 @@
 
 namespace {
 
-template <typename T, int D>
+template <typename T, int D, bool PANEL = false>
 __global__ __launch_bounds__(waves_for(D) * 64) void attention_combine_kernel(
     const float *__restrict__ partial, T *__restrict__ out, int64_t ldo, int64_t H, int64_t M, int64_t Mp, int64_t nqb,
-    int64_t id0, int nsplit, int xcd_groups, const int32_t *__restrict__ q_count, const DevPlan *__restrict__ dev_plan) {
+    int64_t id0, int nsplit, int xcd_groups, const int32_t *__restrict__ q_count, const DevPlan *__restrict__ dev_plan,
+    int64_t nsamples) {
     constexpr int WAVES = waves_for(D), NT = WAVES * 64, QB = WAVES * QW, DV = (D + 31) / 32;
     constexpr bool PV16 = pv16_for(D);
     constexpr int NA = acc_floats(D), NM = max_floats(D), REC = rec_floats(D);
@@ -63,14 +64,18 @@
         f32x16 o[DV];
 #pragma unroll
         for (int r = 0; r < NA; ++r) o[r >> 4][r & 15] = acc[r];
-        write_output<T, D>(o, l, out, ldo, b, h, q0, M, Mp, l31, hi);
-    }
-}
-
-template <typename T, int D>
+        if constexpr (PANEL)
+            write_output_panels<T, D>(o, l, out, ldo, b, h, q0, M, Mp, b + 1 == nsamples ? ldo - b * Mp : Mp,
+                                      lin % nqb == nqb - 1, QB, l31, hi);
+        else
+            write_output<T, D>(o, l, out, ldo, b, h, q0, M, Mp, l31, hi);
+    }
+}
+
+template <typename T, int D, bool PANEL = false>
 __global__ __launch_bounds__(waves_for(D) * 64) void attention_combine_parts_kernel(
     const float *__restrict__ partial, T *__restrict__ out, int64_t ldo, int64_t H, int64_t M, int64_t Mp, int64_t nqb,
-    int64_t id0, int nsplit, int xcd_groups, const int32_t *__restrict__ q_count) {
+    int64_t id0, int nsplit, int xcd_groups, const int32_t *__restrict__ q_count, int64_t nsamples) {
     using elem = typename Frag<T>::elem;
     static_assert(!pv16_for(D), "32-row O^T layout");
     constexpr int WAVES = waves_for(D), NT = WAVES * 64, QB = WAVES * QW;
@@ -104,6 +109,31 @@
     const float l_tot = SPARE ? __shfl(den, l31 + 32 * LHI, 64) : den + __shfl_xor(den, 32, 64);
     const float inv_l = 1.0f / l_tot;
     const int64_t qi = q0 + l31;
+    if constexpr (PANEL) {
+        static_assert(D % 16 == 0, "a part holds whole panels");
+        const int64_t prows = ldo, row_end = b + 1 == nsamples ? prows - b * Mp : Mp;
+        const int dv = r0 >> 4, g0 = (r0 & 15) >> 2;
+        if (dv * 32 + 8 * g0 >= D) return;
+        uint2 w2[2];
+#pragma unroll
+        for (int gi = 0; gi < 2; ++gi) {
+            elem w4[4];
+#pragma unroll
+            for (int e = 0; e < 4; ++e) w4[e] = (elem)(acc[gi * 4 + e] * inv_l);
+            w2[gi] = *reinterpret_cast<uint2 *>(w4);
+        }
+        const uint2 keep = hi ? w2[1] : w2[0], give = hi ? w2[0] : w2[1];
+        uint2 got;
+        got.x = __shfl_xor(give.x, 32, 64);
+        got.y = __shfl_xor(give.y, 32, 64);
+        uint4 v = hi ? make_uint4(got.x, got.y, keep.x, keep.y) : make_uint4(keep.x, keep.y, got.x, got.y);
+        if (qi >= M) v = make_uint4(0, 0, 0, 0);
+        uint4 *op = reinterpret_cast<uint4 *>(out) + (h * (D / 8) + dv * 4 + g0 + hi) * prows + b * Mp;
+        if (qi < row_end) op[qi] = v;
+        if (lin % nqb == nqb - 1)
+            for (int64_t r = qi + QB; r < row_end; r += QB) op[r] = make_uint4(0, 0, 0, 0);
+        return;
+    }
     if (qi < M) {
         T *op = out + (b * Mp + qi) * ldo + h * D;
         const int dv = r0 >> 4, g0 = (r0 & 15) >> 2;
@@ -120,14 +150,14 @@
     }
 }
 
-template <typename T, int D, bool FOLD>
+template <typename T, int D, bool FOLD, bool PANEL = false>
 __global__ __launch_bounds__(waves_for(D) * 64, (D <= 48 ? 4 : D <= 96 ? 4 : 1)) void attention_kernel(
     const T *__restrict__ q, int64_t ldq, const T *__restrict__ k, int64_t ldk,
     const T *__restrict__ vt, int64_t ldvt, T *__restrict__ out, int64_t ldo, int64_t H,
     int64_t M, int64_t Mp, int64_t Mk_arg, int64_t Mkp, float scale_log2e, int64_t src_batch, int64_t nqb, int64_t nwhole,
     int nsplit_tail, float *__restrict__ partial_base, int xcd_groups, const int32_t *__restrict__ q_count,
     int64_t split_major_items, const int32_t *__restrict__ k_count, const uint32_t *__restrict__ k_bias, int64_t ldkb,
-    const DevPlan *__restrict__ dev_plan) {
+    const DevPlan *__restrict__ dev_plan, int64_t nsamples) {
     using F = Frag<T>;
     using vec = typename F::vec;
     using elem = typename F::elem;
@@ -531,36 +561,39 @@
     }
     if constexpr (PV16)
         write_output16<T, D>(o16, out, ldo, b, h, q0, M, Mp, lane);
+    else if constexpr (PANEL)
+        write_output_panels<T, D>(o, l_run, out, ldo, b, h, q0, M, Mp, b + 1 == nsamples ? ldo - b * Mp : Mp,
+                                  lin % nqb == nqb - 1, QB, l31, hi);
     else
         write_output<T, D>(o, l_run, out, ldo, b, h, q0, M, Mp, l31, hi);
 }
 
 constexpr size_t lds_for(int D) { return (size_t)2 * (KV * ((D + 15) / 16 * 16 + 8) + vrows_for(D) * VT_STRIDE) * 2; }
 
-template <typename T, int D, bool FOLD>
+template <typename T, int D, bool FOLD, bool PANEL>
 void launch_main(const Call &c, const Launch &g) {
-    hipLaunchKernelGGL((attention_kernel<T, D, FOLD>), dim3((unsigned)g.wgs), dim3(waves_for(D) * 64), lds_for(D), c.s,
+    hipLaunchKernelGGL((attention_kernel<T, D, FOLD, PANEL>), dim3((unsigned)g.wgs), dim3(waves_for(D) * 64), lds_for(D), c.s,
                        (const T *)c.q, c.ldq, (const T *)c.k, c.ldk, (const T *)c.vt, c.ldvt, (T *)c.out, c.ldo, c.h, c.M, c.Mp,
                        c.Mk, c.Mkp, g.scale_log2e, g.src_batch, g.nqb, g.whole, g.nsplit, g.partial, g.xcd_groups, c.q_count,
-                       g.split_major, c.k_count, c.k_bias, c.ldkb, plan_of(g));
-}
-
-template <typename T, int D>
+                       g.split_major, c.k_count, c.k_bias, c.ldkb, plan_of(g), c.B);
+}
+
+template <typename T, int D, bool PANEL>
 void launch_combine(const Call &c, const Launch &g) {
     if constexpr (!pv16_for(D) && acc_floats(D) % 8 == 0) {
         if (g.plan == nullptr && g.split_items * 4 <= vtm::device_cus()) {
-            hipLaunchKernelGGL((attention_combine_parts_kernel<T, D>), dim3((unsigned)g.split_items, (unsigned)(acc_floats(D) / 8)),
+            hipLaunchKernelGGL((attention_combine_parts_kernel<T, D, PANEL>), dim3((unsigned)g.split_items, (unsigned)(acc_floats(D) / 8)),
                                dim3(waves_for(D) * 64), 0, c.s, (const float *)g.partial, (T *)c.out, c.ldo, c.h, c.M, c.Mp,
-                               g.nqb, g.whole, g.nsplit, g.xcd_groups, c.q_count);
+                               g.nqb, g.whole, g.nsplit, g.xcd_groups, c.q_count, c.B);
             return;
         }
     }
-    hipLaunchKernelGGL((attention_combine_kernel<T, D>), dim3((unsigned)g.split_items), dim3(waves_for(D) * 64), 0, c.s,
+    hipLaunchKernelGGL((attention_combine_kernel<T, D, PANEL>), dim3((unsigned)g.split_items), dim3(waves_for(D) * 64), 0, c.s,
                        (const float *)g.partial, (T *)c.out, c.ldo, c.h, c.M, c.Mp, g.nqb, g.whole, g.nsplit, g.xcd_groups,
-                       c.q_count, plan_of(g));
-}
-
-template <typename T, int D, bool FOLD = false>
+                       c.q_count, plan_of(g), c.B);
+}
+
+template <typename T, int D, bool FOLD = false, bool PANEL = false>
 Family make_family() {
     Family f;
     f.qb = waves_for(D) * QW;
@@ -568,9 +601,9 @@
     f.rec_bytes = (size_t)rec_floats(D) * (waves_for(D) * 64) * sizeof(float);
     f.xcd_min_nqb = 64;
     f.ws_devplan_min_tiles = 16;
-    if constexpr (lds_for(D) > 64 * 1024) f.lds_opt_in = opt_in_lds<attention_kernel<T, D, FOLD>, lds_for(D)>;
-    f.main = launch_main<T, D, FOLD>;
-    f.combine = launch_combine<T, D>;
+    if constexpr (lds_for(D) > 64 * 1024) f.lds_opt_in = opt_in_lds<attention_kernel<T, D, FOLD, PANEL>, lds_for(D)>;
+    f.main = launch_main<T, D, FOLD, PANEL>;
+    f.combine = launch_combine<T, D, PANEL>;
     return f;
 }
 
@@ -600,7 +633,7 @@
     VTM_REQUIRE(c.share_groups >= 1 && c.B % c.share_groups == 0, "%s: B %% share_groups != 0", who);
     if (c.fold)
         VTM_REQUIRE(d == 40 || d == 8, "%s: head dim %lld has no spare k-slots for the bias (d = 8, 40 do)", who, (long long)d);
-    VTM_REQUIRE(c.ldq % 8 == 0 && c.ldk % 8 == 0 && c.ldvt % 8 == 0 && c.ldo % 4 == 0 && c.ldvt >= c.Mk,
+    VTM_REQUIRE(c.ldq % 8 == 0 && c.ldk % 8 == 0 && c.ldvt % 8 == 0 && (c.panel_rows != 0 || c.ldo % 4 == 0) && c.ldvt >= c.Mk,
                 "%s: leading dimensions must keep 16-byte alignment (ldvt >= Mk, %% 8)", who);
     VTM_REQUIRE((c.Mkp * c.ldk + d) * 2 < (1ll << 31) && (d * c.ldvt + c.Mkp) * 2 < (1ll << 31) &&
                     (!c.fold || c.Mkp * 4 < (1ll << 31)),
@@ -621,10 +654,20 @@
 static int attention_any(const void *q, int64_t ldq, const void *k, int64_t ldk, const void *vt, int64_t ldvt,
                          void *out, int64_t ldo, int dtype, int64_t B, int64_t h, int64_t Mq, int64_t Mqp, int64_t Mk,
                          int64_t Mkp, int64_t d, float scale, int share_groups, void *ws, size_t ws_bytes,
-                         const int32_t *q_count, vtm_stream_t stream) {
-    const Call c{q, ldq, k, ldk, vt, ldvt, out, ldo, dtype, B, h, Mq, Mqp, Mk, Mkp, scale, share_groups, ws, ws_bytes,
-                 q_count, vtm::as_stream(stream), false, nullptr, nullptr, 0};
+                         const int32_t *q_count, vtm_stream_t stream, int64_t panel_rows = 0) {
+    Call c{q, ldq, k, ldk, vt, ldvt, out, ldo, dtype, B, h, Mq, Mqp, Mk, Mkp, scale, share_groups, ws, ws_bytes,
+           q_count, vtm::as_stream(stream), false, nullptr, nullptr, 0};
+    c.panel_rows = panel_rows;
     if (const int e = check_call(c, d, "vtm_attention")) return e;
+    if (panel_rows != 0) {
+        if (dtype != VTM_F16 && dtype != VTM_BF16)
+            return vtm::fail(VTM_EINVAL, "vtm_attention_kv_panels: dtype must be VTM_F16 or VTM_BF16");
+        const bool f16 = dtype == VTM_F16;
+        if (d == 64) return planned_launch(c, f16 ? make_family<__half, 64, false, true>() : make_family<vtm_bf16, 64, false, true>());
+        if (d == 80) return planned_launch(c, f16 ? make_family<__half, 80, false, true>() : make_family<vtm_bf16, 80, false, true>());
+        if (d == 160) return planned_launch(c, f16 ? make_family<__half, 160, false, true>() : make_family<vtm_bf16, 160, false, true>());
+        return vtm::fail(VTM_EINVAL, "vtm_attention_kv_panels: head dim %lld has no panel output (have 64, 80, 160)", (long long)d);
+    }
     if (dtype == VTM_F32) return attention_f32(c, d);
     const int ng = shape16_for(d, share_groups, dtype);
     if (ng == 1) return attention16(c);
@@ -643,6 +686,16 @@
                                 vtm_stream_t stream) {
     return attention_any(q, ldq, k, ldk, vt, ldvt, out, ldo, dtype, B, h, Mq, Mqp, Mk, Mkp, d, scale, share_groups, ws,
                          ws_bytes, nullptr, stream);
+}
+
+VTM_EXPORT int vtm_attention_kv_panels(const void *q, int64_t ldq, const void *k, int64_t ldk, const void *vt, int64_t ldvt,
+                                       void *out_panels, int64_t panel_rows, int dtype, int64_t B, int64_t h, int64_t Mq,
+                                       int64_t Mqp, int64_t Mk, int64_t Mkp, int64_t d, float scale, int share_groups,
+                                       const int32_t *q_count, void *ws, size_t ws_bytes, vtm_stream_t stream) {
+    VTM_REQUIRE(panel_rows >= B * Mqp && (reinterpret_cast<uintptr_t>(out_panels) & 15) == 0,
+                "vtm_attention_kv_panels: panel_rows must hold the B * Mqp rows, 16-byte aligned output");
+    return attention_any(q, ldq, k, ldk, vt, ldvt, out_panels, panel_rows, dtype, B, h, Mq, Mqp, Mk, Mkp, d, scale, share_groups,
+                         ws, ws_bytes, q_count, stream, panel_rows);
 }
 
 VTM_EXPORT int vtm_attention_kv_bounded(const void *q, int64_t ldq, const void *k, int64_t ldk, const void *vt, int64_t ldvt,
diff --git a/vidtome_amd/csrc/attention_common.h b/vidtome_amd/csrc/attention_common.h
--- a/vidtome_amd/csrc/attention_common.h
+++ b/vidtome_amd/csrc/attention_common.h
@@ -116,6 +116,55 @@
 }
 
 template <typename T, int D>
+__device__ __forceinline__ void write_output_panels(const f32x16 (&o)[(D + 31) / 32], float l_run, T *__restrict__ out,
+                                                    int64_t prows, int64_t b, int64_t h, int64_t q0, int64_t M, int64_t Mp,
+                                                    int64_t row_end, bool last_block, int qb_rows, int l31, int hi) {
+    using elem = typename Frag<T>::elem;
+    static_assert(D % 16 == 0, "a lane pair trades the halves of TWO panels");
+    constexpr int DV = (D + 31) / 32;
+    constexpr bool SPARE = (D % 32) != 0;
+    float l_tot;
+    if constexpr (SPARE) {
+        constexpr int LB = D / 32, LR = D % 32;
+        constexpr int LHI = (LR >> 2) & 1, LREG = (LR & 3) + 4 * (LR >> 3);
+        l_tot = __shfl(o[LB][LREG], l31 + 32 * LHI, 64);
+    } else {
+        l_tot = l_run + __shfl_xor(l_run, 32, 64);
+    }
+    const float inv_l = 1.0f / l_tot;
+    const int64_t qi = q0 + l31;
+    uint4 *op = reinterpret_cast<uint4 *>(out) + (h * (D / 8)) * prows + b * Mp;
+#pragma unroll
+    for (int dv = 0; dv < DV; ++dv)
+#pragma unroll
+        for (int gp = 0; gp < 2; ++gp) {
+            if (dv * 32 + 16 * gp < D) {
+                uint2 w2[2];
+#pragma unroll
+                for (int gi = 0; gi < 2; ++gi) {
+                    elem w[4];
+#pragma unroll
+                    for (int e = 0; e < 4; ++e) w[e] = (elem)(o[dv][(2 * gp + gi) * 4 + e] * inv_l);
+                    w2[gi] = *reinterpret_cast<uint2 *>(w);
+                }
+                const uint2 keep = hi ? w2[1] : w2[0], give = hi ? w2[0] : w2[1];
+                uint2 got;
+                got.x = __shfl_xor(give.x, 32, 64);
+                got.y = __shfl_xor(give.y, 32, 64);
+                uint4 v = hi ? make_uint4(got.x, got.y, keep.x, keep.y) : make_uint4(keep.x, keep.y, got.x, got.y);
+                if (qi >= M) v = make_uint4(0, 0, 0, 0);
+                if (qi < row_end) op[(dv * 4 + 2 * gp + hi) * prows + qi] = v;
+            }
+        }
+    if (last_block) {
+        const int64_t blk_end = q0 - q0 % qb_rows + qb_rows;
+        for (int64_t r = blk_end + q0 % qb_rows + l31; r < row_end; r += qb_rows)
+#pragma unroll
+            for (int p = hi; p < D / 8; p += 2) op[p * prows + r] = make_uint4(0, 0, 0, 0);
+    }
+}
+
+template <typename T, int D>
 __device__ __forceinline__ void write_output16(const f32x4 (&o)[(D + 16) / 16][2], T *__restrict__ out, int64_t ldo,
                                                int64_t b, int64_t h, int64_t q0, int64_t M, int64_t Mp, int lane) {
     using elem = typename Frag<T>::elem;
diff --git a/vidtome_amd/csrc/attention_plan.h b/vidtome_amd/csrc/attention_plan.h
--- a/vidtome_amd/csrc/attention_plan.h
+++ b/vidtome_amd/csrc/attention_plan.h
@@ -50,6 +50,7 @@
     int dtype; int64_t B, h, M, Mp, Mk, Mkp; float scale; int share_groups; void *ws; size_t ws_bytes;
     const int32_t *q_count; hipStream_t s; bool fold; const int32_t *k_count; const uint32_t *k_bias; int64_t ldkb;
     const struct KeySets *sets = nullptr;
+    int64_t panel_rows = 0;
 };
 
 constexpr int MAX_KEY_SETS = 8;
diff --git a/vidtome_amd/csrc/ff.hip b/vidtome_amd/csrc/ff.hip
--- a/vidtome_amd/csrc/ff.hip
+++ b/vidtome_amd/csrc/ff.hip
@@ -56,9 +56,11 @@
     int64_t n;
     int64_t N;
     int64_t nbias;
+    int64_t w_batch;
+    int64_t out_batch;
 };
 
-template <typename T, int EPI>
+template <typename T, int EPI, bool BATCH = false>
 __global__ __launch_bounds__(THREADS, 2) void panel_gemm_kernel(
     const uint4 *__restrict__ ah, const uint4 *__restrict__ bh, int64_t Ns_pad, int64_t Nd_pad, int64_t C_pad,
     int ns_tiles, int nd_tiles, int nsplit, int tiles_per_split, int total_src_tiles, int patch_tiles, Epi E) {
@@ -85,10 +87,14 @@
     const int KT = (int)(C_pad / FBK);
     const int steps = (jt1 - jt0) * KT;
     const uint4 *srch = ah, *dsth = bh;
+    if constexpr (BATCH) dsth += (int64_t)blockIdx.y * E.w_batch;
     const int64_t srow0 = (int64_t)st_ * FBS + wave * 64;
 
     __shared__ Epi sE;
-    if (tid == 0) sE = E;
+    if (tid == 0) {
+        sE = E;
+        if constexpr (BATCH) sE.out = static_cast<uint16_t *>(E.out) + (int64_t)blockIdx.y * E.out_batch;
+    }
     {
         const int cnt = (jt1 - jt0) * FBD;
         const float *bsrc = E.bias != nullptr ? E.bias + (int64_t)jt0 * FBD : nullptr;
@@ -320,9 +326,9 @@
 
 inline int64_t pad256(int64_t n) { return vtm::cdiv(n, FBS) * FBS; }
 
-template <typename T, int EPI>
+template <typename T, int EPI, bool BATCH = false>
 int launch_panel_gemm(const void *tok, int64_t n, int64_t n_pad, const void *w, int64_t Nw, int64_t Nw_pad, int64_t K,
-                      const Epi &E, hipStream_t s) {
+                      const Epi &E, hipStream_t s, int64_t nbatch = 1) {
     VTM_REQUIRE(2 * n_pad * 16 < (1ll << 32), "panel GEMM: %lld token panel rows exceed the 32-bit fragment offset",
                 (long long)n_pad);
     const int ns_tiles = (int)vtm::cdiv(n, FBS), nd_tiles = (int)vtm::cdiv(Nw, FBD);
@@ -340,7 +346,7 @@
     nsplit = vtm::cdiv(nd_tiles, tiles_per_split);
     const int64_t grid = (int64_t)8 * vtm::cdiv(ngroups, 8) * patch_tiles * nsplit;
     if (grid >= (1ll << 31)) return vtm::fail(VTM_EINVAL, "vtm_ff: grid too large");
-    hipLaunchKernelGGL((panel_gemm_kernel<T, EPI>), dim3((unsigned)grid), dim3(THREADS), 0, s, (const uint4 *)tok,
+    hipLaunchKernelGGL((panel_gemm_kernel<T, EPI, BATCH>), dim3((unsigned)grid, (unsigned)nbatch), dim3(THREADS), 0, s, (const uint4 *)tok,
                        (const uint4 *)w, n_pad, Nw_pad, K, ns_tiles, nd_tiles, (int)nsplit, tiles_per_split, total_src_tiles,
                        patch_tiles, E);
     return vtm::launch_status("vtm_ff");
@@ -383,7 +389,7 @@
     VTM_REQUIRE(n > 0 && n_pad >= n && n_pad % FBS == 0, "vtm_ff_geglu: token rows must be padded to 256");
     VTM_REQUIRE(D > 0 && D % 64 == 0 && w_rows_pad >= 2 * D && w_rows_pad % FBS == 0, "vtm_ff_geglu: D %% 64, packed weight rows padded to 256");
     VTM_REQUIRE(K > 0 && K % FBK == 0, "vtm_ff_geglu: K must be a multiple of 64");
-    Epi E{bias, out_panels, n_pad, 0, nullptr, n, D, 2 * D};
+    Epi E{bias, out_panels, n_pad, 0, nullptr, n, D, 2 * D, 0, 0};
     hipStream_t s = vtm::as_stream(stream);
     if (dtype == VTM_F16) return launch_panel_gemm<__half, EPI_GEGLU>(x_panels, n, n_pad, w1_panels, 2 * D, w_rows_pad, K, E, s);
     if (dtype == VTM_BF16) return launch_panel_gemm<vtm_bf16, EPI_GEGLU>(x_panels, n, n_pad, w1_panels, 2 * D, w_rows_pad, K, E, s);
@@ -399,9 +405,27 @@
     VTM_REQUIRE(K > 0 && K % FBK == 0, "vtm_linear_panels: K must be a multiple of 64");
     VTM_REQUIRE(ldo >= N && ldo % 8 == 0 && (reinterpret_cast<uintptr_t>(out) & 15) == 0 &&
                     (reinterpret_cast<uintptr_t>(resid) & 15) == 0, "vtm_linear_panels: output rows must be 16-byte aligned");
-    Epi E{bias, out, 0, ldo, resid, n, N, N};
+    Epi E{bias, out, 0, ldo, resid, n, N, N, 0, 0};
     hipStream_t s = vtm::as_stream(stream);
     if (dtype == VTM_F16) return launch_panel_gemm<__half, EPI_ROWS>(x_panels, n, n_pad, w_panels, N, w_rows_pad, K, E, s);
     if (dtype == VTM_BF16) return launch_panel_gemm<vtm_bf16, EPI_ROWS>(x_panels, n, n_pad, w_panels, N, w_rows_pad, K, E, s);
     return vtm::fail(VTM_EINVAL, "vtm_linear_panels: dtype must be VTM_F16 or VTM_BF16");
 }
+
+VTM_EXPORT int vtm_linear_panels_batched(const void *x_panels, int64_t n, int64_t n_pad, const void *w_panels, int64_t N,
+                                         int64_t w_rows_pad, int64_t K, const float *bias, int dtype, void *out, int64_t ldo,
+                                         int64_t nbatch, int64_t w_batch_rows, int64_t out_batch, vtm_stream_t stream) {
+    VTM_REQUIRE(x_panels && w_panels && out, "vtm_linear_panels_batched: null pointer");
+    VTM_REQUIRE(n > 0 && n_pad >= vtm::cdiv(n, FBS) * FBS, "vtm_linear_panels_batched: token rows must be padded to 256");
+    VTM_REQUIRE(nbatch >= 1 && nbatch <= 65535 && w_batch_rows >= 0 && out_batch >= 0, "vtm_linear_panels_batched: bad batch");
+    VTM_REQUIRE(N > 0 && N % 8 == 0 && (nbatch - 1) * w_batch_rows + vtm::cdiv(N, FBD) * FBD <= w_rows_pad,
+                "vtm_linear_panels_batched: N %% 8, every sample's weight rows padded to 128 inside the panel");
+    VTM_REQUIRE(K > 0 && K % FBK == 0, "vtm_linear_panels_batched: K must be a multiple of 64");
+    VTM_REQUIRE(ldo >= N && ldo % 8 == 0 && out_batch % 8 == 0 && (reinterpret_cast<uintptr_t>(out) & 15) == 0,
+                "vtm_linear_panels_batched: output rows must be 16-byte aligned");
+    Epi E{bias, out, 0, ldo, nullptr, n, N, N, w_batch_rows, out_batch};
+    hipStream_t s = vtm::as_stream(stream);
+    if (dtype == VTM_F16) return launch_panel_gemm<__half, EPI_ROWS, true>(x_panels, n, n_pad, w_panels, N, w_rows_pad, K, E, s, nbatch);
+    if (dtype == VTM_BF16) return launch_panel_gemm<vtm_bf16, EPI_ROWS, true>(x_panels, n, n_pad, w_panels, N, w_rows_pad, K, E, s, nbatch);
+    return vtm::fail(VTM_EINVAL, "vtm_linear_panels_batched: dtype must be VTM_F16 or VTM_BF16");
+}
diff --git a/vidtome_amd/patch.py b/vidtome_amd/patch.py
--- a/vidtome_amd/patch.py
+++ b/vidtome_amd/patch.py
@@ -429,21 +429,27 @@
     wv, _ = _panel_weight(attn.to_v)
     k_op = _lib.linear_panels(xp, B * Mpad, wk, C, bk).view(B, Mpad, C)
     vt = torch.empty((B, C, Mpad), dtype=x0.dtype, device=x0.device)
-    M8 = (M + 7) // 8 * 8
-    for b in range(B):
-        _lib.linear_panels(wv, C, xp[:, b * Mpad:(b + 1) * Mpad], M8, None, out=vt[b])
+    _lib.linear_panels_batched(wv, C, xp, B, (M + 7) // 8 * 8, Mpad, vt)
+    panel_out = (C // heads) in _lib.PANEL_SITE_HEAD_DIMS
     if q_rows is None:
         q_op = _lib.linear_panels(xp, B * Mpad, wq, C, bq).view(B, Mpad, C)
-        o = _lib.attention(q_op, k_op, vt, heads, M, scale, share)
         Mq, Mqpad = M, Mpad
+        if panel_out:
+            op = _lib.attention_kv_panels(q_op, k_op, vt, heads, M, M, scale, share_groups=share)
+        else:
+            o = _lib.attention(q_op, k_op, vt, heads, M, scale, share)
     else:
         Mq = q_rows.shape[1]
         Mqpad = _lib.panel_rows(Mq)
         qp = _lib.gather_panels(x0, x1, rows, q_rows, Mq)
         q_op = _lib.linear_panels(qp, B * Mqpad, wq, C, bq).view(B, Mqpad, C)
-        o = _lib.attention_kv(q_op, k_op, vt, heads, Mq, M, scale, q_count=q_count, share_groups=share)
+        if panel_out:
+            op = _lib.attention_kv_panels(q_op, k_op, vt, heads, Mq, M, scale, q_count=q_count, share_groups=share)
+        else:
+            o = _lib.attention_kv(q_op, k_op, vt, heads, Mq, M, scale, q_count=q_count, share_groups=share)
     wo, bo = _panel_weight(_out_linear(attn))
-    op = _lib.to_panels(o.view(B * Mqpad, C))
+    if not panel_out:
+        op = _lib.to_panels(o.view(B * Mqpad, C))
     return _lib.linear_panels(op, B * Mqpad, wo, C, bo).view(B, Mqpad, C)
 
 
@@ -484,9 +490,11 @@
     xp = _lib.layernorm_panels(hs, norm.weight, norm.bias, norm.eps)
     qkv = _lib.linear_panels(xp, n, wqkv, 3 * C, bqkv).view(BF, N, 3 * C)
     vt = _lib.transpose_cols(qkv, 2 * C, C)
-    o = _lib.attention(qkv[:, :, :C], qkv[:, :, C:2 * C], vt, heads, N, scale, 1)
     wo, bo = _panel_weight(_out_linear(attn))
-    op = _lib.to_panels(o.view(n, C))
+    if (C // heads) in _lib.PANEL_SITE_HEAD_DIMS:
+        op = _lib.attention_kv_panels(qkv[:, :, :C], qkv[:, :, C:2 * C], vt, heads, N, N, scale)
+    else:
+        op = _lib.to_panels(_lib.attention(qkv[:, :, :C], qkv[:, :, C:2 * C], vt, heads, N, scale, 1).view(n, C))
     return _lib.linear_panels(op, n, wo, C, bo, resid=hs.view(n, C)).view(BF, N, C)
 
 
@@ -681,11 +689,13 @@
     if ip is None:
         Mk = encoder_hidden_states.shape[1]
         k, vt = _cross_kv(attn.to_k, attn.to_v, _pad_keys(encoder_hidden_states, dt), C)
-        o = _lib.attention_kv(q, k, vt, heads, N, Mk, scale)
+        if (C // heads) in _lib.PANEL_SITE_HEAD_DIMS:
+            op = _lib.attention_kv_panels(q, k, vt, heads, N, Mk, scale)
+        else:
+            op = _lib.to_panels(_lib.attention_kv(q, k, vt, heads, N, Mk, scale).view(n, C))
     else:
         k, vt, sets = _ip_key_sets(attn, ip, dt, C, True)
-        o = _lib.attention_kv_sets(q, k, vt, heads, N, sets, scale)
-    op = _lib.to_panels(o.view(n, C))
+        op = _lib.to_panels(_lib.attention_kv_sets(q, k, vt, heads, N, sets, scale).view(n, C))
     return _lib.linear_panels(op, n, wo, C, bo, resid=hs.view(n, C)).view(B, N, C)
 
 
```
